# rs-anderson/explicit-alignment-for-vqa-tasks

Measured on AMD Instinct MI355X. Metric: mapper_train_samples_per_sec, higher is better.
Workload: dtype bf16; 1 GPU; cfg2: CLIP ViT-B/32 -> GPT-2-large (774M), MLP mapper, prefix 10, CC-shaped synthetic batches; per-GPU batch 64, S=42; fwd+bwd+AdamW; random-init weights; global_batch=64, seq_len=42, parallelism=dp1

## Files before the change

### explicit-alignment-for-vqa-tasks_amd/_lib.py

```python
from __future__ import annotations

import ctypes as C
import os

_HERE = os.path.dirname(os.path.abspath(__file__))
LIB_PATH = os.path.join(_HERE, "csrc", "libeavqa_hip.so")

F32, BF16 = 0, 1
ACT = {"none": 0, "tanh": 1, "relu": 2, "gelu_new": 3, "quick_gelu": 4}

i32, i64, f32, ptr = C.c_int, C.c_int64, C.c_float, C.c_void_p

SIGNATURES = {
    "eavqa_abi_version": [],
    "eavqa_strerror": [i32],
    "eavqa_check_device": [],
    "eavqa_gemm": [i32, i32, i32, i32, i32, i32, ptr, i64, ptr, i64, ptr, i64, i32, f32, ptr, i32, ptr, ptr, i64, ptr, i64, ptr],
    "eavqa_layernorm_fwd": [i32, i32, i32, i32, ptr, i64, ptr, ptr, f32, ptr, i64, ptr, ptr, ptr],
    "eavqa_layernorm_bwd": [i32, i32, i32, i32, ptr, i64, ptr, i64, ptr, ptr, ptr, ptr, ptr, i64, ptr, ptr, ptr, i64, ptr],
    "eavqa_layernorm_fwd_fp8": [i32, i32, i32, ptr, i64, ptr, ptr, f32, ptr, i64, ptr, ptr, ptr, ptr],
    "eavqa_layernorm_bwd_fp8": [i32, i32, i32, ptr, i64, ptr, i64, ptr, ptr, ptr, ptr, ptr, i64, ptr, i64, ptr, ptr],
    "eavqa_attention_fwd": [i32, i32, i32, i32, i32, i32, ptr, i64, ptr, i64, ptr, i64, ptr, i64, i64, i64, ptr, i64, ptr, i32, f32, ptr, ptr],
    "eavqa_attention_decode": [i32, i32, i32, i32, i32, ptr, i64, ptr, i64, ptr, i64, i64, ptr, ptr, i64, ptr, i64, ptr, i64, f32, ptr],
    "eavqa_attention_decode_splitk": [i32, i32, i32, i32, i32, ptr, i32, ptr, ptr, i64, ptr, i64, i64, ptr, i64, ptr, i64, f32, ptr],
    "eavqa_attention_bwd": [i32, i32, i32, i32, i32, i32, ptr, i64, ptr, i64, ptr, i64, ptr, i64, ptr, i64,
                            ptr, i64, ptr, i64, ptr, i64, ptr, ptr, i32, f32, ptr, ptr, ptr],
    "eavqa_build_prefix_rows": [i32, i32, i32, ptr, ptr, i32, i32, i32, ptr, ptr, ptr, ptr],
    "eavqa_build_fewshot_rows": [i32, i32, i32, i32, i64, ptr, ptr, i32, ptr, ptr, ptr, ptr, ptr],
    "eavqa_build_row_plan": [i32, i32, i32, ptr, ptr, ptr, ptr, ptr, ptr, ptr, ptr, ptr, ptr],
    "eavqa_copy_rows": [i32, i32, i32, i32, ptr, i64, i64, ptr, i64, i64, i64, ptr],
    "eavqa_transpose": [i32, i32, i32, ptr, i64, ptr, i64, ptr],
    "eavqa_select_rows": [i32, ptr, i32, ptr, ptr, ptr, ptr],
    "eavqa_move_rows": [i32, i32, i32, i32, ptr, i64, ptr, ptr, i64, ptr],
    "eavqa_l2_normalize_rows": [i32, i32, ptr, i64, ptr],
    "eavqa_topk_rows": [i32, i32, ptr, i64, i32, ptr, ptr, ptr],
    "eavqa_gemm_splitk_plan": [i32, i32, i32],
    "eavqa_gemm_splitk": [i32, i32, i32, i32, ptr, i64, ptr, i64, ptr, i32, ptr],
    "eavqa_splitk_finish": [i32, i32, i32, ptr, i32, ptr, i32, ptr, i64, i32, i32, ptr, i64, ptr, i64, ptr, i64, ptr],
    "eavqa_layernorm_splitk": [i32, i32, i32, ptr, i64, ptr, i32, ptr, ptr, i64, ptr, ptr, f32, ptr, i64, ptr],
    "eavqa_gemm_fp8_splitk_plan": [i32, i32, i32],
    "eavqa_gemm_fp8_splitk": [i32, i32, i32, ptr, i64, ptr, ptr, i64, f32, ptr, i32, ptr],
    "eavqa_layernorm_splitk_fp8": [i32, i32, ptr, i64, ptr, i32, ptr, ptr, i64, ptr, ptr, f32, ptr, i64, ptr, ptr],
    "eavqa_rmsnorm_splitk": [i32, i32, i32, ptr, i64, ptr, i32, ptr, i64, ptr, f32, ptr, i64, ptr],
    "eavqa_splitk_finish_gated": [i32, i32, i32, ptr, i32, i32, ptr, i64, ptr],
    "eavqa_attention_decode_splitk_rel": [i32, i32, i32, i32, i32, ptr, i32, i32, ptr, i64, ptr, i64, i64, ptr, i64, ptr, i64, f32, ptr, i64, i32, ptr],
    "eavqa_colsum": [i32, i32, i32, ptr, i64, ptr, i32, ptr],
    "eavqa_embed_assemble": [i32, i32, i32, ptr, ptr, ptr, i64, ptr, i64, ptr, i64, ptr, i64, ptr],
    "eavqa_embed_assemble_bwd": [i32, i32, i32, ptr, ptr, i64, ptr, i64, ptr],
    "eavqa_build_labels": [i32, i32, i32, i32, ptr, i64, i64, ptr, ptr],
    "eavqa_ce_fwd": [i32, i32, i32, ptr, i64, ptr, ptr, ptr, ptr, ptr, ptr],
    "eavqa_guard_count": [ptr, i32, ptr, ptr],
    "eavqa_ce_bwd": [i32, i32, i32, i32, ptr, i64, ptr, ptr, ptr, ptr, ptr, i64, ptr],
    "eavqa_greedy_pick": [i32, i32, ptr, i64, i64, i64, ptr, ptr, i64, ptr, ptr, ptr, ptr],
    "eavqa_adamw": [i64, ptr, ptr, ptr, ptr, i32, f32, f32, f32, f32, f32, f32, i32, ptr, ptr],
    "eavqa_patchify": [i32, i32, i32, i32, ptr, ptr, i64, ptr],
    "eavqa_vit_assemble": [i32, i32, i32, i32, ptr, i64, ptr, ptr, ptr, i64, ptr],
    "eavqa_cast_rows": [i32, i32, i64, ptr, i64, ptr, i64, ptr],
    "eavqa_quantize_rows_fp8": [i32, i32, i32, ptr, i64, ptr, i64, ptr, ptr],
    "eavqa_rmsnorm_fwd": [i32, i32, i32, i32, ptr, i64, ptr, f32, ptr, i64, ptr, ptr],
    "eavqa_rmsnorm_bwd": [i32, i32, i32, i32, ptr, i64, ptr, i64, ptr, ptr, ptr, ptr, i64, ptr, i64, ptr],
    "eavqa_gated_act_fwd": [i32, i32, i32, i32, ptr, i64, ptr, i64, ptr],
    "eavqa_gated_act_bwd": [i32, i32, i32, i32, ptr, i64, ptr, i64, ptr, i64, ptr],
    "eavqa_attention_fwd_rel": [i32, i32, i32, i32, i32, i32, ptr, i64, ptr, i64, ptr, i64, ptr, i64, i64, i64, ptr, i64, i32, f32, ptr, i64, i32, ptr, ptr],
    "eavqa_attention_bwd_rel": [i32, i32, i32, i32, i32, i32, ptr, i64, ptr, i64, ptr, i64, ptr, i64, ptr, i64, ptr, i64, ptr, i64, ptr, i64,
                                ptr, i32, f32, ptr, i64, i32, ptr, ptr, ptr],
    "eavqa_gemm_fp8": [i32, i32, i32, ptr, i64, ptr, ptr, i64, f32, ptr, i64, i32, f32, ptr, i32, ptr, ptr, i64, ptr, i64, ptr, i32],
}
class LMLayer(C.Structure):
    _fields_ = [(n, C.c_void_p) for n in ("ln1_g", "ln1_b", "w_qkv", "b_qkv", "w_o", "b_o", "ln2_g", "ln2_b", "w_fc1", "b_fc1",
                                          "w_fc2", "b_fc2", "k_cache", "v_cache")]


class LMLayerScales(C.Structure):
    _fields_ = [(n, C.c_float) for n in ("s_qkv", "s_o", "s_fc1", "s_fc2")]


class T5DecLayer(C.Structure):
    _fields_ = [(n, C.c_void_p) for n in ("ln_sa", "w_qkv", "w_o", "ln_ca", "w_q_ca", "w_o_ca", "ln_ff", "w_i", "w_o_ff", "k_cache", "v_cache",
                                          "cross_kv")]


class DecodeGemm(C.Structure):
    _fields_ = [("M", i32), ("N", i32), ("K", i32), ("A", ptr), ("lda", i64), ("a_kind", i32), ("gamma", ptr), ("beta", ptr), ("eps", f32),
                ("stats_in", ptr), ("n_stats_in", i32), ("stats_in_cols", i32), ("B", ptr), ("ldb", i64), ("gated_rows", i32),
                ("bias", ptr), ("act", i32), ("residual", ptr), ("ld_residual", i64), ("out_f32", i32), ("n_seg", i32),
                ("out", ptr * 3), ("ld_out", i64 * 3), ("stats_out", ptr)]


class GemmLn(C.Structure):
    _fields_ = [("copy_out", ptr), ("ld_copy", i64), ("stats_out", ptr), ("stats_ld", i32), ("ln_stats", ptr), ("ln_parts", i32),
                ("ln_ld", i32), ("ln_cols", i32), ("ln_c", ptr), ("ln_eps", f32), ("mean_out", ptr), ("rstd_out", ptr)]


SIGNATURES["eavqa_gemm_ln"] = SIGNATURES["eavqa_gemm"][:-1] + [C.POINTER(GemmLn), ptr]
SIGNATURES["eavqa_gemm_decode_cols"] = [i32, i32, i32, i32, i32]
SIGNATURES["eavqa_gemm_decode"] = [C.POINTER(DecodeGemm), ptr]
SIGNATURES["eavqa_t5_decoder_step_workspace_bytes"] = [i32, i32, i32, i32, i32, i32]
SIGNATURES["eavqa_t5_decoder_step"] = [i32, i32, C.POINTER(T5DecLayer), ptr, i32, i32, i32, i32, i32, i32, f32, i32, i32, i32, i32, ptr, ptr, ptr, i64,
                                       ptr, i64, i32, ptr, i64, ptr]
SIGNATURES["eavqa_lm_block_workspace_bytes"] = [i32, i32, i32, i32]
SIGNATURES["eavqa_lm_block_fp8_workspace_bytes"] = [i32, i32, i32]
SIGNATURES["eavqa_lm_block_forward_fp8"] = [i32, C.POINTER(LMLayer), C.POINTER(LMLayerScales), i32, i32, i32, i32, f32, i32, i32, i32, i32, ptr, ptr, i64, ptr, i64, ptr]
SIGNATURES["eavqa_lm_block_forward"] = [i32, i32, C.POINTER(LMLayer), i32, i32, i32, i32, f32, i32, i32, i32, i32, ptr, ptr, i64, ptr, i64, ptr]

SIGNATURES["eavqa_gemm_ex"] = SIGNATURES["eavqa_gemm"] + [i32]
SIGNATURES["eavqa_gemm_ln_ex"] = SIGNATURES["eavqa_gemm_ln"] + [i32]
SIGNATURES["eavqa_attention_fwd_ex"] = SIGNATURES["eavqa_attention_fwd"] + [i32]
SIGNATURES["eavqa_attention_bwd_ex"] = SIGNATURES["eavqa_attention_bwd"] + [i32]
SIGNATURES["eavqa_gemm_splitk_ex"] = SIGNATURES["eavqa_gemm_splitk"] + [i32]
SIGNATURES["eavqa_lm_block_forward_ex"] = SIGNATURES["eavqa_lm_block_forward"] + [i32]
SIGNATURES["eavqa_gemm_decode_ex"] = SIGNATURES["eavqa_gemm_decode"] + [i32]
SIGNATURES["eavqa_t5_decoder_step_ex"] = SIGNATURES["eavqa_t5_decoder_step"] + [i32]

_RESTYPES = {"eavqa_strerror": C.c_char_p, "eavqa_lm_block_workspace_bytes": C.c_int64, "eavqa_lm_block_fp8_workspace_bytes": C.c_int64, "eavqa_t5_decoder_step_workspace_bytes": C.c_int64}

_lib = None


class EavqaError(RuntimeError):
    pass


def load() -> C.CDLL:
    global _lib
    if _lib is not None:
        return _lib
    if not os.path.exists(LIB_PATH):
        raise EavqaError(
            f"{LIB_PATH} is missing: the HIP extension is the only compute path. "
            "Build it with `python -m eavqa_amd.build` (needs hipcc, no GPU required to compile)."
        )
    import torch
    lib = C.CDLL(LIB_PATH)
    for name, argtypes in SIGNATURES.items():
        fn = getattr(lib, name)
        fn.argtypes = argtypes
        fn.restype = _RESTYPES.get(name, C.c_int)
    got = lib.eavqa_abi_version()
    if got != 1:
        raise EavqaError(f"libeavqa_hip.so ABI version {got}, host code expects 1")
    _lib = lib
    return lib


def call(name: str, *args) -> None:
    lib = load()
    rc = getattr(lib, name)(*args)
    if rc != 0:
        raise EavqaError(f"{name} failed: {lib.eavqa_strerror(rc).decode()} (code {rc})")
```

### explicit-alignment-for-vqa-tasks_amd/csrc/gemm.hip

```cpp
#include "common.h"

namespace {

struct Knobs {
    int stagger;
    int ablate;
    bool disable_fast;
    int k64_mode;
    int big_mode;
    int deep;
    int shape_mode;
    int group_n;
    bool no_row_split;
    explicit Knobs(int k = 0) : stagger(k & 15), ablate((k >> 4) & 7), disable_fast(((k >> 7) & 1) != 0), k64_mode((k >> 8) & 63),
                                big_mode((k >> 14) & 3), deep((k >> 16) & 3), shape_mode((k >> 18) & 7), group_n((k >> 21) & 15),
                                no_row_split(((k >> 25) & 1) != 0) {}
};

struct GemmParamsBase {
    const void* A; const void* B; void* C;
    const float* bias; const void* aux_in; void* aux_out; const void* residual;
    const float* row_scale;
    int M, N, K;
    int64_t lda, ldb, ldc, ld_aux, ldr;
    int act, out_f32, res_lowp;
    int out_f16;
    int ablate;
    float alpha;
    int tiles_m, tiles_n;
    int group_n;
    int vec_c, vec_aux, vec_res, vec_bias;
};
struct GemmParams : GemmParamsBase {
    void* copy_out = nullptr; int64_t ld_copy = 0; int vec_copy = 0;
    float* stats_out = nullptr; int stats_ld = 0;
    const float* ln_stats = nullptr; int ln_parts = 0, ln_ld = 0;
    const float* ln_c = nullptr; float ln_inv_n = 0.f, ln_eps = 0.f;
    float* mean_out = nullptr; float* rstd_out = nullptr;
};
constexpr int LN_ROWSTAT_BYTES = 2048;
inline int ln_lds(const GemmParams& p) { return p.ln_stats ? LN_ROWSTAT_BYTES : 0; }
__device__ __forceinline__ GemmParams widen(const GemmParams& k) { return k; }
__device__ __forceinline__ GemmParams widen(const GemmParamsBase& k) { GemmParams p; static_cast<GemmParamsBase&>(p) = k; return p; }
template <bool LNX> struct KernArg { using type = GemmParamsBase; };
template <> struct KernArg<true> { using type = GemmParams; };

constexpr int BM = 128, BN = 128;
constexpr int CS_PITCH = 132;
constexpr int CS_BYTES = BM * CS_PITCH * 4;

__device__ __forceinline__ void tile_coords(const GemmParams& p, int& tm, int& tn) {
    const int nwg = p.tiles_m * p.tiles_n;
    const int bid = blockIdx.x;
    const int q = nwg >> 3, r = nwg & 7, xcd = bid & 7;
    const int wgid = (xcd < r ? xcd * (q + 1) : r * (q + 1) + (xcd - r) * q) + (bid >> 3);
    tm = wgid % p.tiles_m;
    tn = wgid / p.tiles_m;
}

__device__ __forceinline__ void ln_rowstat_fill(const GemmParams& p, float2* rowstat, int m0, int n0, int rows, int tid, int nthreads) {
    if (!p.ln_stats) return;
    for (int r = tid; r < rows; r += nthreads) {
        const int m = min(m0 + r, p.M - 1);
        const float2* q = reinterpret_cast<const float2*>(p.ln_stats) + (int64_t)m * p.ln_ld;
        float s = 0.f, ss = 0.f;
        if (((p.ln_ld | p.ln_parts) & 1) == 0 && (reinterpret_cast<uintptr_t>(p.ln_stats) & 15) == 0) {
            const float4* q4 = reinterpret_cast<const float4*>(q);
            const int n4 = p.ln_parts >> 1;
            for (int i = 0; i < n4; i += 4) {
                float4 t[4];
#pragma unroll
                for (int k = 0; k < 4; ++k) t[k] = q4[min(i + k, n4 - 1)];
#pragma unroll
                for (int k = 0; k < 4; ++k) {
                    const float w = (i + k < n4) ? 1.f : 0.f;
                    s += w * (t[k].x + t[k].z);
                    ss += w * (t[k].y + t[k].w);
                }
            }
        } else {
            for (int i = 0; i < p.ln_parts; ++i) { const float2 t = q[i]; s += t.x; ss += t.y; }
        }
        const float mean = s * p.ln_inv_n;
        const float rstd = 1.0f / sqrtf(fmaxf(ss * p.ln_inv_n - mean * mean, 0.f) + p.ln_eps);
        rowstat[r] = make_float2(rstd, -rstd * mean);
        if (n0 == 0 && m0 + r < p.M && p.mean_out) { p.mean_out[m] = mean; p.rstd_out[m] = rstd; }
    }
}

template <int TPR_, int RPP_, int NPASS_, int PITCH_, int ROWS_ = RPP_ * NPASS_, int LN_UNROLL_ = 4> struct EpiGeo {
    static constexpr int TPR = TPR_, RPP = RPP_, NPASS = NPASS_, PITCH = PITCH_, ROWS = ROWS_;
    static constexpr int LN_UNROLL = LN_UNROLL_;
};
using EpiGeo128 = EpiGeo<32, 8, 16, CS_PITCH>;

template <typename T, int ACT, int MODE, bool FULL, bool LNX>
__device__ __forceinline__ void epilogue_quad(const GemmParams& p, int m, int n, float (&v)[4], const float (&bias4)[4], const float2 rs,
                                              const float (&c4)[4]) {
    const T* aux_in = reinterpret_cast<const T*>(p.aux_in);
    T* aux_out = reinterpret_cast<T*>(p.aux_out);
    const bool full = FULL || (n + 3 < p.N);
    const float al = p.row_scale ? p.alpha * p.row_scale[m] : p.alpha;
    if (LNX && p.ln_stats) {
#pragma unroll
        for (int j = 0; j < 4; ++j) v[j] = (al * rs.x) * v[j] + (bias4[j] + rs.y * c4[j]);
    } else {
#pragma unroll
        for (int j = 0; j < 4; ++j) v[j] = al * v[j] + bias4[j];
    }
    if (aux_out) {
        T* q = aux_out + (int64_t)m * p.ld_aux + n;
        if (FULL || (full && p.vec_aux)) elem<T>::st4(q, make_float4(v[0], v[1], v[2], v[3]));
        else
            for (int j = 0; j < 4; ++j)
                if (n + j < p.N) elem<T>::st(q + j, v[j]);
    }
    if (MODE == 2) {
        const T* q = aux_in + (int64_t)m * p.ld_aux + n;
        float u[4] = {0.f, 0.f, 0.f, 0.f};
        if (FULL || (full && p.vec_aux)) { float4 t = elem<T>::ld4(q); u[0] = t.x; u[1] = t.y; u[2] = t.z; u[3] = t.w; }
        else
            for (int j = 0; j < 4; ++j)
                if (n + j < p.N) u[j] = elem<T>::ld(q + j);
#pragma unroll
        for (int j = 0; j < 4; ++j) v[j] *= act_bwd(ACT, u[j]);
    } else if (MODE == 1) {
#pragma unroll
        for (int j = 0; j < 4; ++j) v[j] = act_fwd(ACT, v[j]);
    }
    if (p.residual) {
        if (p.res_lowp == 2) {
            const f16_t* q = reinterpret_cast<const f16_t*>(p.residual) + (int64_t)m * p.ldr + n;
            if (FULL || (full && p.vec_res)) { float4 t = elem<f16_t>::ld4(q); v[0] += t.x; v[1] += t.y; v[2] += t.z; v[3] += t.w; }
            else
                for (int j = 0; j < 4; ++j)
                    if (n + j < p.N) v[j] += elem<f16_t>::ld(q + j);
        } else if (p.res_lowp) {
            const T* q = reinterpret_cast<const T*>(p.residual) + (int64_t)m * p.ldr + n;
            if (FULL || (full && p.vec_res)) { float4 t = elem<T>::ld4(q); v[0] += t.x; v[1] += t.y; v[2] += t.z; v[3] += t.w; }
            else
                for (int j = 0; j < 4; ++j)
                    if (n + j < p.N) v[j] += elem<T>::ld(q + j);
        } else {
            const float* q = reinterpret_cast<const float*>(p.residual) + (int64_t)m * p.ldr + n;
            if (FULL || (full && p.vec_res)) { float4 t = *reinterpret_cast<const float4*>(q); v[0] += t.x; v[1] += t.y; v[2] += t.z; v[3] += t.w; }
            else
                for (int j = 0; j < 4; ++j)
                    if (n + j < p.N) v[j] += q[j];
        }
    }
    if (p.out_f32) {
        float* q = reinterpret_cast<float*>(p.C) + (int64_t)m * p.ldc + n;
        if (FULL || (full && p.vec_c)) *reinterpret_cast<float4*>(q) = make_float4(v[0], v[1], v[2], v[3]);
        else
            for (int j = 0; j < 4; ++j)
                if (n + j < p.N) q[j] = v[j];
    } else if (p.out_f16) {
        f16_t* q = reinterpret_cast<f16_t*>(p.C) + (int64_t)m * p.ldc + n;
        if (FULL || (full && p.vec_c)) elem<f16_t>::st4(q, make_float4(v[0], v[1], v[2], v[3]));
        else
            for (int j = 0; j < 4; ++j)
                if (n + j < p.N) elem<f16_t>::st(q + j, v[j]);
    } else {
        T* q = reinterpret_cast<T*>(p.C) + (int64_t)m * p.ldc + n;
        if (FULL || (full && p.vec_c)) elem<T>::st4(q, make_float4(v[0], v[1], v[2], v[3]));
        else
            for (int j = 0; j < 4; ++j)
                if (n + j < p.N) elem<T>::st(q + j, v[j]);
    }
    if (LNX && p.copy_out) {
        T* q = reinterpret_cast<T*>(p.copy_out) + (int64_t)m * p.ld_copy + n;
        if (full && p.vec_copy) elem<T>::st4(q, make_float4(v[0], v[1], v[2], v[3]));
        else
            for (int j = 0; j < 4; ++j)
                if (n + j < p.N) elem<T>::st(q + j, v[j]);
    }
}

template <bool FULL>
__device__ __forceinline__ void load_bias4(const GemmParams& p, int n, float (&bias4)[4]) {
    bias4[0] = bias4[1] = bias4[2] = bias4[3] = 0.f;
    if (p.bias) {
        if (FULL) { const float4 b = *reinterpret_cast<const float4*>(p.bias + n); bias4[0] = b.x; bias4[1] = b.y; bias4[2] = b.z; bias4[3] = b.w; }
        else {
#pragma unroll
            for (int j = 0; j < 4; ++j)
                if (n + j < p.N) bias4[j] = p.bias[n + j];
        }
    }
}

struct LnArgs { const float2* rowstat; int row_base; };

template <typename T, int ACT, int MODE, bool FULL, typename G, bool LNX>
__device__ __forceinline__ void epilogue_body(const GemmParams& p, float* Cs, int m0, int n0, const LnArgs ln) {
    const int tid = threadIdx.x;
    if (G::ROWS != G::RPP * G::NPASS && tid >= G::TPR * G::RPP) return;
    const int c4 = (tid % G::TPR) * 4;
    const int n = n0 + c4;
    float bias4[4], lc4[4] = {0.f, 0.f, 0.f, 0.f};
    load_bias4<FULL>(p, n, bias4);
    if (LNX && p.ln_stats) {
#pragma unroll
        for (int j = 0; j < 4; ++j)
            if (FULL || n + j < p.N) lc4[j] = p.ln_c[n + j];
    }
    auto one_pass = [&](int pass) {
        const int row = (tid / G::TPR) + pass * G::RPP;
        const int m = m0 + row;
        if (G::ROWS != G::RPP * G::NPASS && row >= G::ROWS) return;
        if (!FULL && (m >= p.M || n >= p.N)) return;
        const float4 a = *reinterpret_cast<const float4*>(&Cs[row * G::PITCH + c4]);
        float v[4] = {a.x, a.y, a.z, a.w};
        const float2 rs = (LNX && p.ln_stats) ? ln.rowstat[ln.row_base + row] : make_float2(1.f, 0.f);
        epilogue_quad<T, ACT, MODE, FULL, LNX>(p, m, n, v, bias4, rs, lc4);
        if (LNX && p.stats_out) {
            if (!FULL) {
#pragma unroll
                for (int j = 0; j < 4; ++j)
                    if (n + j >= p.N) v[j] = 0.f;
            }
            *reinterpret_cast<float4*>(&Cs[row * G::PITCH + c4]) = make_float4(v[0], v[1], v[2], v[3]);
        }
    };
    if constexpr (LNX && G::LN_UNROLL == 1) {
#pragma unroll 1
        for (int pass = 0; pass < G::NPASS; ++pass) one_pass(pass);
    } else {
#pragma unroll 4
        for (int pass = 0; pass < G::NPASS; ++pass) one_pass(pass);
    }
}

template <typename G>
__device__ __forceinline__ void epilogue_row_sums(const GemmParams& p, const float* Cs, int m0, int n0) {
    constexpr int COLS = G::TPR * 4;
    static_assert(COLS >= 64 && COLS % 4 == 0, "a tile covers at least one 64-column slot");
    __syncthreads();
    const int cols = min(COLS, p.N - n0);
    const int slot0 = n0 / 64, slot1 = (n0 + COLS < p.N) ? (n0 + COLS) / 64 : p.stats_ld;
    for (int r = threadIdx.x; r < G::ROWS; r += blockDim.x) {
        const int m = m0 + r;
        if (m >= p.M) continue;
        float s = 0.f, ss = 0.f;
        for (int c = 0; c < cols; c += 4) {
            const float4 t = *reinterpret_cast<const float4*>(&Cs[r * G::PITCH + c]);
            s += (t.x + t.y) + (t.z + t.w);
            ss += (t.x * t.x + t.y * t.y) + (t.z * t.z + t.w * t.w);
        }
        float2* q = reinterpret_cast<float2*>(p.stats_out) + (int64_t)m * p.stats_ld;
        q[slot0] = make_float2(s, ss);
        for (int i = slot0 + 1; i < slot1; ++i) q[i] = make_float2(0.f, 0.f);
    }
}

template <typename T, int ACT, int MODE, typename G, bool LNX>
__device__ __forceinline__ void epilogue_mode(const GemmParams& p, float* Cs, int m0, int n0, const LnArgs ln) {
    constexpr int ROWS = G::ROWS, COLS = G::TPR * 4;
    const bool full_tile = (m0 + ROWS <= p.M) && (n0 + COLS <= p.N) && p.vec_c && (!(p.aux_in || p.aux_out) || p.vec_aux) &&
                           (!p.residual || p.vec_res) && (!p.bias || p.vec_bias);
    if (full_tile) epilogue_body<T, ACT, MODE, true, G, LNX>(p, Cs, m0, n0, ln);
    else epilogue_body<T, ACT, MODE, false, G, LNX>(p, Cs, m0, n0, ln);
    if (LNX && p.stats_out) epilogue_row_sums<G>(p, Cs, m0, n0);
}

template <typename T, typename G = EpiGeo128, bool LNX = true>
__device__ __forceinline__ void epilogue(const GemmParams& p, float* Cs, int m0, int n0, const LnArgs ln = LnArgs{nullptr, 0}) {
    const int mode = p.aux_in ? 2 : (p.act != EAVQA_ACT_NONE ? 1 : 0);
    if (mode == 0) { epilogue_mode<T, EAVQA_ACT_NONE, 0, G, LNX>(p, Cs, m0, n0, ln); return; }
    switch (p.act) {
        case EAVQA_ACT_TANH:
            if (mode == 1) epilogue_mode<T, EAVQA_ACT_TANH, 1, G, LNX>(p, Cs, m0, n0, ln); else epilogue_mode<T, EAVQA_ACT_TANH, 2, G, LNX>(p, Cs, m0, n0, ln);
            break;
        case EAVQA_ACT_RELU:
            if (mode == 1) epilogue_mode<T, EAVQA_ACT_RELU, 1, G, LNX>(p, Cs, m0, n0, ln); else epilogue_mode<T, EAVQA_ACT_RELU, 2, G, LNX>(p, Cs, m0, n0, ln);
            break;
        case EAVQA_ACT_GELU_NEW:
            if (mode == 1) epilogue_mode<T, EAVQA_ACT_GELU_NEW, 1, G, LNX>(p, Cs, m0, n0, ln); else epilogue_mode<T, EAVQA_ACT_GELU_NEW, 2, G, LNX>(p, Cs, m0, n0, ln);
            break;
        case EAVQA_ACT_QUICK_GELU:
            if (mode == 1) epilogue_mode<T, EAVQA_ACT_QUICK_GELU, 1, G, LNX>(p, Cs, m0, n0, ln); else epilogue_mode<T, EAVQA_ACT_QUICK_GELU, 2, G, LNX>(p, Cs, m0, n0, ln);
            break;
        default:
            epilogue_mode<T, EAVQA_ACT_NONE, 0, G, LNX>(p, Cs, m0, n0, ln);
    }
}

template <typename T, typename G = EpiGeo128>
__device__ __forceinline__ void epilogue_any(const GemmParams& p, float* Cs, int m0, int n0, const LnArgs ln = LnArgs{nullptr, 0}) {
    if (p.ln_stats || p.stats_out || p.copy_out) epilogue<T, G, true>(p, Cs, m0, n0, ln);
    else epilogue<T, G, false>(p, Cs, m0, n0, ln);
}


constexpr int BK16 = 64;
constexpr int OPER16_BYTES = 128 * BK16 * 2;

__device__ __forceinline__ int swz16(int row, int kc) { return row * 128 + ((kc ^ (row & 7)) << 4); }

template <bool KC>
__device__ __forceinline__ void g2r_16(uint4 (&r)[4], const bf16_t* X, int64_t ld, int row0, int rows_max,
                                       int k0, int K) {
    const int tid = threadIdx.x;
#pragma unroll
    for (int i = 0; i < 4; ++i) {
        const int c = tid + 256 * i;
        uint4 v = make_uint4(0u, 0u, 0u, 0u);
        if (KC) {
            const int row = c >> 3, kc = c & 7;
            const int gr = row0 + row, gk = k0 + kc * 8;
            if (gr < rows_max && gk < K) v = *reinterpret_cast<const uint4*>(X + (int64_t)gr * ld + gk);
        } else {
            const int k = c >> 4, rc = c & 15;
            const int gk = k0 + k, gr = row0 + rc * 8;
            if (gk < K && gr < rows_max) v = *reinterpret_cast<const uint4*>(X + (int64_t)gk * ld + gr);
        }
        r[i] = v;
    }
}
template <bool KC>
__device__ __forceinline__ void r2s_16(const uint4 (&r)[4], char* S) {
    const int tid = threadIdx.x;
#pragma unroll
    for (int i = 0; i < 4; ++i) {
        const int c = tid + 256 * i;
        if (KC) {
            const int row = c >> 3, kc = c & 7;
            *reinterpret_cast<uint4*>(S + swz16(row, kc)) = r[i];
        } else {
            const int k = c >> 4, rc = c & 15;
            const unsigned w[4] = {r[i].x, r[i].y, r[i].z, r[i].w};
#pragma unroll
            for (int j = 0; j < 8; ++j) {
                const int row = rc * 8 + j;
                const unsigned short e = (unsigned short)((j & 1) ? (w[j >> 1] >> 16) : (w[j >> 1] & 0xffffu));
                *reinterpret_cast<unsigned short*>(S + swz16(row, k >> 3) + (k & 7) * 2) = e;
            }
        }
    }
}

template <bool A_KC, bool B_KC>
__global__ __launch_bounds__(256) void gemm_bf16_kernel(GemmParams p) {
    extern __shared__ __attribute__((aligned(16))) char smem[];
    char* const As0 = smem;
    char* const Bs0 = smem + 2 * OPER16_BYTES;

    int tm, tn;
    tile_coords(p, tm, tn);
    const int m0 = tm * BM, n0 = tn * BN;
    const int tid = threadIdx.x, lane = tid & 63, wave = tid >> 6;
    const int wm = wave >> 1, wn = wave & 1;
    const bf16_t* A = reinterpret_cast<const bf16_t*>(p.A);
    const bf16_t* B = reinterpret_cast<const bf16_t*>(p.B);

    f32x4 acc[4][4];
#pragma unroll
    for (int i = 0; i < 4; ++i)
#pragma unroll
        for (int j = 0; j < 4; ++j) acc[i][j] = (f32x4){0.f, 0.f, 0.f, 0.f};

    const int nk = (p.K + BK16 - 1) / BK16;
    uint4 ra[4], rb[4];
    g2r_16<A_KC>(ra, A, p.lda, m0, p.M, 0, p.K);
    g2r_16<B_KC>(rb, B, p.ldb, n0, p.N, 0, p.K);
    r2s_16<A_KC>(ra, As0);
    r2s_16<B_KC>(rb, Bs0);
    __syncthreads();

    const int frow = lane & 15, fk = lane >> 4;
    for (int kt = 0; kt < nk; ++kt) {
        const int cur = kt & 1;
        if (kt + 1 < nk) {
            g2r_16<A_KC>(ra, A, p.lda, m0, p.M, (kt + 1) * BK16, p.K);
            g2r_16<B_KC>(rb, B, p.ldb, n0, p.N, (kt + 1) * BK16, p.K);
        }
        const char* Ac = As0 + cur * OPER16_BYTES;
        const char* Bc = Bs0 + cur * OPER16_BYTES;
#pragma unroll
        for (int s = 0; s < 2; ++s) {
            bf16x8 af[4], bfr[4];
#pragma unroll
            for (int i = 0; i < 4; ++i) {
                const int row = wm * 64 + i * 16 + frow;
                af[i] = *reinterpret_cast<const bf16x8*>(Ac + swz16(row, s * 4 + fk));
            }
#pragma unroll
            for (int j = 0; j < 4; ++j) {
                const int row = wn * 64 + j * 16 + frow;
                bfr[j] = *reinterpret_cast<const bf16x8*>(Bc + swz16(row, s * 4 + fk));
            }
#pragma unroll
            for (int i = 0; i < 4; ++i)
#pragma unroll
                for (int j = 0; j < 4; ++j)
                    acc[i][j] = __builtin_amdgcn_mfma_f32_16x16x32_bf16(af[i], bfr[j], acc[i][j], 0, 0, 0);
        }
        if (kt + 1 < nk) {
            r2s_16<A_KC>(ra, As0 + (cur ^ 1) * OPER16_BYTES);
            r2s_16<B_KC>(rb, Bs0 + (cur ^ 1) * OPER16_BYTES);
        }
        __syncthreads();
    }

    float* Cs = reinterpret_cast<float*>(smem);
#pragma unroll
    for (int i = 0; i < 4; ++i)
#pragma unroll
        for (int j = 0; j < 4; ++j)
#pragma unroll
            for (int r = 0; r < 4; ++r) {
                const int row = wm * 64 + i * 16 + (lane >> 4) * 4 + r;
                const int col = wn * 64 + j * 16 + (lane & 15);
                Cs[row * CS_PITCH + col] = acc[i][j][r];
            }
    float2* rowstat = reinterpret_cast<float2*>(smem + CS_BYTES);
    ln_rowstat_fill(p, rowstat, m0, n0, BM, tid, 256);
    __syncthreads();
    if constexpr (A_KC && B_KC) epilogue_any<bf16_t>(p, Cs, m0, n0, LnArgs{rowstat, 0});
    else epilogue<bf16_t, EpiGeo128, false>(p, Cs, m0, n0);
}


constexpr int FBK = 32;
constexpr int FOPER = 128 * FBK * 2;
constexpr int FSTAGE = 2 * FOPER;

__device__ __forceinline__ int fswz(int row, int kc) { return row * 64 + ((kc ^ ((-(row >> 2)) & 3)) << 4); }

struct FastMap { int gx, gy; };

__device__ __forceinline__ bool fast_tile(const GemmParams& p, int gx, int gy, int& tm, int& tn) {
    const int bid = blockIdx.x, xcd = bid & 7, local = bid >> 3;
    const int xi = xcd % gx, yi = xcd / gx;
    const int qm = p.tiles_m / gx, rm = p.tiles_m % gx, qn = p.tiles_n / gy, rn = p.tiles_n % gy;
    const int m_begin = xi * qm + min(xi, rm), m_cnt = qm + (xi < rm ? 1 : 0);
    const int n_begin = yi * qn + min(yi, rn), n_cnt = qn + (yi < rn ? 1 : 0);
    if (m_cnt == 0 || local >= m_cnt * n_cnt) return false;
    tm = m_begin + local % m_cnt;
    tn = n_begin + local / m_cnt;
    return true;
}

#define EAVQA_FAST_STEP(P, t)                                                                         \
    {                                                                                                 \
        const int rem = nk - 2 - (t);                                      \
         \
         \
         \
         \
        __builtin_amdgcn_sched_barrier(0);                                                            \
        __builtin_amdgcn_s_waitcnt(0xC07F);                                            \
        if ((t) + 1 < nk) {                                                                           \
             \
             \
             \
            if (ABL < 3) {                                                                            \
            if (rem >= NST - 2) __builtin_amdgcn_s_waitcnt(vm_only(4 * (NST - 2)));                   \
            else if (rem >= 6) __builtin_amdgcn_s_waitcnt(vm_only(24));                               \
            else if (rem == 5) __builtin_amdgcn_s_waitcnt(vm_only(20));                               \
            else if (rem == 4) __builtin_amdgcn_s_waitcnt(vm_only(16));                               \
            else if (rem == 3) __builtin_amdgcn_s_waitcnt(vm_only(12));                               \
            else if (rem == 2) __builtin_amdgcn_s_waitcnt(vm_only(8));                                \
            else if (rem == 1) __builtin_amdgcn_s_waitcnt(vm_only(4));                                \
            else __builtin_amdgcn_s_waitcnt(vm_only(0));                                              \
            __builtin_amdgcn_s_barrier();                                                             \
            }                                                                                         \
            if ((ABL < 1 || ABL >= 4) && (t) + NST < nk) issue((t) + NST);                            \
            if (ABL < 2) {                                                                            \
            const char* st = smem + (((t) + 1) & (NST - 1)) * FSTAGE;                                 \
            _Pragma("unroll") for (int i = 0; i < 4; ++i)                                             \
                fa[(P) ^ 1][i] = *reinterpret_cast<const bf16x8*>(st + a_off + i * 1024);             \
            _Pragma("unroll") for (int j = 0; j < 4; ++j)                                             \
                fb[(P) ^ 1][j] = *reinterpret_cast<const bf16x8*>(st + b_off + j * 1024);             \
            } else {                                                                                  \
            _Pragma("unroll") for (int i = 0; i < 4; ++i) { fa[(P) ^ 1][i] = fa[P][i]; fb[(P) ^ 1][i] = fb[P][i]; } \
            }                                                                                         \
        }                                                                                             \
        if (ABL != 4) {                                                                               \
        _Pragma("unroll") for (int i = 0; i < 4; ++i)                                                 \
            _Pragma("unroll") for (int j = 0; j < 4; ++j)                                             \
                acc[i][j] = __builtin_amdgcn_mfma_f32_16x16x32_bf16(fa[P][i], fb[P][j], acc[i][j], 0, 0, 0); \
        }                                                                                             \
    }

__device__ __host__ constexpr int vm_only(int n) { return (n & 15) | ((n >> 4) << 14) | 0x0F70; }

template <int ABL, int NST>
__global__ __launch_bounds__(256, 2) void gemm_bf16_fast_kernel(GemmParams p, int gx, int gy, int stagger) {
    extern __shared__ __attribute__((aligned(16))) char smem[];
    int tm, tn;
    if (!fast_tile(p, gx, gy, tm, tn)) return;
    if (stagger > 0 && ((blockIdx.x >> 3) & 1))
        for (int i = 0; i < stagger; ++i) __builtin_amdgcn_s_sleep(8);
    const int m0 = tm * BM, n0 = tn * BN;
    const int tid = threadIdx.x, lane = tid & 63;
    const int wave = __builtin_amdgcn_readfirstlane(tid >> 6);
    const int wm = wave >> 1, wn = wave & 1;
    const bf16_t* A = reinterpret_cast<const bf16_t*>(p.A);
    const bf16_t* B = reinterpret_cast<const bf16_t*>(p.B);

    const bf16_t* asrc[2];
    const bf16_t* bsrc[2];
#pragma unroll
    for (int i = 0; i < 2; ++i) {
        const int c = tid + 256 * i;
        const int row = c >> 2, pc = c & 3;
        const int kc = pc ^ ((-(row >> 2)) & 3);
        asrc[i] = A + (int64_t)min(m0 + row, p.M - 1) * p.lda + kc * 8;
        bsrc[i] = B + (int64_t)min(n0 + row, p.N - 1) * p.ldb + kc * 8;
    }
    const int dma_off = wave * 1024;

    auto issue = [&](int kt) {
        char* st = smem + (kt & (NST - 1)) * FSTAGE;
#pragma unroll
        for (int i = 0; i < 2; ++i) {
            __builtin_amdgcn_global_load_lds((const __attribute__((address_space(1))) void*)(asrc[i] + kt * FBK),
                                             (__attribute__((address_space(3))) void*)(st + dma_off + i * 4096), 16, 0, 0);
            if (ABL != 5 || i == 0 || lane < 16)
            __builtin_amdgcn_global_load_lds((const __attribute__((address_space(1))) void*)(bsrc[i] + kt * FBK),
                                             (__attribute__((address_space(3))) void*)(st + FOPER + dma_off + i * 4096), 16, 0, 0);
        }
    };

    f32x4 acc[4][4];
#pragma unroll
    for (int i = 0; i < 4; ++i)
#pragma unroll
        for (int j = 0; j < 4; ++j) acc[i][j] = (f32x4){0.f, 0.f, 0.f, 0.f};

    const int nk = p.K / FBK;
    const int frow = lane & 15, fk = lane >> 4;
    const int a_off = fswz(wm * 64 + frow, fk);
    const int b_off = FOPER + fswz(wn * 64 + frow, fk);
    bf16x8 fa[2][4], fb[2][4];

#pragma unroll
    for (int i = 0; i < NST; ++i)
        if (i < nk) issue(i);
    {
        const int later = min(nk, NST) - 1;
        if (later >= 7) __builtin_amdgcn_s_waitcnt(vm_only(28));
        else if (later == 6) __builtin_amdgcn_s_waitcnt(vm_only(24));
        else if (later == 5) __builtin_amdgcn_s_waitcnt(vm_only(20));
        else if (later == 4) __builtin_amdgcn_s_waitcnt(vm_only(16));
        else if (later == 3) __builtin_amdgcn_s_waitcnt(vm_only(12));
        else if (later == 2) __builtin_amdgcn_s_waitcnt(vm_only(8));
        else if (later == 1) __builtin_amdgcn_s_waitcnt(vm_only(4));
        else __builtin_amdgcn_s_waitcnt(vm_only(0));
    }
    __builtin_amdgcn_s_barrier();
#pragma unroll
    for (int i = 0; i < 4; ++i) fa[0][i] = *reinterpret_cast<const bf16x8*>(smem + a_off + i * 1024);
#pragma unroll
    for (int j = 0; j < 4; ++j) fb[0][j] = *reinterpret_cast<const bf16x8*>(smem + b_off + j * 1024);

    int t = 0;
    for (; t + 1 < nk; t += 2) {
        EAVQA_FAST_STEP(0, t)
        EAVQA_FAST_STEP(1, t + 1)
    }
    if (t < nk) EAVQA_FAST_STEP(0, t)
    __syncthreads();

    float* Cs = reinterpret_cast<float*>(smem);
#pragma unroll
    for (int i = 0; i < 4; ++i)
#pragma unroll
        for (int j = 0; j < 4; ++j)
#pragma unroll
            for (int r = 0; r < 4; ++r) {
                const int row = wm * 64 + i * 16 + (lane >> 4) * 4 + r;
                const int col = wn * 64 + j * 16 + (lane & 15);
                Cs[row * CS_PITCH + col] = acc[i][j][r];
            }
    __syncthreads();
    epilogue<bf16_t, EpiGeo128, false>(p, Cs, m0, n0);
}
#undef EAVQA_FAST_STEP


typedef void (*fast_kernel_t)(GemmParams, int, int, int);

int launch_fast(const GemmParams& p, hipStream_t stream, const Knobs& kn) {
    static const fast_kernel_t kernels[2] = {gemm_bf16_fast_kernel<0, 4>, gemm_bf16_fast_kernel<0, 8>};
    static std::atomic<bool> configured{false};
    if (!configured.load(std::memory_order_acquire)) {
        for (int i = 0; i < 2; ++i)
            if (hipFuncSetAttribute(reinterpret_cast<const void*>(kernels[i]), hipFuncAttributeMaxDynamicSharedMemorySize,
                                    8 * FSTAGE) != hipSuccess)
                return EAVQA_E_LAUNCH;
        configured.store(true, std::memory_order_release);
    }
    const bool deep = kn.deep == 2;
    const fast_kernel_t kernel = deep ? kernels[1] : kernels[0];
    const int lds_bytes = deep ? 8 * FSTAGE : CS_BYTES;
    int best_gx = 8, best_cost = 1 << 30;
    const int cand[4] = {8, 4, 2, 1};
    for (int c = 0; c < 4; ++c) {
        const int gx = cand[c], gy = 8 / gx;
        const int cost = (p.tiles_m + gx - 1) / gx + (p.tiles_n + gy - 1) / gy;
        if (cost < best_cost) { best_cost = cost; best_gx = gx; }
    }
    const int gx = best_gx, gy = 8 / gx;
    const int per_xcd = ((p.tiles_m + gx - 1) / gx) * ((p.tiles_n + gy - 1) / gy);
    hipLaunchKernelGGL(kernel, dim3(per_xcd * 8), dim3(256), lds_bytes, stream, p, gx, gy, kn.stagger);
    EAVQA_LAUNCH_CHECK();
    return EAVQA_OK;
}


__device__ __forceinline__ bool shaped_tile(int gx, int gy, int tiles_m, int tiles_n, int& tm, int& tn) {
    const int bid = blockIdx.x, xcd = bid & 7, local = bid >> 3;
    if (gx == 0) {
        const int nwg = tiles_m * tiles_n, q = nwg >> 3, r = nwg & 7;
        if (local >= q + (xcd < r ? 1 : 0)) return false;
        const int wgid = (xcd < r ? xcd * (q + 1) : r * (q + 1) + (xcd - r) * q) + local;
        tm = wgid % tiles_m;
        tn = wgid / tiles_m;
        return true;
    }
    const int xi = xcd % gx, yi = xcd / gx;
    const int qm = tiles_m / gx, rm = tiles_m % gx, qn = tiles_n / gy, rn = tiles_n % gy;
    const int m_begin = xi * qm + min(xi, rm), m_cnt = qm + (xi < rm ? 1 : 0);
    const int n_begin = yi * qn + min(yi, rn), n_cnt = qn + (yi < rn ? 1 : 0);
    if (m_cnt == 0 || local >= m_cnt * n_cnt) return false;
    tm = m_begin + local % m_cnt;
    tn = n_begin + local / m_cnt;
    return true;
}

struct GridPlan { int gx, gy, per_xcd; };
inline GridPlan plan_grid(int tiles_m, int tiles_n, int bm, int bn) {
    GridPlan g{8, 1, 0};
    int best_cost = 1 << 30;
    const int cand[4] = {8, 4, 2, 1};
    for (int c = 0; c < 4; ++c) {
        const int gx = cand[c], gy = 8 / gx;
        const int cost = ((tiles_m + gx - 1) / gx) * bm + ((tiles_n + gy - 1) / gy) * bn;
        if (cost < best_cost) { best_cost = cost; g.gx = gx; g.gy = gy; }
    }
    g.per_xcd = ((tiles_m + g.gx - 1) / g.gx) * ((tiles_n + g.gy - 1) / g.gy);
    const int even = (tiles_m * tiles_n + 7) / 8;
    if ((g.per_xcd + 31) / 32 > (even + 31) / 32) { g.gx = 0; g.gy = 0; g.per_xcd = even; }
    return g;
}

template <int WM, int WN, int MF, int NF> struct TileGeo {
    static constexpr int NT = 64 * WM * WN, NW = WM * WN;
    static constexpr int TBM = 16 * MF * WM, TBN = 16 * NF * WN;
    static constexpr int AFULL = 4 * TBM / NT, BFULL = 4 * TBN / NT;
    static constexpr int BREM = (4 * TBN - BFULL * NT) / NW;
    static constexpr int NDMA = AFULL + BFULL + (BREM > 0 ? 1 : 0);
    static constexpr int AOPER = TBM * 64, STAGE = (TBM + TBN) * 64, RING = 4 * STAGE;
    static constexpr int PITCH = TBN + 4;
    static constexpr int SP = (16 * MF * WM * PITCH * 4 <= RING) ? WM : ((16 * MF * (WM / 2) * PITCH * 4 <= RING) ? WM / 2 : 1);
    static constexpr int PROWS = 16 * MF * SP;
    static constexpr int TPR = TBN / 4, RPP = NT / TPR, NPASS = (PROWS + RPP - 1) / RPP;
    static_assert(4 * TBM == AFULL * NT, "A stage must split evenly");
    static_assert(BFULL * NT + BREM * NW == 4 * TBN && BREM < 64, "B stage: full pieces + one partial piece per wave");
    static_assert(16 * MF * PITCH * 4 <= RING, "one wave row of C must fit the ring");
    static_assert(WM % SP == 0, "passes cover whole wave rows");
};

#define EAVQA_SHAPED_STEP(P, t)                                                                       \
    {                                                                                                 \
        const int rem = nk - 2 - (t);                                                                 \
        __builtin_amdgcn_sched_barrier(0);                                                            \
        __builtin_amdgcn_s_waitcnt(0xC07F);                \
        if ((t) + 1 < nk) {                                                                           \
            if (rem >= 2) __builtin_amdgcn_s_waitcnt(vm_only(2 * G::NDMA));                           \
            else if (rem == 1) __builtin_amdgcn_s_waitcnt(vm_only(G::NDMA));                          \
            else __builtin_amdgcn_s_waitcnt(vm_only(0));                                              \
            __builtin_amdgcn_s_barrier();                                                             \
            if ((t) + 4 < nk) issue((t) + 4);                                                         \
            const char* st = smem + (((t) + 1) & 3) * G::STAGE;                                       \
            _Pragma("unroll") for (int i = 0; i < MF; ++i)                                            \
                fa[(P) ^ 1][i] = *reinterpret_cast<const bf16x8*>(st + a_off + i * 1024);             \
            _Pragma("unroll") for (int j = 0; j < NF; ++j)                                            \
                fb[(P) ^ 1][j] = *reinterpret_cast<const bf16x8*>(st + b_off + j * 1024);             \
        }                                                                                             \
        _Pragma("unroll") for (int i = 0; i < MF; ++i)                                                \
            _Pragma("unroll") for (int j = 0; j < NF; ++j)                                            \
                acc[i][j] = __builtin_amdgcn_mfma_f32_16x16x32_bf16(fa[P][i], fb[P][j], acc[i][j], 0, 0, 0); \
    }

template <int WM, int WN, int MF, int NF>
__global__ __launch_bounds__(64 * WM * WN, (WM * WN <= 4) ? 2 : 1) void gemm_bf16_shaped_kernel(GemmParams p, int gx, int gy, int tiles_m, int tiles_n) {
    using G = TileGeo<WM, WN, MF, NF>;
    extern __shared__ __attribute__((aligned(16))) char smem[];
    int tm, tn;
    if (!shaped_tile(gx, gy, tiles_m, tiles_n, tm, tn)) return;
    const int m0 = tm * G::TBM, n0 = tn * G::TBN;
    const int tid = threadIdx.x, lane = tid & 63;
    const int wave = __builtin_amdgcn_readfirstlane(tid >> 6);
    const int wm = wave / WN, wn = wave % WN;
    const bf16_t* A = reinterpret_cast<const bf16_t*>(p.A);
    const bf16_t* B = reinterpret_cast<const bf16_t*>(p.B);

    auto src_of = [&](const bf16_t* X, int64_t ld, int row0, int rows_max, int c) {
        const int row = c >> 2, pc = c & 3;
        return X + (int64_t)min(row0 + row, rows_max - 1) * ld + (pc ^ ((-(row >> 2)) & 3)) * 8;
    };
    const bf16_t* asrc[G::AFULL];
    const bf16_t* bsrc[G::BFULL + 1];
#pragma unroll
    for (int i = 0; i < G::AFULL; ++i) asrc[i] = src_of(A, p.lda, m0, p.M, tid + G::NT * i);
#pragma unroll
    for (int i = 0; i < G::BFULL; ++i) bsrc[i] = src_of(B, p.ldb, n0, p.N, tid + G::NT * i);
    bsrc[G::BFULL] = src_of(B, p.ldb, n0, p.N, G::BFULL * G::NT + wave * G::BREM + min(lane, max(G::BREM, 1) - 1));
    const int dma_off = wave * 1024;
    const int dma_off_x = G::AOPER + G::BFULL * G::NT * 16 + wave * G::BREM * 16;

    auto issue = [&](int kt) {
        char* st = smem + (kt & 3) * G::STAGE;
#pragma unroll
        for (int i = 0; i < G::AFULL; ++i)
            __builtin_amdgcn_global_load_lds((const __attribute__((address_space(1))) void*)(asrc[i] + kt * FBK),
                                             (__attribute__((address_space(3))) void*)(st + dma_off + i * G::NT * 16), 16, 0, 0);
#pragma unroll
        for (int i = 0; i < G::BFULL; ++i)
            __builtin_amdgcn_global_load_lds((const __attribute__((address_space(1))) void*)(bsrc[i] + kt * FBK),
                                             (__attribute__((address_space(3))) void*)(st + G::AOPER + dma_off + i * G::NT * 16), 16, 0, 0);
        if (G::BREM > 0 && lane < G::BREM)
            __builtin_amdgcn_global_load_lds((const __attribute__((address_space(1))) void*)(bsrc[G::BFULL] + kt * FBK),
                                             (__attribute__((address_space(3))) void*)(st + dma_off_x), 16, 0, 0);
    };

    f32x4 acc[MF][NF];
#pragma unroll
    for (int i = 0; i < MF; ++i)
#pragma unroll
        for (int j = 0; j < NF; ++j) acc[i][j] = (f32x4){0.f, 0.f, 0.f, 0.f};

    const int nk = p.K / FBK;
    const int frow = lane & 15, fk = lane >> 4;
    const int a_off = fswz(wm * 16 * MF + frow, fk);
    const int b_off = G::AOPER + fswz(wn * 16 * NF + frow, fk);
    bf16x8 fa[2][MF], fb[2][NF];

#pragma unroll
    for (int i = 0; i < 4; ++i)
        if (i < nk) issue(i);
    {
        const int later = min(nk, 4) - 1;
        if (later == 3) __builtin_amdgcn_s_waitcnt(vm_only(3 * G::NDMA));
        else if (later == 2) __builtin_amdgcn_s_waitcnt(vm_only(2 * G::NDMA));
        else if (later == 1) __builtin_amdgcn_s_waitcnt(vm_only(G::NDMA));
        else __builtin_amdgcn_s_waitcnt(vm_only(0));
    }
    __builtin_amdgcn_s_barrier();
#pragma unroll
    for (int i = 0; i < MF; ++i) fa[0][i] = *reinterpret_cast<const bf16x8*>(smem + a_off + i * 1024);
#pragma unroll
    for (int j = 0; j < NF; ++j) fb[0][j] = *reinterpret_cast<const bf16x8*>(smem + b_off + j * 1024);

    int t = 0;
    for (; t + 1 < nk; t += 2) {
        EAVQA_SHAPED_STEP(0, t)
        EAVQA_SHAPED_STEP(1, t + 1)
    }
    if (t < nk) EAVQA_SHAPED_STEP(0, t)
    __syncthreads();

    float* Cs = reinterpret_cast<float*>(smem);
    for (int pass = 0; pass < WM / G::SP; ++pass) {
        if (wm / G::SP == pass) {
            const int r0 = (wm % G::SP) * 16 * MF;
#pragma unroll
            for (int i = 0; i < MF; ++i)
#pragma unroll
                for (int j = 0; j < NF; ++j)
#pragma unroll
                    for (int r = 0; r < 4; ++r) {
                        const int row = r0 + i * 16 + (lane >> 4) * 4 + r;
                        const int col = wn * 16 * NF + j * 16 + (lane & 15);
                        Cs[row * G::PITCH + col] = acc[i][j][r];
                    }
        }
        __syncthreads();
        epilogue<bf16_t, EpiGeo<G::TPR, G::RPP, G::NPASS, G::PITCH, G::PROWS>, false>(p, Cs, m0 + pass * G::PROWS, n0);
        if (pass + 1 < WM / G::SP) __syncthreads();
    }
}
#undef EAVQA_SHAPED_STEP

template <int WM, int WN, int MF, int NF>
int launch_shaped(const GemmParams& p, hipStream_t stream) {
    using G = TileGeo<WM, WN, MF, NF>;
    static std::atomic<bool> configured{false};
    if (!configured.load(std::memory_order_acquire)) {
        if (hipFuncSetAttribute(reinterpret_cast<const void*>(gemm_bf16_shaped_kernel<WM, WN, MF, NF>),
                                hipFuncAttributeMaxDynamicSharedMemorySize, G::RING) != hipSuccess)
            return EAVQA_E_LAUNCH;
        configured.store(true, std::memory_order_release);
    }
    const int tiles_m = (p.M + G::TBM - 1) / G::TBM, tiles_n = (p.N + G::TBN - 1) / G::TBN;
    const GridPlan g = plan_grid(tiles_m, tiles_n, G::TBM, G::TBN);
    hipLaunchKernelGGL((gemm_bf16_shaped_kernel<WM, WN, MF, NF>), dim3(g.per_xcd * 8), dim3(G::NT), G::RING, stream, p, g.gx, g.gy,
                       tiles_m, tiles_n);
    EAVQA_LAUNCH_CHECK();
    return EAVQA_OK;
}


struct ShapeChoice { int bm, bn; float rate; int (*launch)(const GemmParams&, hipStream_t); };
const ShapeChoice SHAPES[5] = {
    {128, 80, 1.17f, launch_shaped<4, 1, 2, 5>}, {128, 96, 1.20f, launch_shaped<4, 1, 2, 6>},
    {256, 128, 1.15f, launch_shaped<4, 2, 4, 4>}, {256, 160, 1.23f, launch_shaped<4, 2, 4, 5>}, {256, 192, 1.39f, launch_shaped<4, 2, 4, 6>},
};
constexpr float RATE_FAST = 1.245f, RATE_BIG = 1.27f;

inline float tile_cost(const GemmParams& p, int bm, int bn, float rate) {
    const int tiles_m = (p.M + bm - 1) / bm, tiles_n = (p.N + bn - 1) / bn;
    const GridPlan g = plan_grid(tiles_m, tiles_n, bm, bn);
    const float rounds = float((g.per_xcd + 31) / 32);
    return rounds * (rate * (bm + bn) * (p.K / 32) + 0.25f * bm * bn);
}

constexpr int GBM = 256, GBN = 256, GBK = 64;
constexpr int BIG_GROUP_N = 8;
constexpr int GOPER = GBM * GBK * 2;
constexpr int GSTAGE = 2 * GOPER;
constexpr int GCS_PITCH = GBN + 4;
constexpr int GLDS_BYTES = 2 * GSTAGE;
using EpiGeo256 = EpiGeo<64, 16, 4, GCS_PITCH, 64, 1>;

__device__ __forceinline__ bool big_tile(const GemmParams& p, int gx, int gy, int tiles_m, int tiles_n, int& tm, int& tn) {
    const int bid = blockIdx.x, xcd = bid & 7, local = bid >> 3;
    const int xi = xcd % gx, yi = xcd / gx;
    const int qm = tiles_m / gx, rm = tiles_m % gx, qn = tiles_n / gy, rn = tiles_n % gy;
    const int m_begin = xi * qm + min(xi, rm), m_cnt = qm + (xi < rm ? 1 : 0);
    const int n_begin = yi * qn + min(yi, rn), n_cnt = qn + (yi < rn ? 1 : 0);
    if (m_cnt == 0 || local >= m_cnt * n_cnt) return false;
    const int GN = p.group_n;
    if (GN <= 0) {
        tm = m_begin + local % m_cnt;
        tn = n_begin + local / m_cnt;
        return true;
    }
    const int per_group = m_cnt * GN;
    const int g = local / per_group, r = local - g * per_group;
    const int gn = min(GN, n_cnt - g * GN);
    tm = m_begin + r / gn;
    tn = n_begin + g * GN + r % gn;
    return true;
}

template <bool LNX>
__global__ __launch_bounds__(1024) void gemm_bf16_big_kernel(typename KernArg<LNX>::type pk, int gx, int gy, int tiles_m, int tiles_n) {
    const GemmParams p = widen(pk);
    extern __shared__ __attribute__((aligned(16))) char smem[];
    int tm, tn;
    if (!big_tile(p, gx, gy, tiles_m, tiles_n, tm, tn)) return;
    const int m0 = tm * GBM, n0 = tn * GBN;
    const int tid = threadIdx.x, lane = tid & 63;
    const int wave = __builtin_amdgcn_readfirstlane(tid >> 6);
    const int wm = wave >> 2, wn = wave & 3;
    const bf16_t* A = reinterpret_cast<const bf16_t*>(p.A);
    const bf16_t* B = reinterpret_cast<const bf16_t*>(p.B);

    const bf16_t* asrc[2];
    const bf16_t* bsrc[2];
#pragma unroll
    for (int i = 0; i < 2; ++i) {
        const int c = tid + 1024 * i;
        const int row = c >> 3, pc = c & 7;
        asrc[i] = A + (int64_t)min(m0 + row, p.M - 1) * p.lda + (pc ^ (row & 7)) * 8;
        bsrc[i] = B + (int64_t)min(n0 + row, p.N - 1) * p.ldb + (pc ^ (row & 7)) * 8;
    }
    const int dma_off = wave * 1024;
    auto issue = [&](int kt) {
        char* st = smem + (kt & 1) * GSTAGE;
#pragma unroll
        for (int i = 0; i < 2; ++i) {
            __builtin_amdgcn_global_load_lds((const __attribute__((address_space(1))) void*)(asrc[i] + kt * GBK),
                                             (__attribute__((address_space(3))) void*)(st + dma_off + i * 16384), 16, 0, 0);
            __builtin_amdgcn_global_load_lds((const __attribute__((address_space(1))) void*)(bsrc[i] + kt * GBK),
                                             (__attribute__((address_space(3))) void*)(st + GOPER + dma_off + i * 16384), 16, 0, 0);
        }
    };

    f32x4 acc[4][4];
#pragma unroll
    for (int i = 0; i < 4; ++i)
#pragma unroll
        for (int j = 0; j < 4; ++j) acc[i][j] = (f32x4){0.f, 0.f, 0.f, 0.f};

    const int nk = p.K / GBK;
    const int frow = lane & 15, fk = lane >> 4;
    const int arow = wm * 64 + frow, brow = wn * 64 + frow;
    issue(0);
    float2* rowstat = reinterpret_cast<float2*>(smem + GLDS_BYTES);
    if (LNX) ln_rowstat_fill(p, rowstat, m0, n0, GBM, tid, 1024);
    for (int kt = 0; kt < nk; ++kt) {
        __builtin_amdgcn_sched_barrier(0);
        __builtin_amdgcn_s_waitcnt(0x0070);
        __builtin_amdgcn_s_barrier();
        if (kt + 1 < nk) issue(kt + 1);
        const char* st = smem + (kt & 1) * GSTAGE;
#pragma unroll
        for (int s = 0; s < 2; ++s) {
            bf16x8 af[4], bfr[4];
            const int sw = ((s * 4 + fk) ^ (frow & 7)) << 4;
#pragma unroll
            for (int i = 0; i < 4; ++i) af[i] = *reinterpret_cast<const bf16x8*>(st + (arow + 16 * i) * 128 + sw);
#pragma unroll
            for (int j = 0; j < 4; ++j) bfr[j] = *reinterpret_cast<const bf16x8*>(st + GOPER + (brow + 16 * j) * 128 + sw);
#pragma unroll
            for (int i = 0; i < 4; ++i)
#pragma unroll
                for (int j = 0; j < 4; ++j)
                    acc[i][j] = __builtin_amdgcn_mfma_f32_16x16x32_bf16(af[i], bfr[j], acc[i][j], 0, 0, 0);
        }
    }
    __syncthreads();

    float* Cs = reinterpret_cast<float*>(smem);
    for (int slab = 0; slab < 4; ++slab) {
        if (wm == slab) {
#pragma unroll
            for (int i = 0; i < 4; ++i)
#pragma unroll
                for (int j = 0; j < 4; ++j)
#pragma unroll
                    for (int r = 0; r < 4; ++r) {
                        const int row = i * 16 + (lane >> 4) * 4 + r;
                        const int col = wn * 64 + j * 16 + (lane & 15);
                        Cs[row * GCS_PITCH + col] = acc[i][j][r];
                    }
        }
        __syncthreads();
        epilogue<bf16_t, EpiGeo256, LNX>(p, Cs, m0 + slab * 64, n0, LnArgs{rowstat, slab * 64});
        __syncthreads();
    }
}

inline int big_grid(int tiles_m, int tiles_n, int& gx, int& gy) {
    int best_gx = 8, best_cost = 1 << 30, best_rounds = 1 << 30;
    const int cand[4] = {8, 4, 2, 1};
    for (int c = 0; c < 4; ++c) {
        const int x = cand[c], y = 8 / x;
        const int pm = (tiles_m + x - 1) / x, pn = (tiles_n + y - 1) / y;
        const int rounds = (pm * pn + 31) / 32, cost = pm + pn;
        if (rounds < best_rounds || (rounds == best_rounds && cost < best_cost)) { best_rounds = rounds; best_cost = cost; best_gx = x; }
    }
    gx = best_gx; gy = 8 / gx;
    return ((tiles_m + gx - 1) / gx) * ((tiles_n + gy - 1) / gy);
}

int launch_big(const GemmParams& p, hipStream_t stream) {
    static std::atomic<bool> configured{false};
    if (!configured.load(std::memory_order_acquire)) {
        if (hipFuncSetAttribute(reinterpret_cast<const void*>(gemm_bf16_big_kernel<false>), hipFuncAttributeMaxDynamicSharedMemorySize,
                                GLDS_BYTES) != hipSuccess ||
            hipFuncSetAttribute(reinterpret_cast<const void*>(gemm_bf16_big_kernel<true>), hipFuncAttributeMaxDynamicSharedMemorySize,
                                GLDS_BYTES + LN_ROWSTAT_BYTES) != hipSuccess)
            return EAVQA_E_LAUNCH;
        configured.store(true, std::memory_order_release);
    }
    const int tiles_m = (p.M + GBM - 1) / GBM, tiles_n = (p.N + GBN - 1) / GBN;
    int gx, gy;
    const int per_xcd = big_grid(tiles_m, tiles_n, gx, gy);
    if (p.ln_stats || p.stats_out || p.copy_out)
        hipLaunchKernelGGL(gemm_bf16_big_kernel<true>, dim3(per_xcd * 8), dim3(1024), GLDS_BYTES + ln_lds(p), stream, p, gx, gy, tiles_m, tiles_n);
    else
        hipLaunchKernelGGL(gemm_bf16_big_kernel<false>, dim3(per_xcd * 8), dim3(1024), GLDS_BYTES, stream, p, gx, gy, tiles_m, tiles_n);
    EAVQA_LAUNCH_CHECK();
    return EAVQA_OK;
}

inline int big_split_rows(int M, int N) {
    const int rem = M % GBM;
    if (rem == 0 || rem > 192 || M <= GBM) return 0;
    int gx, gy;
    const int tiles_n = (N + GBN - 1) / GBN;
    const int with = (big_grid((M + GBM - 1) / GBM, tiles_n, gx, gy) + 31) / 32, without = (big_grid(M / GBM, tiles_n, gx, gy) + 31) / 32;
    return without < with ? rem : 0;
}

bool use_big(const GemmParams& p, const Knobs& kn) {
    if (p.K % GBK) return false;
    if (kn.big_mode == 1) return false;
    if (kn.big_mode == 2) return true;
    const int tiles = ((p.M + GBM - 1) / GBM) * ((p.N + GBN - 1) / GBN);
    return tiles >= 144;
}


#include "gemm_k64.hip"

inline float k64_cost(const GemmParams& p, const K64Choice& c, float* multi_round_loop = nullptr) {
    const int tiles_m = (p.M + c.bm - 1) / c.bm, tiles_n = (p.N + c.bn - 1) / c.bn;
    const GridPlan g = plan_grid(tiles_m, tiles_n, c.bm, c.bn);
    const float rounds = float((g.per_xcd + 31) / 32);
    const float loop = rounds * c.rate * (c.bm + c.bn) * (p.K / 64);
    if (multi_round_loop) *multi_round_loop = rounds > 1.f ? loop : 0.f;
    return loop + rounds * 0.1f * c.bm * c.bn + 4500.f;
}

#include "gemm_fp8.hip"

template <int MF>
__global__ __launch_bounds__(512) void gemm_bf16_skinny_kernel(GemmParams p) {
    __shared__ float red[8][64][17];
    const int tid = threadIdx.x, lane = tid & 63, wave = tid >> 6;
    const int x = lane & 15, g = lane >> 4;
    const int n0 = blockIdx.x * 16;
    const bf16_t* A = reinterpret_cast<const bf16_t*>(p.A);
    const bf16_t* B = reinterpret_cast<const bf16_t*>(p.B);
    const int nsteps = p.K >> 5;
    const int per_wave = (nsteps + 7) >> 3;
    const int s_begin = wave * per_wave, s_end = min(nsteps, s_begin + per_wave);
    const bf16_t* bp = B + (int64_t)min(n0 + x, p.N - 1) * p.ldb + 8 * g;
    const bf16_t* ap[MF];
#pragma unroll
    for (int f = 0; f < MF; ++f) ap[f] = A + (int64_t)min(16 * f + x, p.M - 1) * p.lda + 8 * g;
    f32x4 acc[MF];
#pragma unroll
    for (int f = 0; f < MF; ++f) acc[f] = (f32x4){0.f, 0.f, 0.f, 0.f};

    int s = s_begin;
    for (; s + 8 <= s_end; s += 8) {
        bf16x8 b[8], a[8][MF];
#pragma unroll
        for (int u = 0; u < 8; ++u) {
            b[u] = *reinterpret_cast<const bf16x8*>(bp + (s + u) * 32);
#pragma unroll
            for (int f = 0; f < MF; ++f) a[u][f] = *reinterpret_cast<const bf16x8*>(ap[f] + (s + u) * 32);
        }
#pragma unroll
        for (int u = 0; u < 8; ++u)
#pragma unroll
            for (int f = 0; f < MF; ++f) acc[f] = __builtin_amdgcn_mfma_f32_16x16x32_bf16(a[u][f], b[u], acc[f], 0, 0, 0);
    }
    for (; s < s_end; ++s) {
        const bf16x8 b = *reinterpret_cast<const bf16x8*>(bp + s * 32);
#pragma unroll
        for (int f = 0; f < MF; ++f) {
            const bf16x8 a = *reinterpret_cast<const bf16x8*>(ap[f] + s * 32);
            acc[f] = __builtin_amdgcn_mfma_f32_16x16x32_bf16(a, b, acc[f], 0, 0, 0);
        }
    }
#pragma unroll
    for (int f = 0; f < MF; ++f)
#pragma unroll
        for (int r = 0; r < 4; ++r) red[wave][16 * f + 4 * g + r][x] = acc[f][r];
    __syncthreads();
    for (int e = tid; e < MF * 16 * 16; e += 512) {
        const int m = e >> 4, c = e & 15, n = n0 + c;
        if (m >= p.M || n >= p.N) continue;
        float v = 0.f;
#pragma unroll
        for (int w = 0; w < 8; ++w) v += red[w][m][c];
        v = p.alpha * v + (p.bias ? p.bias[n] : 0.f);
        const int64_t ia = (int64_t)m * p.ld_aux + n;
        if (p.aux_out) elem<bf16_t>::st(reinterpret_cast<bf16_t*>(p.aux_out) + ia, v);
        if (p.aux_in) v *= act_bwd(p.act, elem<bf16_t>::ld(reinterpret_cast<const bf16_t*>(p.aux_in) + ia));
        else v = act_fwd(p.act, v);
        if (p.residual) v += p.res_lowp == 2 ? elem<f16_t>::ld(reinterpret_cast<const f16_t*>(p.residual) + (int64_t)m * p.ldr + n)
                             : p.res_lowp ? elem<bf16_t>::ld(reinterpret_cast<const bf16_t*>(p.residual) + (int64_t)m * p.ldr + n)
                                          : reinterpret_cast<const float*>(p.residual)[(int64_t)m * p.ldr + n];
        if (p.out_f32) reinterpret_cast<float*>(p.C)[(int64_t)m * p.ldc + n] = v;
        else if (p.out_f16) elem<f16_t>::st(reinterpret_cast<f16_t*>(p.C) + (int64_t)m * p.ldc + n, v);
        else elem<bf16_t>::st(reinterpret_cast<bf16_t*>(p.C) + (int64_t)m * p.ldc + n, v);
    }
}

int launch_skinny(const GemmParams& p, hipStream_t stream) {
    const int blocks = (p.N + 15) / 16;
    const int mf = (p.M + 15) / 16;
    if (mf == 1) hipLaunchKernelGGL(gemm_bf16_skinny_kernel<1>, dim3(blocks), dim3(512), 0, stream, p);
    else if (mf == 2) hipLaunchKernelGGL(gemm_bf16_skinny_kernel<2>, dim3(blocks), dim3(512), 0, stream, p);
    else if (mf == 3) hipLaunchKernelGGL(gemm_bf16_skinny_kernel<3>, dim3(blocks), dim3(512), 0, stream, p);
    else hipLaunchKernelGGL(gemm_bf16_skinny_kernel<4>, dim3(blocks), dim3(512), 0, stream, p);
    EAVQA_LAUNCH_CHECK();
    return EAVQA_OK;
}

constexpr int BK32 = 16;
constexpr int PITCH32 = 17;
constexpr int OPER32_FLOATS = 128 * PITCH32;

template <bool KC>
__device__ __forceinline__ void g2r_32(float4 (&r)[2], const float* X, int64_t ld, int row0, int rows_max,
                                       int k0, int K) {
    const int tid = threadIdx.x;
#pragma unroll
    for (int i = 0; i < 2; ++i) {
        const int c = tid + 256 * i;
        float4 v = make_float4(0.f, 0.f, 0.f, 0.f);
        if (KC) {
            const int row = c >> 2, kc = c & 3;
            const int gr = row0 + row, gk = k0 + kc * 4;
            if (gr < rows_max && gk < K) v = *reinterpret_cast<const float4*>(X + (int64_t)gr * ld + gk);
        } else {
            const int k = c >> 5, rc = c & 31;
            const int gk = k0 + k, gr = row0 + rc * 4;
            if (gk < K && gr < rows_max) v = *reinterpret_cast<const float4*>(X + (int64_t)gk * ld + gr);
        }
        r[i] = v;
    }
}
template <bool KC>
__device__ __forceinline__ void r2s_32(const float4 (&r)[2], float* S) {
    const int tid = threadIdx.x;
#pragma unroll
    for (int i = 0; i < 2; ++i) {
        const int c = tid + 256 * i;
        const float w[4] = {r[i].x, r[i].y, r[i].z, r[i].w};
        if (KC) {
            const int row = c >> 2, kc = c & 3;
#pragma unroll
            for (int j = 0; j < 4; ++j) S[row * PITCH32 + kc * 4 + j] = w[j];
        } else {
            const int k = c >> 5, rc = c & 31;
#pragma unroll
            for (int j = 0; j < 4; ++j) S[(rc * 4 + j) * PITCH32 + k] = w[j];
        }
    }
}

template <bool A_KC, bool B_KC>
__global__ __launch_bounds__(256) void gemm_f32_kernel(GemmParams p) {
    extern __shared__ __attribute__((aligned(16))) char smem[];
    float* sm = reinterpret_cast<float*>(smem);
    float* const As0 = sm;
    float* const Bs0 = sm + 2 * OPER32_FLOATS;

    int tm, tn;
    tile_coords(p, tm, tn);
    const int m0 = tm * BM, n0 = tn * BN;
    const int tid = threadIdx.x, lane = tid & 63, wave = tid >> 6;
    const int wm = wave >> 1, wn = wave & 1;
    const float* A = reinterpret_cast<const float*>(p.A);
    const float* B = reinterpret_cast<const float*>(p.B);

    f32x16 acc[2][2];
#pragma unroll
    for (int i = 0; i < 2; ++i)
#pragma unroll
        for (int j = 0; j < 2; ++j)
#pragma unroll
            for (int r = 0; r < 16; ++r) acc[i][j][r] = 0.f;

    const int nk = (p.K + BK32 - 1) / BK32;
    float4 ra[2], rb[2];
    g2r_32<A_KC>(ra, A, p.lda, m0, p.M, 0, p.K);
    g2r_32<B_KC>(rb, B, p.ldb, n0, p.N, 0, p.K);
    r2s_32<A_KC>(ra, As0);
    r2s_32<B_KC>(rb, Bs0);
    __syncthreads();

    const int frow = lane & 31, fk = lane >> 5;
    for (int kt = 0; kt < nk; ++kt) {
        const int cur = kt & 1;
        if (kt + 1 < nk) {
            g2r_32<A_KC>(ra, A, p.lda, m0, p.M, (kt + 1) * BK32, p.K);
            g2r_32<B_KC>(rb, B, p.ldb, n0, p.N, (kt + 1) * BK32, p.K);
        }
        const float* Ac = As0 + cur * OPER32_FLOATS;
        const float* Bc = Bs0 + cur * OPER32_FLOATS;
#pragma unroll
        for (int s = 0; s < BK32 / 2; ++s) {
            float af[2], bfr[2];
#pragma unroll
            for (int i = 0; i < 2; ++i) af[i] = Ac[(wm * 64 + i * 32 + frow) * PITCH32 + s * 2 + fk];
#pragma unroll
            for (int j = 0; j < 2; ++j) bfr[j] = Bc[(wn * 64 + j * 32 + frow) * PITCH32 + s * 2 + fk];
#pragma unroll
            for (int i = 0; i < 2; ++i)
#pragma unroll
                for (int j = 0; j < 2; ++j)
                    acc[i][j] = __builtin_amdgcn_mfma_f32_32x32x2f32(af[i], bfr[j], acc[i][j], 0, 0, 0);
        }
        if (kt + 1 < nk) {
            r2s_32<A_KC>(ra, As0 + (cur ^ 1) * OPER32_FLOATS);
            r2s_32<B_KC>(rb, Bs0 + (cur ^ 1) * OPER32_FLOATS);
        }
        __syncthreads();
    }

    float* Cs = reinterpret_cast<float*>(smem);
#pragma unroll
    for (int i = 0; i < 2; ++i)
#pragma unroll
        for (int j = 0; j < 2; ++j)
#pragma unroll
            for (int r = 0; r < 16; ++r) {
                const int row = wm * 64 + i * 32 + (r & 3) + 8 * (r >> 2) + 4 * (lane >> 5);
                const int col = wn * 64 + j * 32 + (lane & 31);
                Cs[row * CS_PITCH + col] = acc[i][j][r];
            }
    float2* rowstat = reinterpret_cast<float2*>(smem + CS_BYTES);
    ln_rowstat_fill(p, rowstat, m0, n0, BM, tid, 256);
    __syncthreads();
    if constexpr (A_KC && B_KC) epilogue_any<float>(p, Cs, m0, n0, LnArgs{rowstat, 0});
    else epilogue<float, EpiGeo128, false>(p, Cs, m0, n0);
}

typedef void (*gemm_kernel_t)(GemmParams);

int launch(gemm_kernel_t kernel, const GemmParams& p, hipStream_t stream) {
    static std::atomic<gemm_kernel_t> configured[8];
    bool done = false;
    for (int i = 0; i < 8; ++i) done |= (configured[i].load(std::memory_order_acquire) == kernel);
    if (!done) {
        if (hipFuncSetAttribute(reinterpret_cast<const void*>(kernel), hipFuncAttributeMaxDynamicSharedMemorySize,
                                CS_BYTES + LN_ROWSTAT_BYTES) != hipSuccess)
            return EAVQA_E_LAUNCH;
        for (int i = 0; i < 8; ++i) {
            gemm_kernel_t expected = nullptr;
            if (configured[i].compare_exchange_strong(expected, kernel, std::memory_order_acq_rel) || expected == kernel) break;
        }
    }
    const int nwg = p.tiles_m * p.tiles_n;
    hipLaunchKernelGGL(kernel, dim3(nwg), dim3(256), CS_BYTES + ln_lds(p), stream, p);
    EAVQA_LAUNCH_CHECK();
    return EAVQA_OK;
}


}

namespace {
eavqa_gemm_ln_t ln_rows_from(const eavqa_gemm_ln_t& x, int64_t r0, size_t esz) {
    eavqa_gemm_ln_t y = x;
    if (x.copy_out) y.copy_out = static_cast<char*>(x.copy_out) + (size_t)r0 * (size_t)x.ld_copy * esz;
    if (x.stats_out) y.stats_out = x.stats_out + (size_t)r0 * (size_t)x.stats_ld * 2;
    if (x.ln_stats) y.ln_stats = x.ln_stats + (size_t)r0 * (size_t)x.ln_ld * 2;
    if (x.mean_out) y.mean_out = x.mean_out + r0;
    if (x.rstd_out) y.rstd_out = x.rstd_out + r0;
    return y;
}

int gemm_impl(int dtype, int a_kc, int b_kc, int M, int N, int K,
              const void* A, int64_t lda, const void* B, int64_t ldb,
              void* C, int64_t ldc, int out_flags, float alpha,
              const float* bias, int act,
              const void* aux_in, void* aux_out, int64_t ld_aux,
              const void* residual, int64_t ldr, const eavqa_gemm_ln_t* ln, void* stream, int knobs) {
    const Knobs kn(knobs);
    const bool ln_consumer = ln && ln->ln_stats;
    if (ln) {
        if (ln->copy_out && ln->ld_copy < N) return EAVQA_E_ARG;
        if (ln->stats_out && ln->stats_ld < (N + 63) / 64) return EAVQA_E_ARG;
        if (ln_consumer && (!ln->ln_c || ln->ln_parts <= 0 || ln->ln_ld < ln->ln_parts || ln->ln_cols <= 0 || !(ln->ln_eps >= 0.f))) return EAVQA_E_ARG;
        if ((ln->mean_out != nullptr) != (ln->rstd_out != nullptr) || (ln->mean_out && !ln_consumer)) return EAVQA_E_ARG;
        if (!(a_kc && b_kc)) return EAVQA_E_SHAPE;
    }
    if (out_flags & ~(EAVQA_GEMM_OUT_F32 | EAVQA_GEMM_RESIDUAL_LOWP | EAVQA_GEMM_STREAM_F16)) return EAVQA_E_ARG;
    if ((out_flags & (EAVQA_GEMM_RESIDUAL_LOWP | EAVQA_GEMM_STREAM_F16)) && dtype != EAVQA_BF16) return EAVQA_E_DTYPE;
    const int out_f32 = out_flags & EAVQA_GEMM_OUT_F32;
    const int stream_f16 = (out_flags & EAVQA_GEMM_STREAM_F16) != 0;
    const int res_lowp = (out_flags & EAVQA_GEMM_RESIDUAL_LOWP) ? (stream_f16 ? 2 : 1) : 0;
    if (!A || !B || !C) return EAVQA_E_ARG;
    if (M <= 0 || N <= 0 || K <= 0) return EAVQA_E_ARG;
    if (dtype != EAVQA_F32 && dtype != EAVQA_BF16) return EAVQA_E_DTYPE;
    if (act < EAVQA_ACT_NONE || act > EAVQA_ACT_QUICK_GELU) return EAVQA_E_DTYPE;
    const int vec = dtype == EAVQA_BF16 ? 8 : 4;
    const int a_contig = a_kc ? K : M, b_contig = b_kc ? K : N;
    if (a_contig % vec || b_contig % vec) return EAVQA_E_SHAPE;
    if (lda % vec || ldb % vec) return EAVQA_E_ALIGN;
    if (!eavqa_aligned16(A) || !eavqa_aligned16(B)) return EAVQA_E_ALIGN;
    if (lda < a_contig || ldb < b_contig || ldc < N) return EAVQA_E_ARG;
    if ((aux_in || aux_out) && ld_aux < N) return EAVQA_E_ARG;
    if (residual && ldr < N) return EAVQA_E_ARG;

    GemmParams p;
    p.A = A; p.B = B; p.C = C; p.bias = bias; p.aux_in = aux_in; p.aux_out = aux_out; p.residual = residual; p.row_scale = nullptr; p.ablate = kn.ablate;
    p.M = M; p.N = N; p.K = K; p.lda = lda; p.ldb = ldb; p.ldc = ldc; p.ld_aux = ld_aux; p.ldr = ldr;
    p.act = act; p.out_f32 = out_f32; p.res_lowp = res_lowp; p.out_f16 = stream_f16 && !out_f32; p.alpha = alpha;
    p.group_n = kn.group_n == 0 ? BIG_GROUP_N : kn.group_n - 1;
    p.tiles_m = (M + BM - 1) / BM;
    p.tiles_n = (N + BN - 1) / BN;
    const int esz = dtype == EAVQA_BF16 ? 2 : 4;
    auto vec_ok = [](const void* ptr, int64_t ld, int bytes_per_elem) {
        return ((reinterpret_cast<uintptr_t>(ptr) % (4 * bytes_per_elem)) == 0) && (ld % 4 == 0);
    };
    p.vec_c = vec_ok(C, ldc, out_f32 ? 4 : esz);
    p.vec_aux = vec_ok(aux_in ? aux_in : aux_out, ld_aux, esz);
    p.vec_res = vec_ok(residual, ldr, res_lowp ? esz : 4);
    p.vec_bias = (reinterpret_cast<uintptr_t>(bias) % 16) == 0;
    if (ln) {
        p.copy_out = ln->copy_out; p.ld_copy = ln->ld_copy; p.vec_copy = ln->copy_out ? vec_ok(ln->copy_out, ln->ld_copy, esz) : 0;
        p.stats_out = ln->stats_out; p.stats_ld = ln->stats_ld;
        if (ln_consumer) {
            p.ln_stats = ln->ln_stats; p.ln_parts = ln->ln_parts; p.ln_ld = ln->ln_ld; p.ln_c = ln->ln_c;
            p.ln_inv_n = 1.0f / float(ln->ln_cols); p.ln_eps = ln->ln_eps; p.mean_out = ln->mean_out; p.rstd_out = ln->rstd_out;
        }
    }
    hipStream_t s = reinterpret_cast<hipStream_t>(stream);
    if (dtype == EAVQA_BF16) {
        if (a_kc && b_kc && (K % 64) == 0 && kn.k64_mode >= 2 && kn.k64_mode < 2 + N_K64) return K64_SHAPES[kn.k64_mode - 2].launch(p, s);
        const bool few_columns = kn.k64_mode == 0 && kn.shape_mode == 0 && kn.big_mode == 0 && N <= 4096;
        if (!ln && a_kc && b_kc && !kn.disable_fast && M <= 64 && (K % 32) == 0 && N >= 64 && (kn.k64_mode == 1 || (K % 64) != 0 || few_columns)) return launch_skinny(p, s);
        const int big_rem = (a_kc && b_kc && kn.big_mode != 1 && !kn.no_row_split) ? big_split_rows(M, N) : 0;
        const float big_split_ns = big_rem ? 12000.f : 0.f;
        auto run_big = [&](const GemmParams& pp) -> int {
            if (!big_rem) return launch_big(pp, s);
            GemmParams p1 = pp;
            p1.M = M - big_rem;
            p1.tiles_m = (p1.M + BM - 1) / BM;
            const int rc1 = launch_big(p1, s);
            if (rc1) return rc1;
            const int64_t r0 = M - big_rem;
            const size_t ces = out_f32 ? 4 : 2, res_es = res_lowp ? 2 : 4;
            auto off = [](const void* base, int64_t rows, int64_t ld, size_t es) -> const void* {
                return base ? static_cast<const char*>(base) + (size_t)rows * (size_t)ld * es : nullptr;
            };
            eavqa_gemm_ln_t ln2;
            if (ln) ln2 = ln_rows_from(*ln, r0, 2);
            return gemm_impl(dtype, a_kc, b_kc, big_rem, N, K, off(A, r0, lda, 2), lda, B, ldb, const_cast<void*>(off(C, r0, ldc, ces)), ldc, out_flags,
                             alpha, bias, act, off(aux_in, r0, ld_aux, 2), const_cast<void*>(off(aux_out, r0, ld_aux, 2)), ld_aux,
                             off(residual, r0, ldr, res_es), ldr, ln ? &ln2 : nullptr, stream, 0);
        };
        int bgx, bgy;
        const int big_rounds = (big_grid((M - big_rem + GBM - 1) / GBM, (N + GBN - 1) / GBN, bgx, bgy) + 31) / 32;
        const bool many_big_tiles = big_rounds >= 4 || (big_rounds >= 2 && (M + GBM - 1) / GBM > 96);
        if (a_kc && b_kc && !kn.disable_fast && (K % 64) == 0 && kn.k64_mode != 1 && kn.shape_mode == 0 && kn.big_mode == 0 && !many_big_tiles) {
            int pick = K64_AUTO[0];
            float best_loop = 0.f;
            float best = k64_cost(p, K64_SHAPES[pick], &best_loop);
            for (int i = 1; i < N_K64_AUTO; ++i) {
                float loop;
                const float c = k64_cost(p, K64_SHAPES[K64_AUTO[i]], &loop);
                if (c < best) { best = c; pick = K64_AUTO[i]; best_loop = loop; }
            }
            best += 0.35f * best_loop;
            const float big_cost = float(big_rounds) * (float(K / 64) * (big_rounds == 1 ? 1380.f : 1530.f) + 9000.f) + 3000.f + big_split_ns;
            if (M > 64 && big_cost < best) return run_big(p);
            return K64_SHAPES[pick].launch(p, s);
        }
        if (a_kc && b_kc && !kn.disable_fast && (K % FBK) == 0 && !ln) {
            if (kn.shape_mode >= 2 && kn.shape_mode < 7) return SHAPES[kn.shape_mode - 2].launch(p, s);
            const bool big_ok = (K % GBK) == 0 && kn.big_mode != 1;
            if (big_ok && kn.big_mode == 2) return run_big(p);
            float best = tile_cost(p, 128, 128, RATE_FAST);
            int pick = -1;
            if (big_ok && use_big(p, kn)) {
                GemmParams pf = p;
                pf.M = M - big_rem;
                best = fminf(best, tile_cost(pf, 256, 256, RATE_BIG) + big_split_ns);
                pick = -2;
            }
            if (kn.shape_mode != 1)
                for (int i = 0; i < 5; ++i) {
                    const float c = tile_cost(p, SHAPES[i].bm, SHAPES[i].bn, SHAPES[i].rate);
                    if (c < best * 0.95f) { best = c; pick = i; }
                }
            if (pick >= 0) return SHAPES[pick].launch(p, s);
            if (pick == -2) return run_big(p);
            return launch_fast(p, s, kn);
        }
        if (a_kc && b_kc) return launch(gemm_bf16_kernel<true, true>, p, s);
        if (a_kc && !b_kc) return launch(gemm_bf16_kernel<true, false>, p, s);
        if (!a_kc && b_kc) return launch(gemm_bf16_kernel<false, true>, p, s);
        return launch(gemm_bf16_kernel<false, false>, p, s);
    }
    if (a_kc && b_kc) return launch(gemm_f32_kernel<true, true>, p, s);
    if (a_kc && !b_kc) return launch(gemm_f32_kernel<true, false>, p, s);
    if (!a_kc && b_kc) return launch(gemm_f32_kernel<false, true>, p, s);
    return launch(gemm_f32_kernel<false, false>, p, s);
}
}

extern "C" int eavqa_gemm_ex(int dtype, int a_kc, int b_kc, int M, int N, int K,
                             const void* A, int64_t lda, const void* B, int64_t ldb,
                             void* C, int64_t ldc, int out_flags, float alpha,
                             const float* bias, int act,
                             const void* aux_in, void* aux_out, int64_t ld_aux,
                             const void* residual, int64_t ldr, void* stream, int knobs) {
    return gemm_impl(dtype, a_kc, b_kc, M, N, K, A, lda, B, ldb, C, ldc, out_flags, alpha, bias, act, aux_in, aux_out, ld_aux, residual, ldr,
                     nullptr, stream, knobs);
}

extern "C" int eavqa_gemm_ln_ex(int dtype, int a_kc, int b_kc, int M, int N, int K,
                                const void* A, int64_t lda, const void* B, int64_t ldb,
                                void* C, int64_t ldc, int out_flags, float alpha,
                                const float* bias, int act,
                                const void* aux_in, void* aux_out, int64_t ld_aux,
                                const void* residual, int64_t ldr, const eavqa_gemm_ln_t* ln, void* stream, int knobs) {
    if (!ln) return EAVQA_E_ARG;
    return gemm_impl(dtype, a_kc, b_kc, M, N, K, A, lda, B, ldb, C, ldc, out_flags, alpha, bias, act, aux_in, aux_out, ld_aux, residual, ldr,
                     ln, stream, knobs);
}

extern "C" int eavqa_gemm_ln(int dtype, int a_kc, int b_kc, int M, int N, int K,
                             const void* A, int64_t lda, const void* B, int64_t ldb,
                             void* C, int64_t ldc, int out_flags, float alpha,
                             const float* bias, int act,
                             const void* aux_in, void* aux_out, int64_t ld_aux,
                             const void* residual, int64_t ldr, const eavqa_gemm_ln_t* ln, void* stream) {
    return eavqa_gemm_ln_ex(dtype, a_kc, b_kc, M, N, K, A, lda, B, ldb, C, ldc, out_flags, alpha, bias, act, aux_in, aux_out, ld_aux, residual,
                            ldr, ln, stream, 0);
}

extern "C" int eavqa_gemm(int dtype, int a_kc, int b_kc, int M, int N, int K,
                          const void* A, int64_t lda, const void* B, int64_t ldb,
                          void* C, int64_t ldc, int out_flags, float alpha,
                          const float* bias, int act,
                          const void* aux_in, void* aux_out, int64_t ld_aux,
                          const void* residual, int64_t ldr, void* stream) {
    return eavqa_gemm_ex(dtype, a_kc, b_kc, M, N, K, A, lda, B, ldb, C, ldc, out_flags, alpha, bias, act, aux_in, aux_out, ld_aux,
                         residual, ldr, stream, 0);
}

extern "C" int eavqa_quantize_rows_fp8(int dtype, int rows, int cols, const void* x, int64_t ldx, void* out, int64_t ld_out,
                                       float* row_scale, void* stream) {
    if (!x || !out || !row_scale || rows <= 0 || cols <= 0) return EAVQA_E_ARG;
    if (cols % 4) return EAVQA_E_SHAPE;
    if (ldx % 4 || ld_out % 4 || ldx < cols || ld_out < cols) return EAVQA_E_ALIGN;
    if ((reinterpret_cast<uintptr_t>(x) & 7u) || (reinterpret_cast<uintptr_t>(out) & 3u)) return EAVQA_E_ALIGN;
    hipStream_t s = reinterpret_cast<hipStream_t>(stream);
    const bool reg_ok = dtype == EAVQA_BF16 && cols % 8 == 0 && cols <= 16384 && ldx % 8 == 0 && ld_out % 8 == 0 &&
                        !(reinterpret_cast<uintptr_t>(x) & 15u) && !(reinterpret_cast<uintptr_t>(out) & 7u);
    if (reg_ok) {
        const int nv = (cols / 8 + 255) / 256;
#define EAVQA_QR(NV) hipLaunchKernelGGL(quantize_rows_fp8_reg_kernel<NV>, dim3(rows), dim3(256), 0, s, cols, reinterpret_cast<const bf16_t*>(x), \
                                        ldx, reinterpret_cast<unsigned char*>(out), ld_out, row_scale)
        if (nv <= 1) EAVQA_QR(1); else if (nv <= 2) EAVQA_QR(2); else if (nv <= 4) EAVQA_QR(4); else EAVQA_QR(8);
#undef EAVQA_QR
    } else if (dtype == EAVQA_BF16)
        hipLaunchKernelGGL(quantize_rows_fp8_kernel<bf16_t>, dim3(rows), dim3(256), 0, s, cols, reinterpret_cast<const bf16_t*>(x), ldx,
                           reinterpret_cast<unsigned char*>(out), ld_out, row_scale);
    else if (dtype == EAVQA_F32)
        hipLaunchKernelGGL(quantize_rows_fp8_kernel<float>, dim3(rows), dim3(256), 0, s, cols, reinterpret_cast<const float*>(x), ldx,
                           reinterpret_cast<unsigned char*>(out), ld_out, row_scale);
    else return EAVQA_E_DTYPE;
    EAVQA_LAUNCH_CHECK();
    return EAVQA_OK;
}

extern "C" int eavqa_gemm_fp8(int M, int N, int K, const void* A, int64_t lda, const float* a_row_scale, const void* B, int64_t ldb,
                              float b_scale, void* C, int64_t ldc, int out_f32, float alpha, const float* bias, int act,
                              const void* aux_in, void* aux_out, int64_t ld_aux, const float* residual, int64_t ldr, void* stream, int tile) {
    if (!A || !B || !C || !a_row_scale) return EAVQA_E_ARG;
    if (M <= 0 || N <= 0 || K <= 0) return EAVQA_E_ARG;
    if (act < EAVQA_ACT_NONE || act > EAVQA_ACT_QUICK_GELU) return EAVQA_E_DTYPE;
    if (K % 128) return EAVQA_E_SHAPE;
    if (lda % 16 || ldb % 16 || !eavqa_aligned16(A) || !eavqa_aligned16(B)) return EAVQA_E_ALIGN;
    if (lda < K || ldb < K || ldc < N) return EAVQA_E_ARG;
    if ((aux_in || aux_out) && ld_aux < N) return EAVQA_E_ARG;
    if (residual && ldr < N) return EAVQA_E_ARG;
    GemmParams p;
    p.A = A; p.B = B; p.C = C; p.bias = bias; p.aux_in = aux_in; p.aux_out = aux_out; p.residual = residual; p.row_scale = a_row_scale; p.ablate = 0;
    p.M = M; p.N = N; p.K = K; p.lda = lda; p.ldb = ldb; p.ldc = ldc; p.ld_aux = ld_aux; p.ldr = ldr;
    p.act = act; p.out_f32 = out_f32; p.res_lowp = 0; p.out_f16 = 0; p.alpha = alpha * b_scale;
    p.group_n = 0;
    p.tiles_m = (M + BM - 1) / BM;
    p.tiles_n = (N + BN - 1) / BN;
    auto vec_ok = [](const void* ptr, int64_t ld, int bytes_per_elem) {
        return ((reinterpret_cast<uintptr_t>(ptr) % (4 * bytes_per_elem)) == 0) && (ld % 4 == 0);
    };
    p.vec_c = vec_ok(C, ldc, out_f32 ? 4 : 2);
    p.vec_aux = vec_ok(aux_in ? aux_in : aux_out, ld_aux, 2);
    p.vec_res = vec_ok(residual, ldr, 4);
    p.vec_bias = (reinterpret_cast<uintptr_t>(bias) % 16) == 0;
    hipStream_t s = reinterpret_cast<hipStream_t>(stream);
    if (tile > 0 && tile <= N_FP8) return FP8_SHAPES[tile - 1].launch(p, s);
    GemmParams q = p;
    q.K = K / 2;
    int pick = 0;
    float best = k64_cost(q, FP8_SHAPES[0]);
    for (int i = 1; i < N_FP8; ++i) {
        const float c = k64_cost(q, FP8_SHAPES[i]);
        if (c < best) { best = c; pick = i; }
    }
    return FP8_SHAPES[pick].launch(p, s);
}
```

### explicit-alignment-for-vqa-tasks_amd/csrc/gemm_k64.hip

```cpp
template <int N> __device__ __forceinline__ void wait_vm() { __builtin_amdgcn_s_waitcnt(vm_only(N)); }


template <int WM, int WN, int MF, int NF, int NST_, int LW_> struct K64SGeo {
    static constexpr int NST = NST_, LW = LW_;
    static constexpr int NC = WM * WN;
    static constexpr int NT = 64 * (NC + LW);
    static constexpr int TBM = 16 * MF * WM, TBN = 16 * NF * WN;
    static constexpr int PT = (TBM + TBN) / 8;
    static constexpr int P_LO = PT / LW, P_HI = (PT + LW - 1) / LW, N_HI = PT % LW;
    static constexpr int AOPER = TBM * 128, STAGE = (TBM + TBN) * 128, RING = NST * STAGE;
    static constexpr int PITCH = TBN + 4;
    static constexpr int SP = (16 * MF * WM * PITCH * 4 <= RING) ? WM : ((16 * MF * (WM / 2) * PITCH * 4 <= RING && WM >= 2) ? WM / 2 : 1);
    static constexpr int MFC = (16 * MF * PITCH * 4 <= RING) ? MF : MF / 2;
    static constexpr int PROWS = 16 * MFC * SP;
    static constexpr int TPR = TBN / 4;
    static constexpr int RPP = NT / TPR, NPASS = (PROWS + RPP - 1) / RPP;
    static_assert((TBM + TBN) % 8 == 0 && P_LO >= 1, "stage must cut into whole pieces, at least one per loader");
    static_assert(16 * MFC * PITCH * 4 <= RING && MF % MFC == 0 && (MFC == MF || SP == 1), "C staging pass must fit the ring");
    static_assert(WM % SP == 0 && RING <= 160 * 1024 && NT <= 1024, "geometry");
    static_assert(P_HI * (NST - 1) <= 63 && NST >= 2 && NST <= 6, "vmcnt field");
};

template <class G>
__device__ __forceinline__ void k64s_loader_role(const char* A, const char* B, int64_t lda_bytes, int64_t ldb_bytes, int M, int N, int m0,
                                                 int n0, int nk, char* smem, int lw, int lane) {
    constexpr int NST = G::NST;
    const bool hi = lw < G::N_HI;
    const char* src[G::P_HI];
    int dst[G::P_HI];
#pragma unroll
    for (int i = 0; i < G::P_HI; ++i) {
        const int piece = min(lw + G::LW * i, G::PT - 1);
        const int row = piece * 8 + (lane >> 3), slot = lane & 7;
        const int kc = (slot ^ (lane >> 3)) * 16;
        src[i] = row < G::TBM ? A + (int64_t)min(m0 + row, M - 1) * lda_bytes + kc
                              : B + (int64_t)min(n0 + row - G::TBM, N - 1) * ldb_bytes + kc;
        dst[i] = piece * 1024;
    }
    auto issue = [&](int kt, int stage) {
        char* st = smem + stage * G::STAGE;
#pragma unroll
        for (int i = 0; i < G::P_HI; ++i)
            if (i < G::P_LO || hi)
                __builtin_amdgcn_global_load_lds((const __attribute__((address_space(1))) void*)(src[i] + (int64_t)kt * 128),
                                                 (__attribute__((address_space(3))) void*)(st + dst[i]), 16, 0, 0);
    };
    auto wait_tiles = [&](int tiles) {
        if (hi) {
            if (NST >= 6 && tiles >= 5) wait_vm<(NST >= 6 ? 5 : 0) * G::P_HI>();
            else if (NST >= 5 && tiles >= 4) wait_vm<(NST >= 5 ? 4 : 0) * G::P_HI>();
            else if (NST >= 4 && tiles >= 3) wait_vm<(NST >= 4 ? 3 : 0) * G::P_HI>();
            else if (NST >= 3 && tiles >= 2) wait_vm<(NST >= 3 ? 2 : 0) * G::P_HI>();
            else if (tiles >= 1) wait_vm<G::P_HI>();
            else wait_vm<0>();
        } else {
            if (NST >= 6 && tiles >= 5) wait_vm<(NST >= 6 ? 5 : 0) * G::P_LO>();
            else if (NST >= 5 && tiles >= 4) wait_vm<(NST >= 5 ? 4 : 0) * G::P_LO>();
            else if (NST >= 4 && tiles >= 3) wait_vm<(NST >= 4 ? 3 : 0) * G::P_LO>();
            else if (NST >= 3 && tiles >= 2) wait_vm<(NST >= 3 ? 2 : 0) * G::P_LO>();
            else if (tiles >= 1) wait_vm<G::P_LO>();
            else wait_vm<0>();
        }
    };
#pragma unroll
    for (int i = 0; i < NST; ++i)
        if (i < nk) issue(i, i);
    wait_tiles(min(nk, NST) - 1);
    __builtin_amdgcn_s_barrier();
    int stage = 0;
    for (int t = 0; t + 1 < nk; ++t) {
        wait_tiles(min(nk - 1, t + NST - 1) - (t + 1));
        __builtin_amdgcn_s_barrier();
        if (t + NST < nk) issue(t + NST, stage);
        stage = (stage + 1 == NST) ? 0 : stage + 1;
    }
}

template <class G, int WM, int WN, int MF, int NF, bool LNX = false>
__device__ __forceinline__ void k64s_store_tile(const GemmParams& p, const f32x4 (&acc)[MF][NF], char* smem, int wave, int lane, int m0, int n0,
                                                const float2* rowstat = nullptr) {
    const int wm = wave / WN, wn = wave % WN;
    float* Cs = reinterpret_cast<float*>(smem);
    constexpr int CH = MF / G::MFC;
    constexpr int NPASSES = (WM / G::SP) * CH;
    for (int pass = 0; pass < NPASSES; ++pass) {
        const int wgrp = pass / CH, chunk = pass % CH;
        if (wave < G::NC && wm / G::SP == wgrp) {
            const int r0 = (wm % G::SP) * 16 * G::MFC;
#pragma unroll
            for (int i = 0; i < MF; ++i) {
                if (i / G::MFC != chunk) continue;
#pragma unroll
                for (int j = 0; j < NF; ++j)
#pragma unroll
                    for (int r = 0; r < 4; ++r) {
                        const int row = r0 + (i % G::MFC) * 16 + (lane >> 4) * 4 + r;
                        const int col = wn * 16 * NF + j * 16 + (lane & 15);
                        Cs[row * G::PITCH + col] = acc[i][j][r];
                    }
            }
        }
        __syncthreads();
        const int row_base = wgrp * G::SP * 16 * MF + chunk * 16 * G::MFC;
        epilogue<bf16_t, EpiGeo<G::TPR, G::RPP, G::NPASS, G::PITCH, G::PROWS>, LNX>(p, Cs, m0 + row_base, n0, LnArgs{rowstat, row_base});
        if (pass + 1 < NPASSES) __syncthreads();
    }
}

template <int WM, int WN, int MF, int NF, int NST, int LW, bool LNX>
__global__ __launch_bounds__(64 * (WM * WN + LW)) void gemm_bf16_k64s_kernel(typename KernArg<LNX>::type pk, int gx, int gy, int tiles_m, int tiles_n) {
    const GemmParams p = widen(pk);
    using G = K64SGeo<WM, WN, MF, NF, NST, LW>;
    extern __shared__ __attribute__((aligned(16))) char smem[];
    int tm, tn;
    if (!shaped_tile(gx, gy, tiles_m, tiles_n, tm, tn)) return;
    const int m0 = tm * G::TBM, n0 = tn * G::TBN;
    const int tid = threadIdx.x, lane = tid & 63;
    const int wave = __builtin_amdgcn_readfirstlane(tid >> 6);
    if (p.ablate & 4) return;
    const int nk = (p.ablate & 2) ? 1 : (p.K >> 6);
    f32x4 acc[MF][NF];
#pragma unroll
    for (int i = 0; i < MF; ++i)
#pragma unroll
        for (int j = 0; j < NF; ++j) acc[i][j] = (f32x4){0.f, 0.f, 0.f, 0.f};
    const int wm = wave / WN, wn = wave % WN;
    float2* rowstat = reinterpret_cast<float2*>(smem + G::RING);

    if (wave >= G::NC) {
        k64s_loader_role<G>(reinterpret_cast<const char*>(p.A), reinterpret_cast<const char*>(p.B), p.lda * 2, p.ldb * 2, p.M, p.N, m0, n0, nk,
                            smem, wave - G::NC, lane);
    } else {
        const int frow = lane & 15, fk = lane >> 4;
        const int sw0 = ((fk ^ (frow & 7)) << 4);
        const int a_off = (wm * 16 * MF + frow) * 128;
        const int b_off = G::AOPER + (wn * 16 * NF + frow) * 128;
        bf16x8 fa[2][MF], fb[2][NF];
        auto read_frags = [&](int set, const char* st, int sw) {
#pragma unroll
            for (int i = 0; i < MF; ++i) fa[set][i] = *reinterpret_cast<const bf16x8*>(st + a_off + i * 2048 + sw);
#pragma unroll
            for (int j = 0; j < NF; ++j) fb[set][j] = *reinterpret_cast<const bf16x8*>(st + b_off + j * 2048 + sw);
        };
        auto mfma_all = [&](int set) {
#pragma unroll
            for (int i = 0; i < MF; ++i)
#pragma unroll
                for (int j = 0; j < NF; ++j)
                    acc[i][j] = __builtin_amdgcn_mfma_f32_16x16x32_bf16(fa[set][i], fb[set][j], acc[i][j], 0, 0, 0);
        };
        if (LNX) ln_rowstat_fill(p, rowstat, m0, n0, G::TBM, tid, 64 * G::NC);
        __builtin_amdgcn_s_barrier();
        read_frags(0, smem, sw0);
        int stage = 0;
        for (int t = 0; t < nk; ++t) {
            const char* st = smem + stage * G::STAGE;
            const int nstage = (stage + 1 == NST) ? 0 : stage + 1;
            __builtin_amdgcn_sched_barrier(0);
            __builtin_amdgcn_s_waitcnt(0xC07F);
            read_frags(1, st, sw0 ^ 64);
            mfma_all(0);
            __builtin_amdgcn_sched_barrier(0);
            __builtin_amdgcn_s_waitcnt(0xC07F);
            if (t + 1 < nk) {
                __builtin_amdgcn_s_barrier();
                read_frags(0, smem + nstage * G::STAGE, sw0);
            }
            mfma_all(1);
            stage = nstage;
        }
    }
    __syncthreads();
    if (p.ablate & 1) {
        if (acc[0][0][0] == 12345.678f) reinterpret_cast<float*>(p.C)[0] = acc[0][0][0];
        return;
    }
    k64s_store_tile<G, WM, WN, MF, NF, LNX>(p, acc, smem, wave, lane, m0, n0, rowstat);
}

template <int WM, int WN, int MF, int NF, int NST, int LW, bool WITH_LN = false>
int launch_k64s(const GemmParams& p, hipStream_t stream) {
    using G = K64SGeo<WM, WN, MF, NF, NST, LW>;
    const bool ln = p.ln_stats || p.stats_out || p.copy_out;
    if (ln && !WITH_LN) return EAVQA_E_SHAPE;
    static std::atomic<bool> configured{false};
    if (!configured.load(std::memory_order_acquire)) {
        if (hipFuncSetAttribute(reinterpret_cast<const void*>(gemm_bf16_k64s_kernel<WM, WN, MF, NF, NST, LW, false>),
                                hipFuncAttributeMaxDynamicSharedMemorySize, G::RING) != hipSuccess)
            return EAVQA_E_LAUNCH;
        if constexpr (WITH_LN) {
            if (hipFuncSetAttribute(reinterpret_cast<const void*>(gemm_bf16_k64s_kernel<WM, WN, MF, NF, NST, LW, true>),
                                    hipFuncAttributeMaxDynamicSharedMemorySize, G::RING + LN_ROWSTAT_BYTES) != hipSuccess)
                return EAVQA_E_LAUNCH;
        }
        configured.store(true, std::memory_order_release);
    }
    static_assert(!WITH_LN || G::RING + LN_ROWSTAT_BYTES <= 160 * 1024, "ring + row statistics of eavqa_gemm_ln");
    const int tiles_m = (p.M + G::TBM - 1) / G::TBM, tiles_n = (p.N + G::TBN - 1) / G::TBN;
    const GridPlan g = plan_grid(tiles_m, tiles_n, G::TBM, G::TBN);
    if constexpr (WITH_LN) {
        if (ln) {
            hipLaunchKernelGGL((gemm_bf16_k64s_kernel<WM, WN, MF, NF, NST, LW, true>), dim3(g.per_xcd * 8), dim3(G::NT), G::RING + ln_lds(p), stream, p,
                               g.gx, g.gy, tiles_m, tiles_n);
            EAVQA_LAUNCH_CHECK();
            return EAVQA_OK;
        }
    }
    hipLaunchKernelGGL((gemm_bf16_k64s_kernel<WM, WN, MF, NF, NST, LW, false>), dim3(g.per_xcd * 8), dim3(G::NT), G::RING, stream, p, g.gx, g.gy,
                       tiles_m, tiles_n);
    EAVQA_LAUNCH_CHECK();
    return EAVQA_OK;
}

struct K64Choice { int bm, bn, wg_per_cu; float rate; int (*launch)(const GemmParams&, hipStream_t); };
const K64Choice K64_SHAPES[] = {
    {128, 80, 2, 1.1f, launch_k64s<4, 1, 2, 5, 3, 2>},
    {128, 80, 2, 1.1f, launch_k64s<4, 1, 2, 5, 3, 4>},
    {128, 128, 2, 1.1f, launch_k64s<2, 2, 4, 4, 2, 4>},
    {256, 128, 1, 1.97f, launch_k64s<4, 2, 4, 4, 3, 4, true>},
    {256, 160, 1, 1.93f, launch_k64s<4, 2, 4, 5, 3, 4, true>},
    {128, 80, 1, 1.56f, launch_k64s<4, 1, 2, 5, 4, 2, true>},
    {128, 96, 1, 1.1f, launch_k64s<4, 1, 2, 6, 3, 2>},
    {256, 192, 1, 1.1f, launch_k64s<4, 2, 4, 6, 2, 4>},
    {256, 256, 1, 1.1f, launch_k64s<2, 4, 8, 4, 2, 4>},
    {128, 128, 1, 1.73f, launch_k64s<2, 2, 4, 4, 3, 2, true>},
    {128, 256, 1, 1.97f, launch_k64s<2, 4, 4, 4, 3, 4, true>},
};
constexpr int N_K64 = sizeof(K64_SHAPES) / sizeof(K64_SHAPES[0]);
constexpr int K64_AUTO[] = {5, 3, 4, 9, 10};
constexpr int N_K64_AUTO = sizeof(K64_AUTO) / sizeof(K64_AUTO[0]);
```

### explicit-alignment-for-vqa-tasks_amd/models/lm.py

```python
from __future__ import annotations

import json
import math
import os
from dataclasses import dataclass
from typing import Dict, Optional

import torch

from .. import ops

Tensor = torch.Tensor


@dataclass
class LMConfig:
    arch: str
    n_layer: int
    n_head: int
    n_embd: int
    ffn: int
    vocab: int
    n_pos: int
    eps: float = 1e-5
    act: str = "gelu_new"
    eos_token_id: Optional[int] = None
    pad_token_id: Optional[int] = None

    @property
    def head_dim(self) -> int:
        return self.n_embd // self.n_head

    @property
    def pos_mode(self) -> int:
        return 0 if self.arch == "gpt2" else 1

    @staticmethod
    def from_hf_dict(d: dict) -> "LMConfig":
        mt = d.get("model_type", "gpt2")
        if mt == "gpt2":
            E = d.get("n_embd", 768)
            return LMConfig("gpt2", d.get("n_layer", 12), d.get("n_head", 12), E, d.get("n_inner") or 4 * E,
                            d.get("vocab_size", 50257), d.get("n_positions", 1024), d.get("layer_norm_epsilon", 1e-5),
                            d.get("activation_function", "gelu_new"), d.get("eos_token_id", 50256), d.get("pad_token_id"))
        if mt == "opt":
            E = d.get("hidden_size", 768)
            if d.get("word_embed_proj_dim", E) != E or not d.get("do_layer_norm_before", True):
                raise NotImplementedError("OPT-350m style project_in/out / post-LN is not on the hot path")
            return LMConfig("opt", d.get("num_hidden_layers", 12), d.get("num_attention_heads", 12), E, d.get("ffn_dim", 3072),
                            d.get("vocab_size", 50272), d.get("max_position_embeddings", 2048), 1e-5,
                            d.get("activation_function", "relu"), d.get("eos_token_id", 2), d.get("pad_token_id", 1))
        raise NotImplementedError(f"model_type {mt!r} is not a causal LM on the hot path")


KNOWN_CONFIGS = {
    "gpt2": dict(model_type="gpt2", n_embd=768, n_layer=12, n_head=12, vocab_size=50257, n_positions=1024),
    "gpt2-medium": dict(model_type="gpt2", n_embd=1024, n_layer=24, n_head=16, vocab_size=50257, n_positions=1024),
    "gpt2-large": dict(model_type="gpt2", n_embd=1280, n_layer=36, n_head=20, vocab_size=50257, n_positions=1024),
    "gpt2-xl": dict(model_type="gpt2", n_embd=1600, n_layer=48, n_head=25, vocab_size=50257, n_positions=1024),
    "facebook/opt-125m": dict(model_type="opt", hidden_size=768, num_hidden_layers=12, num_attention_heads=12, ffn_dim=3072),
    "facebook/opt-1.3b": dict(model_type="opt", hidden_size=2048, num_hidden_layers=24, num_attention_heads=32, ffn_dim=8192),
    "facebook/opt-2.7b": dict(model_type="opt", hidden_size=2560, num_hidden_layers=32, num_attention_heads=32, ffn_dim=10240),
    "facebook/opt-6.7b": dict(model_type="opt", hidden_size=4096, num_hidden_layers=32, num_attention_heads=32, ffn_dim=16384),
}


def random_init_state_dict(cfg: LMConfig, seed: int = 2021, device="cpu") -> Dict[str, Tensor]:
    g = torch.Generator(device=device).manual_seed(seed)
    E, F, V = cfg.n_embd, cfg.ffn, cfg.vocab

    def n(*shape, std=0.02):
        return torch.randn(*shape, generator=g, device=device) * std

    sd: Dict[str, Tensor] = {}
    ones, zeros = (lambda k: torch.ones(k, device=device)), (lambda k: torch.zeros(k, device=device))
    if cfg.arch == "gpt2":
        sd["transformer.wte.weight"] = n(V, E)
        sd["transformer.wpe.weight"] = n(cfg.n_pos, E)
        ps = 0.02 / math.sqrt(2 * cfg.n_layer)
        for i in range(cfg.n_layer):
            p = f"transformer.h.{i}."
            sd[p + "ln_1.weight"], sd[p + "ln_1.bias"] = ones(E), zeros(E)
            sd[p + "attn.c_attn.weight"], sd[p + "attn.c_attn.bias"] = n(E, 3 * E), zeros(3 * E)
            sd[p + "attn.c_proj.weight"], sd[p + "attn.c_proj.bias"] = n(E, E, std=ps), zeros(E)
            sd[p + "ln_2.weight"], sd[p + "ln_2.bias"] = ones(E), zeros(E)
            sd[p + "mlp.c_fc.weight"], sd[p + "mlp.c_fc.bias"] = n(E, F), zeros(F)
            sd[p + "mlp.c_proj.weight"], sd[p + "mlp.c_proj.bias"] = n(F, E, std=ps), zeros(E)
        sd["transformer.ln_f.weight"], sd["transformer.ln_f.bias"] = ones(E), zeros(E)
    else:
        pre = "model.decoder."
        sd[pre + "embed_tokens.weight"] = n(V, E)
        sd[pre + "embed_positions.weight"] = n(cfg.n_pos + 2, E)
        for i in range(cfg.n_layer):
            p = f"{pre}layers.{i}."
            for nm in ("q_proj", "k_proj", "v_proj", "out_proj"):
                sd[p + f"self_attn.{nm}.weight"], sd[p + f"self_attn.{nm}.bias"] = n(E, E), zeros(E)
            sd[p + "self_attn_layer_norm.weight"], sd[p + "self_attn_layer_norm.bias"] = ones(E), zeros(E)
            sd[p + "fc1.weight"], sd[p + "fc1.bias"] = n(F, E), zeros(F)
            sd[p + "fc2.weight"], sd[p + "fc2.bias"] = n(E, F), zeros(E)
            sd[p + "final_layer_norm.weight"], sd[p + "final_layer_norm.bias"] = ones(E), zeros(E)
        sd[pre + "final_layer_norm.weight"], sd[pre + "final_layer_norm.bias"] = ones(E), zeros(E)
    return sd


def synthetic_weights_notice(model_version: str) -> None:
    if os.environ.get("EAVQA_REQUIRE_PRETRAINED", "0") == "1":
        raise FileNotFoundError(f"{model_version!r}: no local HF directory (EAVQA_MODEL_DIR) and EAVQA_REQUIRE_PRETRAINED=1 forbids "
                                "the seeded random-init stand-in")
    import warnings
    warnings.warn(f"{model_version!r} is not a local HF directory: using SEEDED RANDOM-INIT weights of that architecture (synthetic runs "
                  "only; set EAVQA_MODEL_DIR to a directory of HF checkpoints, or EAVQA_REQUIRE_PRETRAINED=1 to make this an error)",
                  RuntimeWarning, stacklevel=3)


def load_local_hf(path: str):
    with open(os.path.join(path, "config.json")) as f:
        cfg = json.load(f)
    st = os.path.join(path, "model.safetensors")
    if os.path.exists(st):
        from safetensors.torch import load_file
        return cfg, load_file(st)
    pt = os.path.join(path, "pytorch_model.bin")
    if os.path.exists(pt):
        return cfg, torch.load(pt, map_location="cpu", weights_only=True)
    raise FileNotFoundError(f"no model.safetensors / pytorch_model.bin under {path}")


class Fp8Weight:

    __slots__ = ("q", "scale", "shape")

    def __init__(self, q: Tensor, scale: float):
        self.q, self.scale, self.shape = q, float(scale), tuple(q.shape)

    @staticmethod
    def quantize(w: Tensor, device) -> "Fp8Weight":
        w = w.to(device=device, dtype=torch.float32)
        amax = float(w.abs().max().item())
        scale = amax / 448.0 if amax > 0 else 1.0
        q = (w / scale).to(torch.float8_e4m3fn).view(torch.uint8).contiguous()
        return Fp8Weight(q, scale)

    def t(self) -> "Fp8Weight":
        return Fp8Weight(self.q.T.contiguous(), self.scale)

    def dequantize(self) -> Tensor:
        return self.q.view(torch.float8_e4m3fn).float() * self.scale


def linear(a: Tensor, w, **kw) -> Tensor:
    if isinstance(w, Fp8Weight):
        aq, a_scale = a if isinstance(a, tuple) else ops.quantize_rows_fp8(a)
        return ops.gemm_fp8(aq, a_scale, w.q, w.scale, **kw)
    return ops.gemm(a, w, **kw)


class _Layer:
    __slots__ = ("ln1_g", "ln1_b", "w_qkv", "b_qkv", "w_o", "b_o", "ln2_g", "ln2_b", "w_fc1", "b_fc1", "w_fc2", "b_fc2",
                 "w_qkv_t", "w_o_t", "w_fc1_t", "w_fc2_t",
                 "w_qkv_f", "c_qkv", "d_qkv", "w_fc1_f", "c_fc1", "d_fc1")


class FrozenCausalLM:

    def __init__(self, cfg: LMConfig, state_dict: Dict[str, Tensor], dtype: torch.dtype = torch.bfloat16, device="cuda",
                 weight_format: str = "native"):
        self.cfg = cfg
        self.dtype = dtype
        self.device = torch.device(device)
        if weight_format not in ("native", "fp8"):
            raise ValueError("weight_format must be 'native' or 'fp8'")
        if weight_format == "fp8" and (dtype != torch.bfloat16 or cfg.n_embd % 128 or cfg.ffn % 128):
            raise ValueError("fp8 weights need bfloat16 activations and n_embd / ffn multiples of 128")
        self.weight_format = weight_format
        self._pack(state_dict)
        self._bwd_ready = False
        self.fold_layernorm = (dtype == torch.bfloat16 and weight_format == "native" and os.environ.get("EAVQA_LN_FOLD", "0") == "1")
        self._fold_ready = False
        self.fuse_quantizer = os.environ.get("EAVQA_FUSE_QUANT", "1") != "0"

    def _T(self, t: Tensor) -> Tensor:
        return t.to(device=self.device, dtype=self.dtype).contiguous()

    def _F(self, t: Tensor) -> Tensor:
        return t.to(device=self.device, dtype=torch.float32).contiguous()

    def _pack(self, sd: Dict[str, Tensor]) -> None:
        c = self.cfg
        self.layers = []
        if c.arch == "gpt2":
            self.wte = self._T(sd["transformer.wte.weight"])
            self.wpe = self._T(sd["transformer.wpe.weight"])
            for i in range(c.n_layer):
                p = f"transformer.h.{i}."
                L = _Layer()
                L.ln1_g, L.ln1_b = self._F(sd[p + "ln_1.weight"]), self._F(sd[p + "ln_1.bias"])
                L.w_qkv, L.b_qkv = self._T(sd[p + "attn.c_attn.weight"].T), self._F(sd[p + "attn.c_attn.bias"])
                L.w_o, L.b_o = self._T(sd[p + "attn.c_proj.weight"].T), self._F(sd[p + "attn.c_proj.bias"])
                L.ln2_g, L.ln2_b = self._F(sd[p + "ln_2.weight"]), self._F(sd[p + "ln_2.bias"])
                L.w_fc1, L.b_fc1 = self._T(sd[p + "mlp.c_fc.weight"].T), self._F(sd[p + "mlp.c_fc.bias"])
                L.w_fc2, L.b_fc2 = self._T(sd[p + "mlp.c_proj.weight"].T), self._F(sd[p + "mlp.c_proj.bias"])
                L.w_qkv_t = L.w_o_t = L.w_fc1_t = L.w_fc2_t = None
                self.layers.append(L)
            self.lnf_g, self.lnf_b = self._F(sd["transformer.ln_f.weight"]), self._F(sd["transformer.ln_f.bias"])
            head = sd.get("lm_head.weight")
        else:
            pre = "model.decoder."
            self.wte = self._T(sd[pre + "embed_tokens.weight"])
            self.wpe = self._T(sd[pre + "embed_positions.weight"])
            for i in range(c.n_layer):
                p = f"{pre}layers.{i}."
                L = _Layer()
                L.ln1_g, L.ln1_b = self._F(sd[p + "self_attn_layer_norm.weight"]), self._F(sd[p + "self_attn_layer_norm.bias"])
                L.w_qkv = self._T(torch.cat([sd[p + f"self_attn.{n}_proj.weight"] for n in "qkv"], dim=0))
                L.b_qkv = self._F(torch.cat([sd[p + f"self_attn.{n}_proj.bias"] for n in "qkv"], dim=0))
                L.w_o, L.b_o = self._T(sd[p + "self_attn.out_proj.weight"]), self._F(sd[p + "self_attn.out_proj.bias"])
                L.ln2_g, L.ln2_b = self._F(sd[p + "final_layer_norm.weight"]), self._F(sd[p + "final_layer_norm.bias"])
                L.w_fc1, L.b_fc1 = self._T(sd[p + "fc1.weight"]), self._F(sd[p + "fc1.bias"])
                L.w_fc2, L.b_fc2 = self._T(sd[p + "fc2.weight"]), self._F(sd[p + "fc2.bias"])
                L.w_qkv_t = L.w_o_t = L.w_fc1_t = L.w_fc2_t = None
                self.layers.append(L)
            self.lnf_g, self.lnf_b = self._F(sd[pre + "final_layer_norm.weight"]), self._F(sd[pre + "final_layer_norm.bias"])
            head = sd.get("lm_head.weight")
        self.head = self.wte if head is None or head.shape == self.wte.shape and _same(head, self.wte) else self._T(head)
        self.head_t = None
        self.head_q = None
        if self.weight_format == "fp8":
            for L in self.layers:
                for name in ("w_qkv", "w_o", "w_fc1", "w_fc2"):
                    setattr(L, name, Fp8Weight.quantize(getattr(L, name), self.device))
            self.head_q = Fp8Weight.quantize(self.head, self.device)

    @property
    def vocab(self) -> int:
        return self.wte.shape[0]

    @property
    def vpad(self) -> int:
        q = 128 if self.weight_format == "fp8" else 64
        return (self.vocab + q - 1) // q * q

    def _prepare_backward(self) -> None:
        if self._bwd_ready:
            return
        tr = (lambda w: w.t()) if self.weight_format == "fp8" else (lambda w: w.T.contiguous())
        for L in self.layers:
            L.w_qkv_t = tr(L.w_qkv)
            L.w_o_t = tr(L.w_o)
            L.w_fc1_t = tr(L.w_fc1)
            L.w_fc2_t = tr(L.w_fc2)
        V, E = self.head.shape
        if self.weight_format == "fp8":
            qt = torch.zeros((E, self.vpad), device=self.device, dtype=torch.uint8)
            qt[:, :V] = self.head_q.q.T
            self.head_t = Fp8Weight(qt, self.head_q.scale)
        else:
            self.head_t = torch.zeros((E, self.vpad), device=self.device, dtype=self.dtype)
            self.head_t[:, :V] = self.head.T
        self._bwd_ready = True

    def _prepare_fold(self) -> None:
        if self._fold_ready:
            return
        for L in self.layers:
            for w, b, g, be, nm in ((L.w_qkv, L.b_qkv, L.ln1_g, L.ln1_b, "qkv"), (L.w_fc1, L.b_fc1, L.ln2_g, L.ln2_b, "fc1")):
                w32 = w.float()
                wf = (w32 * g[None, :]).to(self.dtype).contiguous()
                setattr(L, f"w_{nm}_f", wf)
                setattr(L, f"c_{nm}", wf.float().sum(1).contiguous())
                setattr(L, f"d_{nm}", (w32 @ be + b).contiguous())
                del w32
        self._fold_ready = True

    def resize_token_embeddings(self, n: int) -> None:
        V, E = self.wte.shape
        if n == V:
            return
        tied = self.head is self.wte
        new = torch.empty((n, E), device=self.device, dtype=self.dtype)
        keep = min(n, V)
        new[:keep] = self.wte[:keep]
        if n > V:
            new[V:] = self.wte.float().mean(0).to(self.dtype)
        self.wte = new
        if tied:
            self.head = new
        else:
            h = torch.empty((n, E), device=self.device, dtype=self.dtype)
            h[:keep] = self.head[:keep]
            if n > V:
                h[V:] = self.head.float().mean(0).to(self.dtype)
            self.head = h
        self.cfg.vocab = n
        self._bwd_ready = False
        if self.weight_format == "fp8":
            self.head_q = Fp8Weight.quantize(self.head, self.device)

    def load_token_embeddings(self, weight: Tensor) -> None:
        if tuple(weight.shape) != tuple(self.wte.shape):
            raise ValueError(f"token embedding shape {tuple(weight.shape)} does not match {tuple(self.wte.shape)}")
        tied = self.head is self.wte
        self.wte = self._T(weight)
        if tied:
            self.head = self.wte
        self._bwd_ready = False
        if self.weight_format == "fp8":
            self.head_q = Fp8Weight.quantize(self.head, self.device)

    def forward(self, prefix_rows: Optional[Tensor], src: Tensor, pos: Tensor, mask: Tensor, B: int, S: int, *,
                labels: Optional[Tensor] = None, save: bool = False, logits: str = "none", pack: bool = False,
                lengths=None, n_scored: Optional[int] = None):
        c, T = self.cfg, self.dtype
        E, H, hd = c.n_embd, c.n_head, c.head_dim
        scale = hd ** -0.5
        cu = flat = row_labels = None
        M = B * S
        if pack:
            cu, src_r, pos_r, row_labels, flat = ops.build_row_plan(mask, labels, src, pos, True)
            M = int(sum(lengths)) if lengths is not None else int(cu[-1].item())
            src, pos, flat = src_r[:M], pos_r[:M], flat[:M]
            row_labels = row_labels[:M] if labels is not None else None
            attn_mask = None
        else:
            attn_mask = mask
        x = ops.embed_assemble(src, pos, self.wte, prefix_rows, self.wpe)
        tape = [] if save else None
        fold = self.fold_layernorm and M > 64
        if fold:
            self._prepare_fold()
        n_slots = (E + 63) // 64
        f32 = dict(device=self.device, dtype=torch.float32)
        fuse_q = self.weight_format == "fp8" and self.fuse_quantizer

        def ln(xx, g, b, stats):
            if fuse_q:
                r = ops.layernorm_fwd_fp8(xx, g, b, c.eps, save_stats=stats)
                return ((r[0], r[1]), r[2], r[3]) if stats else r
            return ops.layernorm_fwd(xx, g, b, c.eps, T, save_stats=stats)

        xT = st = None
        for li, L in enumerate(self.layers):
            if st is not None:
                mean1, rstd1 = (torch.empty(M, **f32), torch.empty(M, **f32)) if save else (None, None)
                qkv = ops.gemm(xT, L.w_qkv_f, bias=L.d_qkv, ln_stats=st, ln_c=L.c_qkv, ln_eps=c.eps, ln_save=(mean1, rstd1) if save else None)
            else:
                if save:
                    a, mean1, rstd1 = ln(x, L.ln1_g, L.ln1_b, True)
                else:
                    a = ln(x, L.ln1_g, L.ln1_b, False)
                qkv = linear(a, L.w_qkv, bias=L.b_qkv)
            q, k, v = qkv[:, :E], qkv[:, E:2 * E], qkv[:, 2 * E:]
            if save:
                ctx, lse = ops.attention_fwd(q, k, v, B, H, S, S, hd, key_mask=attn_mask, causal=True, scale=scale,
                                             save_lse=True, cu_seqlens=cu)
            else:
                ctx = ops.attention_fwd(q, k, v, B, H, S, S, hd, key_mask=attn_mask, causal=True, scale=scale, cu_seqlens=cu)
            if fold:
                x1T = torch.empty((M, E), device=self.device, dtype=T)
                st1 = torch.empty((M, n_slots, 2), **f32)
                x1 = ops.gemm(ctx, L.w_o, bias=L.b_o, residual=x, out_f32=True, copy_out=x1T, stats_out=st1)
                mean2, rstd2 = (torch.empty(M, **f32), torch.empty(M, **f32)) if save else (None, None)
                u = torch.empty((M, c.ffn), device=self.device, dtype=T) if save else None
                f = ops.gemm(x1T, L.w_fc1_f, bias=L.d_fc1, act=c.act, aux_out=u, ln_stats=st1, ln_c=L.c_fc1, ln_eps=c.eps,
                             ln_save=(mean2, rstd2) if save else None)
                if li + 1 < len(self.layers):
                    xT = torch.empty((M, E), device=self.device, dtype=T)
                    st = torch.empty((M, n_slots, 2), **f32)
                    x2 = ops.gemm(f, L.w_fc2, bias=L.b_fc2, residual=x1, out_f32=True, copy_out=xT, stats_out=st)
                else:
                    x2 = ops.gemm(f, L.w_fc2, bias=L.b_fc2, residual=x1, out_f32=True)
            else:
                x1 = linear(ctx, L.w_o, bias=L.b_o, residual=x, out_f32=True)
                if save:
                    a2, mean2, rstd2 = ln(x1, L.ln2_g, L.ln2_b, True)
                    u = torch.empty((M, c.ffn), device=self.device, dtype=T)
                    f = linear(a2, L.w_fc1, bias=L.b_fc1, act=c.act, aux_out=u)
                else:
                    a2 = ln(x1, L.ln2_g, L.ln2_b, False)
                    f = linear(a2, L.w_fc1, bias=L.b_fc1, act=c.act)
                x2 = linear(f, L.w_fc2, bias=L.b_fc2, residual=x1, out_f32=True)
            if save:
                tape.append((x, mean1, rstd1, qkv, ctx, lse, x1, mean2, rstd2, u))
            x = x2
        out = {"rows": M, "flat_index": flat}
        if logits == "last" and labels is None and not pack:
            xl = x.view(B, S, E)[:, -1]
            hf = ops.layernorm_fwd(xl, self.lnf_g, self.lnf_b, c.eps, T)
            out["logits"] = self._head(hf)
            return out
        if save:
            hf, meanf, rstdf = ops.layernorm_fwd(x, self.lnf_g, self.lnf_b, c.eps, T, save_stats=True)
        else:
            hf = ops.layernorm_fwd(x, self.lnf_g, self.lnf_b, c.eps, T)
        out["hidden"] = hf
        if labels is not None or logits == "all":
            sel = sel_count = None
            if pack and labels is not None and n_scored is not None and logits != "all" and 0 < n_scored < M:
                sel, ce_labels, sel_count = ops.select_rows(row_labels, int(n_scored))
                lg = self._head(ops.gather_rows(hf, sel))
            else:
                lg = self._head(hf)
                ce_labels = row_labels if pack else labels
            out["logits"], out["sel"] = lg, sel
            if labels is not None:
                loss, count, row_lse = ops.ce_fwd(lg, ce_labels, self.vocab)
                if sel_count is not None:
                    ops.guard_count(sel_count, int(n_scored), loss)
                out["loss"], out["count"] = loss, count
                if save:
                    out["tape"] = dict(layers=tape, x_last=x, meanf=meanf, rstdf=rstdf, logits=lg, labels=ce_labels, sel=sel,
                                       row_lse=row_lse, count=count, src=src, mask=attn_mask, cu=cu, B=B, S=S, M=M)
        return out

    def _head(self, hf: Tensor) -> Tensor:
        lg = torch.empty((hf.shape[0], self.vpad), device=self.device, dtype=torch.float32)
        if self.head_q is not None:
            linear(hf, self.head_q, out=lg[:, :self.vocab])
            return lg
        if hf.shape[0] <= 64 and hf.dtype == torch.bfloat16 and self.vocab % 4 == 0 and self.cfg.n_embd % 32 == 0:
            ops.splitk_finish(ops.gemm_splitk(hf, self.head[:self.vocab]), [lg[:, :self.vocab]])
        else:
            ops.gemm(hf, self.head, out=lg[:, :self.vocab])
        return lg

    def backward(self, tape: dict, gloss: Tensor, n_prefix_rows: int) -> Tensor:
        self._prepare_backward()
        c, T = self.cfg, self.dtype
        E, H, hd = c.n_embd, c.n_head, c.head_dim
        B, S, M = tape["B"], tape["S"], tape["M"]
        scale = hd ** -0.5
        mask, cu = tape["mask"], tape["cu"]
        lowp = T != torch.float32

        dlog = ops.ce_bwd(tape["logits"], tape["labels"], self.vocab, tape["row_lse"], tape["count"], gloss, T, self.vpad)
        dhf = linear(dlog, self.head_t)
        if tape.get("sel") is not None:
            dhf = ops.scatter_rows(dhf, tape["sel"], M)
        fuse_q = self.weight_format == "fp8" and self.fuse_quantizer
        if fuse_q:
            dxq = (torch.empty((M, E), device=self.device, dtype=torch.uint8), torch.empty(M, device=self.device, dtype=torch.float32))
            dxT = dxq

            def ln_bwd(xx, dy, g, mean, rstd, **kw):
                return ops.layernorm_bwd_fp8(xx, dy, g, mean, rstd, dxq[0], dxq[1], **kw)
        else:
            dxT = torch.empty((M, E), device=self.device, dtype=T) if lowp else None

            def ln_bwd(xx, dy, g, mean, rstd, **kw):
                return ops.layernorm_bwd(xx, dy, g, mean, rstd, lowp_out=dxT, **kw)
        dx = ln_bwd(tape["x_last"], dhf, self.lnf_g, tape["meanf"], tape["rstdf"])
        for L, (x, mean1, rstd1, qkv, ctx, lse, x1, mean2, rstd2, u) in zip(reversed(self.layers), reversed(tape["layers"])):
            du = linear(dxT if lowp else dx, L.w_fc2_t, act=c.act, aux_in=u)
            da2 = linear(du, L.w_fc1_t)
            dx1 = ln_bwd(x1, da2, L.ln2_g, mean2, rstd2, dres=dx, out=dx)
            dctx = linear(dxT if lowp else dx1, L.w_o_t)
            dqkv = torch.empty_like(qkv)
            q, k, v = qkv[:, :E], qkv[:, E:2 * E], qkv[:, 2 * E:]
            ops.attention_bwd(q, k, v, ctx, dctx, lse, B, H, S, S, hd, key_mask=mask, causal=True, scale=scale,
                              dq=dqkv[:, :E], dk=dqkv[:, E:2 * E], dv=dqkv[:, 2 * E:], cu_seqlens=cu)
            da = linear(dqkv, L.w_qkv_t)
            dx = ln_bwd(x, da, L.ln1_g, mean1, rstd1, dres=dx1, out=dx1)
        return ops.embed_assemble_bwd(tape["src"], dx, n_prefix_rows, T)


def _same(a: Tensor, b: Tensor) -> bool:
    try:
        return a.data_ptr() == b.data_ptr() or bool(torch.equal(a.to(b.device, b.dtype), b))
    except Exception:
        return False
```

### explicit-alignment-for-vqa-tasks_amd/ops.py

```python
from __future__ import annotations

import ctypes as C
from typing import Optional, Tuple

import torch

from . import _lib
from ._lib import ACT, BF16, F32, call

Tensor = torch.Tensor


F16 = 2


def dtype_id(dt: torch.dtype, stream: bool = False) -> int:
    if dt == torch.float32:
        return F32
    if dt == torch.bfloat16:
        return BF16
    if stream and dt == torch.float16:
        return F16
    raise _lib.EavqaError(f"unsupported storage dtype {dt}")


def _stream() -> int:
    return torch._C._cuda_getCurrentRawStream(torch._C._cuda_getDevice())


class KernelSelect:
    gemm = 0
    attention = 0
    decode_route = 0


def _p(t: Optional[Tensor]) -> Optional[int]:
    return None if t is None else t.data_ptr()


def _dev(t: Tensor) -> None:
    if not t.is_cuda:
        raise _lib.EavqaError("eavqa ops run on the GPU only (no CPU fallback): got a CPU tensor")


def _ld(t: Tensor) -> int:
    if t.stride(-1) != 1 and t.shape[-1] != 1:
        raise _lib.EavqaError("last dimension must be contiguous")
    return t.stride(-2) if t.dim() >= 2 else t.shape[-1]


def gemm(a: Tensor, b: Tensor, *, a_kc: bool = True, b_kc: bool = True, bias: Optional[Tensor] = None,
         act: str = "none", aux_in: Optional[Tensor] = None, aux_out: Optional[Tensor] = None,
         residual: Optional[Tensor] = None, out: Optional[Tensor] = None, out_f32: bool = False,
         alpha: float = 1.0, copy_out: Optional[Tensor] = None, stats_out: Optional[Tensor] = None, ln_stats: Optional[Tensor] = None,
         ln_c: Optional[Tensor] = None, ln_eps: float = 1e-5, ln_save: Optional[Tuple[Tensor, Tensor]] = None) -> Tensor:
    _dev(a)
    M, K = (a.shape if a_kc else (a.shape[1], a.shape[0]))
    N, Kb = (b.shape if b_kc else (b.shape[1], b.shape[0]))
    if K != Kb:
        raise _lib.EavqaError(f"gemm inner dims differ: {K} vs {Kb}")
    if a.dtype != b.dtype:
        raise _lib.EavqaError("gemm operands must share a dtype")
    dt = dtype_id(a.dtype)
    half = torch.float16
    if out is None:
        out = torch.empty((M, N), device=a.device, dtype=torch.float32 if out_f32 else a.dtype)
    elif out.dtype != torch.float32 and out.dtype != a.dtype and not (out.dtype == half and a.dtype == torch.bfloat16):
        raise _lib.EavqaError("gemm out dtype must be float32, the operand dtype or (bf16 operands) float16")
    out_f32 = out.dtype == torch.float32
    aux = aux_in if aux_in is not None else aux_out
    flags = int(out_f32)
    if residual is not None and residual.dtype != torch.float32:
        if residual.dtype != a.dtype and not (residual.dtype == half and a.dtype == torch.bfloat16):
            raise _lib.EavqaError("gemm residual must be float32, the operand dtype or (bf16 operands) float16")
        flags |= 2
    stream_half = (out.dtype == half) or (residual is not None and residual.dtype == half)
    if stream_half:
        if (out.dtype not in (half, torch.float32)) or (residual is not None and residual.dtype not in (half, torch.float32)):
            raise _lib.EavqaError("gemm: a float16 stream needs float16 (or float32) for both the residual and the output")
        flags |= 4
    args = (dt, int(a_kc), int(b_kc), M, N, K, _p(a), _ld(a), _p(b), _ld(b), _p(out), _ld(out),
            flags, float(alpha), _p(bias), ACT[act], _p(aux_in), _p(aux_out), _ld(aux) if aux is not None else 0,
            _p(residual), _ld(residual) if residual is not None else 0, _stream())
    if copy_out is not None or stats_out is not None or ln_stats is not None:
        g = _lib.GemmLn()
        if copy_out is not None:
            if copy_out.dtype != a.dtype or tuple(copy_out.shape) != (M, N):
                raise _lib.EavqaError("gemm copy_out must be [M, N] in the operand dtype")
            g.copy_out, g.ld_copy = _p(copy_out), _ld(copy_out)
        if stats_out is not None:
            if stats_out.dtype != torch.float32 or stats_out.dim() != 3 or stats_out.shape[0] != M or stats_out.shape[2] != 2 or not stats_out.is_contiguous():
                raise _lib.EavqaError("gemm stats_out must be a contiguous float32 [M, slots, 2]")
            g.stats_out, g.stats_ld = _p(stats_out), stats_out.shape[1]
        if ln_stats is not None:
            if ln_stats.dtype != torch.float32 or ln_stats.dim() != 3 or ln_stats.shape[0] != M or ln_stats.shape[2] != 2 or not ln_stats.is_contiguous():
                raise _lib.EavqaError("gemm ln_stats must be a contiguous float32 [M, slots, 2]")
            if ln_c is None or ln_c.dtype != torch.float32 or ln_c.numel() != N:
                raise _lib.EavqaError("gemm ln_c must be float32 [N]")
            g.ln_stats, g.ln_parts, g.ln_ld, g.ln_cols = _p(ln_stats), ln_stats.shape[1], ln_stats.shape[1], K
            g.ln_c, g.ln_eps = _p(ln_c), float(ln_eps)
            if ln_save is not None:
                g.mean_out, g.rstd_out = _p(ln_save[0]), _p(ln_save[1])
        if KernelSelect.gemm:
            call("eavqa_gemm_ln_ex", *args[:-1], C.byref(g), args[-1], KernelSelect.gemm)
        else:
            call("eavqa_gemm_ln", *args[:-1], C.byref(g), args[-1])
    elif KernelSelect.gemm:
        call("eavqa_gemm_ex", *args, KernelSelect.gemm)
    else:
        call("eavqa_gemm", *args)
    return out


def quantize_rows_fp8(x: Tensor):
    _dev(x)
    rows, cols = x.shape
    q = torch.empty((rows, cols), device=x.device, dtype=torch.uint8)
    sc = torch.empty(rows, device=x.device, dtype=torch.float32)
    call("eavqa_quantize_rows_fp8", dtype_id(x.dtype), rows, cols, _p(x), _ld(x), _p(q), _ld(q), _p(sc), _stream())
    return q, sc


def gemm_fp8(a_q: Tensor, a_scale: Tensor, b_q: Tensor, b_scale: float, *, bias: Optional[Tensor] = None, act: str = "none",
             aux_in: Optional[Tensor] = None, aux_out: Optional[Tensor] = None, residual: Optional[Tensor] = None,
             out: Optional[Tensor] = None, out_f32: bool = False, alpha: float = 1.0, tile: int = 0) -> Tensor:
    _dev(a_q)
    M, K = a_q.shape
    N = b_q.shape[0]
    if b_q.shape[1] != K:
        raise _lib.EavqaError(f"gemm_fp8 inner dims differ: {K} vs {b_q.shape[1]}")
    if out is None:
        out = torch.empty((M, N), device=a_q.device, dtype=torch.float32 if out_f32 else torch.bfloat16)
    aux = aux_in if aux_in is not None else aux_out
    call("eavqa_gemm_fp8", M, N, K, _p(a_q), _ld(a_q), _p(a_scale), _p(b_q), _ld(b_q), float(b_scale), _p(out), _ld(out),
         int(out.dtype == torch.float32), float(alpha), _p(bias), ACT[act], _p(aux_in), _p(aux_out), _ld(aux) if aux is not None else 0,
         _p(residual), _ld(residual) if residual is not None else 0, _stream(), int(tile))
    return out


def layernorm_fwd(x: Tensor, gamma: Optional[Tensor], beta: Optional[Tensor], eps: float, out_dtype: torch.dtype,
                  save_stats: bool = False, out: Optional[Tensor] = None):
    _dev(x)
    rows, cols = x.shape
    y = out if out is not None else torch.empty((rows, cols), device=x.device, dtype=out_dtype)
    mean = rstd = None
    if save_stats:
        mean = torch.empty(rows, device=x.device, dtype=torch.float32)
        rstd = torch.empty(rows, device=x.device, dtype=torch.float32)
    x_kind = {torch.float32: 1, torch.bfloat16: 2, torch.float16: 3}.get(x.dtype)
    if x_kind is None:
        raise _lib.EavqaError(f"unsupported layernorm input dtype {x.dtype}")
    call("eavqa_layernorm_fwd", dtype_id(out_dtype, stream=True), x_kind, rows, cols, _p(x), _ld(x),
         _p(gamma), _p(beta), float(eps), _p(y), _ld(y), _p(mean), _p(rstd), _stream())
    return (y, mean, rstd) if save_stats else y


def layernorm_fwd_fp8(x: Tensor, gamma: Optional[Tensor], beta: Optional[Tensor], eps: float, save_stats: bool = False):
    _dev(x)
    rows, cols = x.shape
    q = torch.empty((rows, cols), device=x.device, dtype=torch.uint8)
    sc = torch.empty(rows, device=x.device, dtype=torch.float32)
    mean = rstd = None
    if save_stats:
        mean = torch.empty(rows, device=x.device, dtype=torch.float32)
        rstd = torch.empty(rows, device=x.device, dtype=torch.float32)
    x_kind = {torch.float32: 1, torch.bfloat16: 2, torch.float16: 3}.get(x.dtype)
    if x_kind is None:
        raise _lib.EavqaError(f"unsupported layernorm input dtype {x.dtype}")
    call("eavqa_layernorm_fwd_fp8", x_kind, rows, cols, _p(x), _ld(x), _p(gamma), _p(beta), float(eps), _p(q), _ld(q), _p(sc), _p(mean), _p(rstd),
         _stream())
    return (q, sc, mean, rstd) if save_stats else (q, sc)


def layernorm_bwd_fp8(x: Tensor, dy: Tensor, gamma: Optional[Tensor], mean: Tensor, rstd: Tensor, q_out: Tensor, scale_out: Tensor,
                      dres: Optional[Tensor] = None, out: Optional[Tensor] = None) -> Tensor:
    _dev(x)
    rows, cols = x.shape
    if dy.dtype != torch.bfloat16:
        raise _lib.EavqaError("layernorm_bwd_fp8: dy must be bfloat16")
    dx = out if out is not None else torch.empty((rows, cols), device=x.device, dtype=torch.float32)
    if dres is not None and _ld(dres) != _ld(dx):
        raise _lib.EavqaError("dres must share dx's leading dimension")
    call("eavqa_layernorm_bwd_fp8", int(x.dtype == torch.float32), rows, cols, _p(x), _ld(x), _p(dy), _ld(dy), _p(gamma), _p(mean), _p(rstd),
         _p(dres), _p(dx), _ld(dx), _p(q_out), _ld(q_out), _p(scale_out), _stream())
    return dx


def layernorm_bwd(x: Tensor, dy: Tensor, gamma: Optional[Tensor], mean: Tensor, rstd: Tensor,
                  dres: Optional[Tensor] = None, dgamma: Optional[Tensor] = None, dbeta: Optional[Tensor] = None,
                  out: Optional[Tensor] = None, lowp_out: Optional[Tensor] = None) -> Tensor:
    _dev(x)
    rows, cols = x.shape
    dx = out if out is not None else torch.empty((rows, cols), device=x.device, dtype=torch.float32)
    if dres is not None and _ld(dres) != _ld(dx):
        raise _lib.EavqaError("dres must share dx's leading dimension")
    call("eavqa_layernorm_bwd", dtype_id(dy.dtype), int(x.dtype == torch.float32), rows, cols, _p(x), _ld(x), _p(dy), _ld(dy),
         _p(gamma), _p(mean), _p(rstd), _p(dres), _p(dx), _ld(dx), _p(dgamma), _p(dbeta), _p(lowp_out),
         _ld(lowp_out) if lowp_out is not None else 0, _stream())
    return dx


def attention_fwd(q: Tensor, k: Tensor, v: Tensor, B: int, H: int, Sq: int, Sk: int, hd: int, *,
                  key_mask: Optional[Tensor] = None, causal: bool = False, scale: float = 1.0, save_lse: bool = False,
                  q_batch_rows: int = 0, kv_batch_rows: int = 0, ld_mask: int = 0, out: Optional[Tensor] = None,
                  cu_seqlens: Optional[Tensor] = None):
    _dev(q)
    o = out if out is not None else torch.empty((q.shape[0] if cu_seqlens is not None else B * Sq, H * hd), device=q.device, dtype=q.dtype)
    lse = torch.empty((B, H, Sq), device=q.device, dtype=torch.float32) if save_lse else None
    args = (dtype_id(q.dtype), B, H, Sq, Sk, hd, _p(q), _ld(q), _p(k), _ld(k), _p(v), _ld(v), _p(o), _ld(o),
            q_batch_rows, kv_batch_rows, _p(key_mask), ld_mask, _p(cu_seqlens), int(causal), float(scale), _p(lse), _stream())
    if KernelSelect.attention:
        call("eavqa_attention_fwd_ex", *args, KernelSelect.attention)
    else:
        call("eavqa_attention_fwd", *args)
    return (o, lse) if save_lse else o


def attention_decode(q: Tensor, k_cache: Tensor, v_cache: Tensor, k_new: Tensor, v_new: Tensor, B: int, H: int, Sk: int, hd: int, *,
                     kv_batch_rows: int, key_mask: Optional[Tensor] = None, ld_mask: int = 0, scale: float = 1.0,
                     out: Optional[Tensor] = None) -> Tensor:
    _dev(q)
    o = out if out is not None else torch.empty((B, H * hd), device=q.device, dtype=q.dtype)
    call("eavqa_attention_decode", dtype_id(q.dtype), B, H, Sk, hd, _p(q), _ld(q), _p(k_cache), _ld(k_cache), _p(v_cache), _ld(v_cache),
         kv_batch_rows, _p(k_new), _p(v_new), _ld(k_new), _p(o), _ld(o), _p(key_mask), ld_mask, float(scale), _stream())
    return o


def attention_decode_splitk(part: Tensor, bias: Optional[Tensor], k_cache: Tensor, v_cache: Tensor, B: int, H: int, Sk: int, hd: int, *,
                            kv_batch_rows: int, key_mask: Optional[Tensor] = None, ld_mask: int = 0, scale: float = 1.0,
                            out: Optional[Tensor] = None) -> Tensor:
    _dev(part)
    o = out if out is not None else torch.empty((B, H * hd), device=part.device, dtype=k_cache.dtype)
    call("eavqa_attention_decode_splitk", dtype_id(k_cache.dtype), B, H, Sk, hd, _p(part), part.shape[0], _p(bias), _p(k_cache), _ld(k_cache),
         _p(v_cache), _ld(v_cache), kv_batch_rows, _p(o), _ld(o), _p(key_mask), ld_mask, float(scale), _stream())
    return o


def attention_bwd(q, k, v, o, d_o, lse, B, H, Sq, Sk, hd, *, key_mask=None, causal=False, scale=1.0,
                  dq=None, dk=None, dv=None, cu_seqlens=None):
    _dev(q)
    nq = q.shape[0] if cu_seqlens is not None else B * Sq
    nk = k.shape[0] if cu_seqlens is not None else B * Sk
    dq = dq if dq is not None else torch.empty((nq, H * hd), device=q.device, dtype=q.dtype)
    dk = dk if dk is not None else torch.empty((nk, H * hd), device=q.device, dtype=q.dtype)
    dv = dv if dv is not None else torch.empty((nk, H * hd), device=q.device, dtype=q.dtype)
    delta = torch.empty((B, H, Sq), device=q.device, dtype=torch.float32)
    args = (dtype_id(q.dtype), B, H, Sq, Sk, hd, _p(q), _ld(q), _p(k), _ld(k), _p(v), _ld(v), _p(o), _ld(o),
            _p(d_o), _ld(d_o), _p(dq), _ld(dq), _p(dk), _ld(dk), _p(dv), _ld(dv), _p(key_mask), _p(cu_seqlens), int(causal),
            float(scale), _p(lse), _p(delta), _stream())
    if KernelSelect.attention:
        call("eavqa_attention_bwd_ex", *args, KernelSelect.attention)
    else:
        call("eavqa_attention_bwd", *args)
    return dq, dk, dv


def build_prefix_rows(tokens: Tensor, question_mask: Tensor, L: int, pos_mode: int, prefix_row_stride: Optional[int] = None,
                      prefix_row_offset: int = 0):
    _dev(tokens)
    B, T = tokens.shape
    tokens = tokens.contiguous()
    qm = question_mask.to(torch.int64).contiguous()
    S = L + T
    src = torch.empty((B, S), device=tokens.device, dtype=torch.int32)
    msk = torch.empty_like(src)
    pos = torch.empty_like(src)
    call("eavqa_build_prefix_rows", B, L, T, _p(tokens), _p(qm), pos_mode, L if prefix_row_stride is None else prefix_row_stride,
         prefix_row_offset, _p(src), _p(msk), _p(pos), _stream())
    return src, msk, pos


def build_fewshot_rows(tokens: Tensor, question_mask: Tensor, L: int, n_img: int, special_token_id: int, pos_mode: int):
    _dev(tokens)
    B, T = tokens.shape
    tokens = tokens.contiguous()
    qm = question_mask.to(torch.int64).contiguous()
    T_out = T + (L - 1) * n_img
    src = torch.empty((B, T_out), device=tokens.device, dtype=torch.int32)
    msk = torch.empty_like(src)
    pos = torch.empty_like(src)
    status = torch.empty(B, device=tokens.device, dtype=torch.int32)
    call("eavqa_build_fewshot_rows", B, T, L, n_img, int(special_token_id), _p(tokens), _p(qm), pos_mode, _p(src), _p(msk),
         _p(pos), _p(status), _stream())
    return src, msk, pos, status


def embed_assemble(src: Tensor, pos: Optional[Tensor], wte: Tensor, prefix_rows: Optional[Tensor], wpe: Optional[Tensor],
                   out: Optional[Tensor] = None) -> Tensor:
    _dev(src)
    rows = src.numel()
    E = wte.shape[1]
    x = out if out is not None else torch.empty((rows, E), device=src.device, dtype=torch.float32)
    call("eavqa_embed_assemble", dtype_id(wte.dtype), rows, E, _p(src), _p(pos), _p(wte), _ld(wte), _p(prefix_rows),
         _ld(prefix_rows) if prefix_rows is not None else 0, _p(wpe), _ld(wpe) if wpe is not None else 0, _p(x), _ld(x), _stream())
    return x


def embed_assemble_bwd(src: Tensor, dx: Tensor, n_prefix_rows: int, dtype: torch.dtype) -> Tensor:
    rows, E = dx.shape
    d = torch.zeros((n_prefix_rows, E), device=dx.device, dtype=dtype)
    call("eavqa_embed_assemble_bwd", dtype_id(dtype), rows, E, _p(src), _p(dx), _ld(dx), _p(d), _ld(d), _stream())
    return d


def build_labels(input_ids: Tensor, L: int, pad_token_id: int, bos_token_id: int = -1, mode: int = 0) -> Tensor:
    _dev(input_ids)
    B, T = input_ids.shape
    ids = input_ids.contiguous()
    out = torch.empty((B, L + T), device=ids.device, dtype=torch.int64)
    call("eavqa_build_labels", mode, B, T, L, _p(ids), int(pad_token_id), int(bos_token_id), _p(out), _stream())
    return out


def build_row_plan(mask: Tensor, labels: Optional[Tensor], src: Tensor, pos: Tensor, pack: bool):
    _dev(mask)
    B, S = mask.shape
    dev = mask.device
    cu = torch.empty(B + 1, device=dev, dtype=torch.int32)
    src_r = torch.empty(B * S, device=dev, dtype=torch.int32)
    pos_r = torch.empty(B * S, device=dev, dtype=torch.int32)
    flat = torch.empty(B * S, device=dev, dtype=torch.int32)
    lab = torch.empty(B * S, device=dev, dtype=torch.int64)
    call("eavqa_build_row_plan", B, S, int(pack), _p(mask), _p(labels), _p(src), _p(pos), _p(cu), _p(src_r), _p(pos_r), _p(lab),
         _p(flat), _stream())
    return cu, src_r, pos_r, lab, flat


def _ce_dims(labels: Tensor):
    if labels.dim() == 2:
        return labels.shape[0], labels.shape[1], labels.shape[0] * labels.shape[1]
    return labels.shape[0], 0, labels.shape[0]


def ce_fwd(logits: Tensor, labels: Tensor, V: int):
    _dev(logits)
    B, S, rows = _ce_dims(labels)
    row_loss = torch.empty(rows, device=logits.device, dtype=torch.float32)
    row_lse = torch.empty(rows, device=logits.device, dtype=torch.float32)
    loss = torch.empty(1, device=logits.device, dtype=torch.float32)
    count = torch.empty(1, device=logits.device, dtype=torch.float32)
    call("eavqa_ce_fwd", B, S, V, _p(logits), _ld(logits), _p(labels), _p(row_loss), _p(row_lse), _p(loss), _p(count), _stream())
    return loss, count, row_lse


def guard_count(count: Tensor, capacity: int, loss: Tensor) -> None:
    call("eavqa_guard_count", _p(count), int(capacity), _p(loss), _stream())


def ce_bwd(logits: Tensor, labels: Tensor, V: int, row_lse: Tensor, count: Tensor, gscale: Tensor, dtype: torch.dtype,
           ldd: int) -> Tensor:
    B, S, rows = _ce_dims(labels)
    d = torch.empty((rows, ldd), device=logits.device, dtype=dtype)
    call("eavqa_ce_bwd", dtype_id(dtype), B, S, V, _p(logits), _ld(logits), _p(labels), _p(row_lse), _p(count), _p(gscale),
         _p(d), ldd, _stream())
    return d


def greedy_pick(logits: Tensor, V: int, pad_token_id: int, eos_token_id: Optional[int], raw: Tensor, emitted_col: Tensor,
                unfinished: Tensor, logprob: Optional[Tensor] = None, any_unfinished: Optional[Tensor] = None) -> None:
    B = logits.shape[0]
    call("eavqa_greedy_pick", B, V, _p(logits), _ld(logits), int(pad_token_id if pad_token_id is not None else 0),
         int(eos_token_id) if eos_token_id is not None else -1, _p(raw), _p(emitted_col), emitted_col.stride(0),
         _p(unfinished), _p(logprob), _p(any_unfinished), _stream())


def adamw(param: Tensor, grad: Tensor, m: Tensor, v: Tensor, step: int, lr: float, beta1: float = 0.9, beta2: float = 0.999,
          eps: float = 1e-8, weight_decay: float = 0.01, grad_scale: float = 1.0, shadow: Optional[Tensor] = None) -> None:
    _dev(param)
    call("eavqa_adamw", param.numel(), _p(param), _p(grad), _p(m), _p(v), int(step), float(lr), float(beta1), float(beta2),
         float(eps), float(weight_decay), float(grad_scale), dtype_id(shadow.dtype) if shadow is not None else 0, _p(shadow), _stream())


def patchify(pixels: Tensor, ps: int, dtype: torch.dtype, ldp: int) -> Tensor:
    _dev(pixels)
    B, C3, img, _ = pixels.shape
    g = img // ps
    pixels = pixels.contiguous().float()
    out = torch.empty((B * g * g, ldp), device=pixels.device, dtype=dtype)
    call("eavqa_patchify", dtype_id(dtype), B, img, ps, _p(pixels), _p(out), ldp, _stream())
    return out


def vit_assemble(patch_embed: Tensor, cls: Tensor, pos: Tensor, B: int, n_patch: int) -> Tensor:
    W = patch_embed.shape[1]
    x = torch.empty((B * (n_patch + 1), W), device=patch_embed.device, dtype=torch.float32)
    call("eavqa_vit_assemble", dtype_id(patch_embed.dtype), B, n_patch, W, _p(patch_embed), _ld(patch_embed), _p(cls), _p(pos),
         _p(x), _ld(x), _stream())
    return x


def cast_rows(x: Tensor, dtype: torch.dtype, out: Optional[Tensor] = None) -> Tensor:
    rows, cols = x.shape
    y = out if out is not None else torch.empty((rows, cols), device=x.device, dtype=dtype)
    call("eavqa_cast_rows", dtype_id(dtype), rows, cols, _p(x), _ld(x), _p(y), _ld(y), _stream())
    return y


def copy_rows(src: Tensor, dst: Tensor, B: int, S: int, cols: int, src_batch_rows: int, dst_batch_rows: int, dst_row0: int) -> None:
    call("eavqa_copy_rows", dtype_id(src.dtype), B, S, cols, _p(src), _ld(src), src_batch_rows, _p(dst), _ld(dst),
         dst_batch_rows, dst_row0, _stream())


def colsum(x: Tensor, out: Tensor, accumulate: bool) -> None:
    rows, cols = x.shape
    call("eavqa_colsum", dtype_id(x.dtype), rows, cols, _p(x), _ld(x), _p(out), int(accumulate), _stream())


def transpose(x: Tensor, out: Optional[Tensor] = None) -> Tensor:
    rows, cols = x.shape
    y = out if out is not None else torch.empty((cols, rows), device=x.device, dtype=x.dtype)
    call("eavqa_transpose", dtype_id(x.dtype), rows, cols, _p(x), _ld(x), _p(y), _ld(y), _stream())
    return y


def gemm_splitk(a: Tensor, b: Tensor, ks: Optional[int] = None, unroll: int = 0, out: Optional[Tensor] = None) -> Tensor:
    M, K = a.shape
    N = b.shape[0]
    if ks is None:
        ks = int(_lib.load().eavqa_gemm_splitk_plan(M, N, K))
        if ks <= 0:
            raise _lib.EavqaError(f"eavqa_gemm_splitk: unsupported shape M={M} N={N} K={K}")
    part = out if out is not None else torch.empty((ks, M, N), device=a.device, dtype=torch.float32)
    if unroll:
        call("eavqa_gemm_splitk_ex", dtype_id(a.dtype), M, N, K, _p(a), _ld(a), _p(b), _ld(b), _p(part), ks, _stream(), unroll)
    else:
        call("eavqa_gemm_splitk", dtype_id(a.dtype), M, N, K, _p(a), _ld(a), _p(b), _ld(b), _p(part), ks, _stream())
    return part


def splitk_finish(part: Tensor, outs, bias: Optional[Tensor] = None, act: str = "none", residual: Optional[Tensor] = None) -> None:
    ks, M, N = part.shape
    o = list(outs) + [None] * (3 - len(outs))
    call("eavqa_splitk_finish", dtype_id(outs[0].dtype), M, N, _p(part), ks, _p(bias),
         _lib.ACT[act], _p(residual), residual.stride(0) if residual is not None else 0, int(outs[0].dtype == torch.float32), len(outs),
         _p(o[0]), o[0].stride(0), _p(o[1]), o[1].stride(0) if o[1] is not None else 0, _p(o[2]), o[2].stride(0) if o[2] is not None else 0,
         _stream())


def layernorm_splitk(x_in: Tensor, gamma: Tensor, beta: Tensor, eps: float, out_dtype, part: Optional[Tensor] = None,
                     bias: Optional[Tensor] = None, x_out: Optional[Tensor] = None) -> Tensor:
    rows, cols = x_in.shape
    y = torch.empty((rows, cols), device=x_in.device, dtype=out_dtype)
    call("eavqa_layernorm_splitk", dtype_id(out_dtype), rows, cols, _p(x_in), _ld(x_in), _p(part), 0 if part is None else part.shape[0],
         _p(bias), _p(x_out), _ld(x_out) if x_out is not None else 0, _p(gamma), _p(beta), float(eps), _p(y), _ld(y), _stream())
    return y


def gemm_fp8_splitk(a_q: Tensor, a_scale: Tensor, b_q: Tensor, b_scale: float, ks: Optional[int] = None, out: Optional[Tensor] = None) -> Tensor:
    M, K = a_q.shape
    N = b_q.shape[0]
    if ks is None:
        ks = int(_lib.load().eavqa_gemm_fp8_splitk_plan(M, N, K))
        if ks <= 0:
            raise _lib.EavqaError(f"eavqa_gemm_fp8_splitk: unsupported shape M={M} N={N} K={K}")
    part = out if out is not None else torch.empty((ks, M, N), device=a_q.device, dtype=torch.float32)
    call("eavqa_gemm_fp8_splitk", M, N, K, _p(a_q), _ld(a_q), _p(a_scale), _p(b_q), _ld(b_q), float(b_scale), _p(part), ks, _stream())
    return part


def layernorm_splitk_fp8(x_in: Tensor, gamma: Tensor, beta: Tensor, eps: float, part: Optional[Tensor] = None, bias: Optional[Tensor] = None,
                         x_out: Optional[Tensor] = None):
    rows, cols = x_in.shape
    yq = torch.empty((rows, cols), device=x_in.device, dtype=torch.uint8)
    sc = torch.empty(rows, device=x_in.device, dtype=torch.float32)
    call("eavqa_layernorm_splitk_fp8", rows, cols, _p(x_in), _ld(x_in), _p(part), 0 if part is None else part.shape[0], _p(bias), _p(x_out),
         _ld(x_out) if x_out is not None else 0, _p(gamma), _p(beta), float(eps), _p(yq), _ld(yq), _p(sc), _stream())
    return yq, sc


def rmsnorm_splitk(x_in: Tensor, gamma: Tensor, eps: float, out_dtype, part: Optional[Tensor] = None, x_out: Optional[Tensor] = None,
                   out: Optional[Tensor] = None) -> Tensor:
    rows, cols = x_in.shape
    y = out if out is not None else torch.empty((rows, cols), device=x_in.device, dtype=out_dtype)
    call("eavqa_rmsnorm_splitk", dtype_id(out_dtype), rows, cols, _p(x_in), _ld(x_in), _p(part), 0 if part is None else part.shape[0],
         _p(x_out), _ld(x_out) if x_out is not None else 0, _p(gamma), float(eps), _p(y), _ld(y), _stream())
    return y


def splitk_finish_gated(part: Tensor, act: str, out_dtype) -> Tensor:
    ks, M, N2 = part.shape
    h = torch.empty((M, N2 // 2), device=part.device, dtype=out_dtype)
    call("eavqa_splitk_finish_gated", dtype_id(out_dtype), M, N2 // 2, _p(part), ks, _lib.ACT[act], _p(h), _ld(h), _stream())
    return h


def attention_decode_splitk_rel(part: Tensor, k: Tensor, v: Tensor, B: int, H: int, Sk: int, hd: int, *, kv_batch_rows: int,
                                key_mask: Optional[Tensor] = None, scale: float = 1.0, rel_bias: Optional[Tensor] = None, rel_zero: int = 0) -> Tensor:
    ks, _, cols = part.shape
    o = torch.empty((B, H * hd), device=part.device, dtype=k.dtype)
    call("eavqa_attention_decode_splitk_rel", dtype_id(k.dtype), B, H, Sk, hd, _p(part), ks, cols, _p(k), k.stride(0), _p(v), v.stride(0),
         kv_batch_rows, _p(o), _ld(o), _p(key_mask), key_mask.stride(0) if key_mask is not None else 0, float(scale),
         _p(rel_bias), rel_bias.stride(0) if rel_bias is not None else 0, int(rel_zero), _stream())
    return o


def gemm_decode_cols(M: int, N: int, K: int, a_kind: int = 0, gated: bool = False) -> int:
    return int(_lib.load().eavqa_gemm_decode_cols(M, N, K, a_kind, int(gated)))


def gemm_decode(a: Tensor, b: Tensor, outs, *, norm: Optional[str] = None, gamma: Optional[Tensor] = None, beta: Optional[Tensor] = None,
                eps: float = 1e-5, stats_in: Optional[Tensor] = None, stats_in_cols: int = 0, gated: bool = False,
                bias: Optional[Tensor] = None, act: str = "none", residual: Optional[Tensor] = None, want_stats: bool = False, sel: int = 0):
    M, K = a.shape
    N = b.shape[0] // 2 if gated else b.shape[0]
    a_kind = {None: 0, "layer": 1, "rms": 2}[norm]
    g = _lib.DecodeGemm()
    g.M, g.N, g.K = M, N, K
    g.A, g.lda, g.a_kind = _p(a), _ld(a), a_kind
    g.gamma, g.beta, g.eps = _p(gamma), _p(beta), float(eps)
    if a_kind:
        g.stats_in, g.n_stats_in, g.stats_in_cols = _p(stats_in), stats_in.shape[1], int(stats_in_cols)
    g.B, g.ldb, g.gated_rows = _p(b), _ld(b), N if gated else 0
    g.bias, g.act = _p(bias), _lib.ACT[act]
    g.residual, g.ld_residual = _p(residual), residual.stride(0) if residual is not None else 0
    g.out_f32, g.n_seg = int(outs[0].dtype == torch.float32), len(outs)
    for i, o in enumerate(outs):
        g.out[i], g.ld_out[i] = _p(o), o.stride(0)
    stats = None
    if want_stats:
        nf = (sel & 0xF) * (8 if gated else 16) if (sel & 0xF) else gemm_decode_cols(M, N, K, a_kind, gated)
        if nf <= 0:
            raise _lib.EavqaError(f"eavqa_gemm_decode: unsupported shape M={M} N={N} K={K}")
        stats = torch.empty((M, (N + nf - 1) // nf, 2), device=a.device, dtype=torch.float32)
        g.stats_out = _p(stats)
    import ctypes
    if sel:
        call("eavqa_gemm_decode_ex", ctypes.byref(g), _stream(), sel)
    else:
        call("eavqa_gemm_decode", ctypes.byref(g), _stream())
    return stats


def l2_normalize_rows_(x: Tensor) -> Tensor:
    if x.dtype != torch.float32:
        raise _lib.EavqaError("l2_normalize_rows_: float32 only")
    call("eavqa_l2_normalize_rows", x.shape[0], x.shape[1], _p(x), _ld(x), _stream())
    return x


def topk_rows(scores: Tensor, k: int):
    if scores.dtype != torch.float32:
        raise _lib.EavqaError("topk_rows: float32 scores only")
    rows, cols = scores.shape
    val = torch.empty((rows, k), device=scores.device, dtype=torch.float32)
    idx = torch.empty((rows, k), device=scores.device, dtype=torch.int64)
    call("eavqa_topk_rows", rows, cols, _p(scores), _ld(scores), int(k), _p(val), _p(idx), _stream())
    return val, idx


def select_rows(row_labels: Tensor, capacity: int):
    M = row_labels.shape[0]
    idx = torch.zeros(capacity, device=row_labels.device, dtype=torch.int32)
    lab = torch.full((capacity,), -100, device=row_labels.device, dtype=torch.int64)
    cnt = torch.zeros(1, device=row_labels.device, dtype=torch.int32)
    call("eavqa_select_rows", M, _p(row_labels), int(capacity), _p(idx), _p(lab), _p(cnt), _stream())
    return idx, lab, cnt


def gather_rows(src: Tensor, idx: Tensor) -> Tensor:
    out = torch.empty((idx.shape[0], src.shape[1]), device=src.device, dtype=src.dtype)
    call("eavqa_move_rows", dtype_id(src.dtype), 0, idx.shape[0], src.shape[1], _p(src), _ld(src), _p(idx), _p(out), _ld(out), _stream())
    return out


def scatter_rows(src: Tensor, idx: Tensor, rows: int) -> Tensor:
    out = torch.zeros((rows, src.shape[1]), device=src.device, dtype=src.dtype)
    call("eavqa_move_rows", dtype_id(src.dtype), 1, idx.shape[0], src.shape[1], _p(src), _ld(src), _p(idx), _p(out), _ld(out), _stream())
    return out


_X_KIND = {torch.float32: 1, torch.bfloat16: 2, torch.float16: 3}


def rmsnorm_fwd(x: Tensor, gamma: Optional[Tensor], eps: float, out_dtype: torch.dtype, save_stats: bool = False):
    _dev(x)
    rows, cols = x.shape
    y = torch.empty((rows, cols), device=x.device, dtype=out_dtype)
    rstd = torch.empty(rows, device=x.device, dtype=torch.float32) if save_stats else None
    call("eavqa_rmsnorm_fwd", dtype_id(out_dtype), _X_KIND[x.dtype], rows, cols, _p(x), _ld(x), _p(gamma), float(eps), _p(y), _ld(y), _p(rstd), _stream())
    return (y, rstd) if save_stats else y


def rmsnorm_bwd(x: Tensor, dy: Tensor, gamma: Optional[Tensor], rstd: Tensor, dres: Optional[Tensor] = None, out: Optional[Tensor] = None,
                lowp_out: Optional[Tensor] = None) -> Tensor:
    _dev(x)
    rows, cols = x.shape
    dx = out if out is not None else torch.empty((rows, cols), device=x.device, dtype=torch.float32)
    if dres is not None and _ld(dres) != _ld(dx):
        raise _lib.EavqaError("dres must share dx's leading dimension")
    call("eavqa_rmsnorm_bwd", dtype_id(dy.dtype), _X_KIND[x.dtype], rows, cols, _p(x), _ld(x), _p(dy), _ld(dy), _p(gamma), _p(rstd), _p(dres),
         _p(dx), _ld(dx), _p(lowp_out), _ld(lowp_out) if lowp_out is not None else 0, _stream())
    return dx


def gated_act_fwd(u: Tensor, act: str) -> Tensor:
    _dev(u)
    rows, F2 = u.shape
    h = torch.empty((rows, F2 // 2), device=u.device, dtype=u.dtype)
    call("eavqa_gated_act_fwd", dtype_id(u.dtype), rows, F2 // 2, ACT[act], _p(u), _ld(u), _p(h), _ld(h), _stream())
    return h


def gated_act_bwd(u: Tensor, dh: Tensor, act: str) -> Tensor:
    rows, F2 = u.shape
    du = torch.empty_like(u)
    call("eavqa_gated_act_bwd", dtype_id(u.dtype), rows, F2 // 2, ACT[act], _p(u), _ld(u), _p(dh), _ld(dh), _p(du), _ld(du), _stream())
    return du


def attention_fwd_rel(q: Tensor, k: Tensor, v: Tensor, B: int, H: int, Sq: int, Sk: int, hd: int, *, rel_bias: Optional[Tensor], rel_zero: int = 0,
                      key_mask: Optional[Tensor] = None, causal: bool = False, scale: float = 1.0, save_lse: bool = False,
                      q_batch_rows: int = 0, kv_batch_rows: int = 0, ld_mask: int = 0):
    _dev(q)
    o = torch.empty((B * Sq, H * hd), device=q.device, dtype=q.dtype)
    lse = torch.empty((B, H, Sq), device=q.device, dtype=torch.float32) if save_lse else None
    call("eavqa_attention_fwd_rel", dtype_id(q.dtype), B, H, Sq, Sk, hd, _p(q), _ld(q), _p(k), _ld(k), _p(v), _ld(v), _p(o), _ld(o), q_batch_rows,
         kv_batch_rows, _p(key_mask), ld_mask, int(causal), float(scale), _p(rel_bias), rel_bias.stride(0) if rel_bias is not None else 0,
         int(rel_zero), _p(lse), _stream())
    return (o, lse) if save_lse else o


def attention_bwd_rel(q, k, v, o, d_o, lse, B, H, Sq, Sk, hd, *, rel_bias=None, rel_zero=0, key_mask=None, causal=False, scale=1.0,
                      dq=None, dk=None, dv=None):
    _dev(q)
    dq = dq if dq is not None else torch.empty((B * Sq, H * hd), device=q.device, dtype=q.dtype)
    dk = dk if dk is not None else torch.empty((B * Sk, H * hd), device=q.device, dtype=q.dtype)
    dv = dv if dv is not None else torch.empty((B * Sk, H * hd), device=q.device, dtype=q.dtype)
    delta = torch.empty((B, H, Sq), device=q.device, dtype=torch.float32)
    call("eavqa_attention_bwd_rel", dtype_id(q.dtype), B, H, Sq, Sk, hd, _p(q), _ld(q), _p(k), _ld(k), _p(v), _ld(v), _p(o), _ld(o), _p(d_o), _ld(d_o),
         _p(dq), _ld(dq), _p(dk), _ld(dk), _p(dv), _ld(dv), _p(key_mask), int(causal), float(scale), _p(rel_bias),
         rel_bias.stride(0) if rel_bias is not None else 0, int(rel_zero), _p(lse), _p(delta), _stream())
    return dq, dk, dv
```

### include/eavqa.h

```cpp
#ifndef EAVQA_H
#define EAVQA_H

#include <stdint.h>

#ifdef __cplusplus
extern "C" {
#endif
#pragma GCC visibility push(default)

#define EAVQA_ABI_VERSION 1

enum { EAVQA_F32 = 0, EAVQA_BF16 = 1,
       EAVQA_F16 = 2 };

enum { EAVQA_GEMM_OUT_F32 = 1, EAVQA_GEMM_RESIDUAL_LOWP = 2, EAVQA_GEMM_STREAM_F16 = 4 };
enum { EAVQA_ACT_NONE = 0, EAVQA_ACT_TANH = 1, EAVQA_ACT_RELU = 2, EAVQA_ACT_GELU_NEW = 3, EAVQA_ACT_QUICK_GELU = 4 };

enum {
    EAVQA_OK = 0,
    EAVQA_E_ARG = -1,
    EAVQA_E_ALIGN = -2,
    EAVQA_E_SHAPE = -3,
    EAVQA_E_DTYPE = -4,
    EAVQA_E_LAUNCH = -5,
    EAVQA_E_ARCH = -6
};

int eavqa_abi_version(void);
const char* eavqa_strerror(int code);
int eavqa_check_device(void);

int eavqa_gemm(int dtype, int a_kc, int b_kc, int M, int N, int K,
               const void* A, int64_t lda, const void* B, int64_t ldb,
               void* C, int64_t ldc, int out_flags, float alpha,
               const float* bias, int act,
               const void* aux_in, void* aux_out, int64_t ld_aux,
               const void* residual, int64_t ldr, void* stream);

typedef struct {
    void* copy_out; int64_t ld_copy;
    float* stats_out; int32_t stats_ld;
    const float* ln_stats; int32_t ln_parts; int32_t ln_ld; int32_t ln_cols;
    const float* ln_c; float ln_eps;
    float* mean_out; float* rstd_out;
} eavqa_gemm_ln_t;
int eavqa_gemm_ln(int dtype, int a_kc, int b_kc, int M, int N, int K,
                  const void* A, int64_t lda, const void* B, int64_t ldb,
                  void* C, int64_t ldc, int out_flags, float alpha,
                  const float* bias, int act,
                  const void* aux_in, void* aux_out, int64_t ld_aux,
                  const void* residual, int64_t ldr, const eavqa_gemm_ln_t* ln, void* stream);

int eavqa_layernorm_fwd(int dtype, int x_kind, int rows, int cols, const void* x, int64_t ldx,
                        const float* gamma, const float* beta, float eps,
                        void* y, int64_t ldy, float* mean, float* rstd, void* stream);
int eavqa_layernorm_bwd(int dtype, int x_f32, int rows, int cols, const void* x, int64_t ldx,
                        const void* dy, int64_t lddy, const float* gamma,
                        const float* mean, const float* rstd,
                        const float* dres, float* dx, int64_t lddx,
                        float* dgamma, float* dbeta, void* dx_lowp, int64_t ld_lowp, void* stream);
int eavqa_layernorm_fwd_fp8(int x_kind, int rows, int cols, const void* x, int64_t ldx, const float* gamma, const float* beta,
                            float eps, void* yq, int64_t ldq, float* row_scale, float* mean, float* rstd, void* stream);
int eavqa_layernorm_bwd_fp8(int x_f32, int rows, int cols, const void* x, int64_t ldx, const void* dy, int64_t lddy,
                            const float* gamma, const float* mean, const float* rstd, const float* dres, float* dx, int64_t lddx,
                            void* dxq, int64_t ldq, float* row_scale, void* stream);


int eavqa_attention_fwd(int dtype, int B, int H, int Sq, int Sk, int hd,
                        const void* q, int64_t ldq, const void* k, int64_t ldk,
                        const void* v, int64_t ldv, void* o, int64_t ldo,
                        int64_t q_batch_rows, int64_t kv_batch_rows,
                        const int32_t* key_mask, int64_t ld_mask, const int32_t* cu_seqlens, int causal, float scale,
                        float* lse, void* stream);
int eavqa_attention_decode(int dtype, int B, int H, int Sk, int hd, const void* q, int64_t ldq, void* k_cache, int64_t ldk,
                           void* v_cache, int64_t ldv, int64_t kv_batch_rows, const void* k_new, const void* v_new, int64_t ld_new,
                           void* o, int64_t ldo, const int32_t* key_mask, int64_t ld_mask, float scale, void* stream);
int eavqa_attention_decode_splitk(int dtype, int B, int H, int Sk, int hd, const float* qkv_partials, int ks, const float* qkv_bias,
                                  void* k_cache, int64_t ldk, void* v_cache, int64_t ldv, int64_t kv_batch_rows, void* o, int64_t ldo,
                                  const int32_t* key_mask, int64_t ld_mask, float scale, void* stream);
int eavqa_attention_bwd(int dtype, int B, int H, int Sq, int Sk, int hd,
                        const void* q, int64_t ldq, const void* k, int64_t ldk,
                        const void* v, int64_t ldv, const void* o, int64_t ldo,
                        const void* d_o, int64_t lddo,
                        void* dq, int64_t lddq, void* dk, int64_t lddk, void* dv, int64_t lddv,
                        const int32_t* key_mask, const int32_t* cu_seqlens, int causal, float scale,
                        const float* lse, float* delta, void* stream);

int eavqa_build_prefix_rows(int B, int L, int T, const int64_t* tokens, const int64_t* question_mask,
                            int pos_mode, int prefix_row_stride, int prefix_row_offset,
                            int32_t* src, int32_t* mask_out, int32_t* pos, void* stream);
int eavqa_build_fewshot_rows(int B, int T, int L, int n_img, int64_t special_token_id,
                             const int64_t* tokens, const int64_t* question_mask, int pos_mode,
                             int32_t* src, int32_t* mask_out, int32_t* pos, int32_t* status, void* stream);
int eavqa_build_row_plan(int B, int S, int pack, const int32_t* mask, const int64_t* labels, const int32_t* src,
                         const int32_t* pos, int32_t* cu_seqlens, int32_t* src_rows, int32_t* pos_rows,
                         int64_t* row_labels, int32_t* flat_index, void* stream);
int eavqa_copy_rows(int dtype, int B, int S, int cols, const void* src, int64_t lds, int64_t src_batch_rows,
                    void* dst, int64_t ldd, int64_t dst_batch_rows, int64_t dst_row0, void* stream);
int eavqa_select_rows(int M, const int64_t* row_labels, int capacity, int32_t* sel_idx, int64_t* sel_labels, int32_t* count,
                      void* stream);
int eavqa_move_rows(int dtype, int scatter, int n, int cols, const void* src, int64_t ld_src, const int32_t* idx, void* dst,
                    int64_t ld_dst, void* stream);
int eavqa_transpose(int dtype, int rows, int cols, const void* src, int64_t ld_src, void* dst, int64_t ld_dst, void* stream);
int eavqa_colsum(int dtype, int rows, int cols, const void* x, int64_t ldx, float* out, int accumulate, void* stream);
int eavqa_embed_assemble(int dtype, int rows, int E, const int32_t* src, const int32_t* pos,
                         const void* wte, int64_t ld_wte, const void* prefix_rows, int64_t ld_prefix,
                         const void* wpe, int64_t ld_wpe, float* x, int64_t ldx, void* stream);
int eavqa_embed_assemble_bwd(int dtype, int rows, int E, const int32_t* src, const float* dx, int64_t lddx,
                             void* dprefix, int64_t ld_dprefix, void* stream);

int eavqa_build_labels(int mode, int B, int T, int L, const int64_t* input_ids, int64_t pad_token_id,
                       int64_t bos_token_id, int64_t* labels_out, void* stream);

int eavqa_ce_fwd(int B, int S, int V, const float* logits, int64_t ld, const int64_t* labels,
                 float* row_loss, float* row_lse, float* loss, float* count, void* stream);
int eavqa_guard_count(const int32_t* count, int capacity, float* loss, void* stream);
int eavqa_ce_bwd(int dtype, int B, int S, int V, const float* logits, int64_t ld, const int64_t* labels,
                 const float* row_lse, const float* count, const float* gscale,
                 void* dlogits, int64_t ldd, void* stream);
int eavqa_greedy_pick(int B, int V, const float* logits, int64_t ld, int64_t pad_token_id, int64_t eos_token_id,
                      int32_t* raw, int64_t* emitted, int64_t ld_emitted, int32_t* unfinished, float* logprob,
                      int32_t* any_unfinished, void* stream);

int eavqa_adamw(int64_t n, float* param, const float* grad, float* m, float* v, int step,
                float lr, float beta1, float beta2, float eps, float weight_decay, float grad_scale,
                int shadow_dtype, void* shadow, void* stream);

int eavqa_patchify(int dtype, int B, int img, int ps, const float* pixels, void* patches, int64_t ldp, void* stream);
int eavqa_vit_assemble(int dtype, int B, int n_patch, int W, const void* patch_embed, int64_t ldpe,
                       const float* cls, const float* pos, float* x, int64_t ldx, void* stream);

typedef struct {
    const float* ln1_g; const float* ln1_b;
    const void* w_qkv; const float* b_qkv;
    const void* w_o; const float* b_o;
    const float* ln2_g; const float* ln2_b;
    const void* w_fc1; const float* b_fc1;
    const void* w_fc2; const float* b_fc2;
    void* k_cache; void* v_cache;
} eavqa_lm_layer_t;
int64_t eavqa_lm_block_workspace_bytes(int dtype, int rows, int E, int F);
int eavqa_lm_block_forward(int dtype, int n_layer, const eavqa_lm_layer_t* layers, int E, int H, int F, int act, float eps,
                           int B, int Sq, int row0, int S_max, float* x, const int32_t* key_mask, int64_t ld_mask,
                           void* workspace, int64_t workspace_bytes, void* stream);

typedef struct { float s_qkv, s_o, s_fc1, s_fc2; } eavqa_lm_layer_scales_t;
int64_t eavqa_lm_block_fp8_workspace_bytes(int rows, int E, int F);
int eavqa_lm_block_forward_fp8(int n_layer, const eavqa_lm_layer_t* layers, const eavqa_lm_layer_scales_t* scales, int E, int H, int F, int act,
                               float eps, int B, int Sq, int row0, int S_max, float* x, const int32_t* key_mask, int64_t ld_mask,
                               void* workspace, int64_t workspace_bytes, void* stream);

typedef struct {
    const float* ln_sa; const void* w_qkv; const void* w_o;
    const float* ln_ca; const void* w_q_ca; const void* w_o_ca;
    const float* ln_ff; const void* w_i; const void* w_o_ff;
    void* k_cache; void* v_cache;
    const void* cross_kv;
} eavqa_t5_dec_layer_t;
int64_t eavqa_t5_decoder_step_workspace_bytes(int dtype, int B, int E, int inner, int F, int gated);
int eavqa_t5_decoder_step(int dtype, int n_layer, const eavqa_t5_dec_layer_t* layers, const float* ln_final, int E, int inner, int H,
                          int F, int gated, int act, float eps, int B, int t, int t_max, int S, float* x, void* out,
                          const int32_t* enc_mask, int64_t ld_mask, const float* rel_bias, int64_t rel_ld, int rel_zero,
                          void* workspace, int64_t workspace_bytes, void* stream);

int eavqa_gemm_splitk_plan(int M, int N, int K);
int eavqa_gemm_splitk(int dtype, int M, int N, int K, const void* A, int64_t lda, const void* B, int64_t ldb,
                      float* partials, int ks, void* stream);
int eavqa_splitk_finish(int dtype, int M, int N, const float* partials, int ks, const float* bias, int act,
                        const float* residual, int64_t ld_residual, int out_f32, int n_seg,
                        void* out0, int64_t ld0, void* out1, int64_t ld1, void* out2, int64_t ld2, void* stream);
int eavqa_layernorm_splitk(int dtype, int rows, int cols, const float* x_in, int64_t ldx, const float* partials, int ks,
                           const float* bias, float* x_out, int64_t ld_out, const float* gamma, const float* beta,
                           float eps, void* y, int64_t ldy, void* stream);

int eavqa_gemm_fp8_splitk_plan(int M, int N, int K);
int eavqa_gemm_fp8_splitk(int M, int N, int K, const void* A, int64_t lda, const float* a_row_scale, const void* B, int64_t ldb,
                          float b_scale, float* partials, int ks, void* stream);
int eavqa_layernorm_splitk_fp8(int rows, int cols, const float* x_in, int64_t ldx, const float* partials, int ks, const float* bias,
                               float* x_out, int64_t ld_out, const float* gamma, const float* beta, float eps, void* yq, int64_t ldq,
                               float* row_scale, void* stream);

int eavqa_rmsnorm_splitk(int dtype, int rows, int cols, const float* x_in, int64_t ldx, const float* partials, int ks,
                         float* x_out, int64_t ld_out, const float* gamma, float eps, void* y, int64_t ldy, void* stream);
int eavqa_splitk_finish_gated(int dtype, int M, int F, const float* partials, int ks, int act, void* out, int64_t ld, void* stream);
int eavqa_attention_decode_splitk_rel(int dtype, int B, int H, int Sk, int hd, const float* partials, int ks, int part_cols,
                                      void* k, int64_t ldk, void* v, int64_t ldv, int64_t kv_batch_rows, void* o, int64_t ldo,
                                      const int32_t* key_mask, int64_t ld_mask, float scale, const float* rel_bias, int64_t rel_ld,
                                      int rel_zero, void* stream);

typedef struct {
    int M, N, K;
    const void* A; int64_t lda; int a_kind;
    const float* gamma; const float* beta; float eps;
    const float* stats_in; int n_stats_in; int stats_in_cols;
    const void* B; int64_t ldb; int gated_rows;
    const float* bias; int act;
    const float* residual; int64_t ld_residual;
    int out_f32; int n_seg; void* out[3]; int64_t ld_out[3];
    float* stats_out;
} eavqa_decode_gemm_t;
int eavqa_gemm_decode_cols(int M, int N, int K, int a_kind, int gated);
int eavqa_gemm_decode(const eavqa_decode_gemm_t* args, void* stream);

int eavqa_l2_normalize_rows(int rows, int cols, float* x, int64_t ld, void* stream);
int eavqa_topk_rows(int rows, int cols, const float* scores, int64_t ld, int k, float* out_val, int64_t* out_idx, void* stream);

int eavqa_quantize_rows_fp8(int dtype, int rows, int cols, const void* x, int64_t ldx, void* out, int64_t ld_out,
                            float* row_scale, void* stream);
int eavqa_gemm_fp8(int M, int N, int K, const void* A, int64_t lda, const float* a_row_scale, const void* B, int64_t ldb,
                   float b_scale, void* C, int64_t ldc, int out_f32, float alpha, const float* bias, int act,
                   const void* aux_in, void* aux_out, int64_t ld_aux, const float* residual, int64_t ldr, void* stream, int tile);

int eavqa_rmsnorm_fwd(int dtype, int x_kind, int rows, int cols, const void* x, int64_t ldx, const float* gamma, float eps,
                      void* y, int64_t ldy, float* rstd, void* stream);
int eavqa_rmsnorm_bwd(int dtype, int x_kind, int rows, int cols, const void* x, int64_t ldx, const void* dy, int64_t lddy,
                      const float* gamma, const float* rstd, const float* dres, float* dx, int64_t lddx, void* dx_lowp,
                      int64_t ld_lowp, void* stream);
int eavqa_gated_act_fwd(int dtype, int rows, int F, int act, const void* u, int64_t ldu, void* h, int64_t ldh, void* stream);
int eavqa_gated_act_bwd(int dtype, int rows, int F, int act, const void* u, int64_t ldu, const void* dh, int64_t lddh,
                        void* du, int64_t lddu, void* stream);
int eavqa_attention_fwd_rel(int dtype, int B, int H, int Sq, int Sk, int hd, const void* q, int64_t ldq, const void* k, int64_t ldk,
                            const void* v, int64_t ldv, void* o, int64_t ldo, int64_t q_batch_rows, int64_t kv_batch_rows,
                            const int32_t* key_mask, int64_t ld_mask, int causal, float scale, const float* rel_bias,
                            int64_t rel_ld, int rel_zero, float* lse, void* stream);
int eavqa_attention_bwd_rel(int dtype, int B, int H, int Sq, int Sk, int hd, const void* q, int64_t ldq, const void* k, int64_t ldk,
                            const void* v, int64_t ldv, const void* o, int64_t ldo, const void* d_o, int64_t lddo,
                            void* dq, int64_t lddq, void* dk, int64_t lddk, void* dv, int64_t lddv,
                            const int32_t* key_mask, int causal, float scale, const float* rel_bias, int64_t rel_ld,
                            int rel_zero, const float* lse, float* delta, void* stream);

int eavqa_cast_rows(int dtype, int rows, int64_t cols, const float* x, int64_t ldx, void* y, int64_t ldy, void* stream);

#pragma GCC visibility pop
#ifdef __cplusplus
}
#endif
#endif
```

Baseline: 4695 samples/s.

## Prefetch next layer's weights into cache during GEMM loader tail

Adds a prefetching variant of the k64 bf16 GEMM kernel. Near the end of the K loop and after the tile store, its loader waves touch the next GEMM's weight tensor one 128-byte line at a time, so those weights are warm in L2/MALL when the next kernel launches. The LM forward and backward passes now pass the next weight as a hint for each linear, enabled by default for native bf16 weights. The extra loads compete with the current GEMM for memory bandwidth and change vmcnt accounting, and they only help if the cache holds the next weight.

```diff
diff --git a/explicit-alignment-for-vqa-tasks_amd/_lib.py b/explicit-alignment-for-vqa-tasks_amd/_lib.py
--- a/explicit-alignment-for-vqa-tasks_amd/_lib.py
+++ b/explicit-alignment-for-vqa-tasks_amd/_lib.py
@@ -93,6 +93,7 @@
 
 
 SIGNATURES["eavqa_gemm_ln"] = SIGNATURES["eavqa_gemm"][:-1] + [C.POINTER(GemmLn), ptr]
+SIGNATURES["eavqa_gemm_pf"] = SIGNATURES["eavqa_gemm"] + [ptr, i64]
 SIGNATURES["eavqa_gemm_decode_cols"] = [i32, i32, i32, i32, i32]
 SIGNATURES["eavqa_gemm_decode"] = [C.POINTER(DecodeGemm), ptr]
 SIGNATURES["eavqa_t5_decoder_step_workspace_bytes"] = [i32, i32, i32, i32, i32, i32]
diff --git a/explicit-alignment-for-vqa-tasks_amd/csrc/gemm.hip b/explicit-alignment-for-vqa-tasks_amd/csrc/gemm.hip
--- a/explicit-alignment-for-vqa-tasks_amd/csrc/gemm.hip
+++ b/explicit-alignment-for-vqa-tasks_amd/csrc/gemm.hip
@@ -37,11 +37,14 @@
     const float* ln_stats = nullptr; int ln_parts = 0, ln_ld = 0;
     const float* ln_c = nullptr; float ln_inv_n = 0.f, ln_eps = 0.f;
     float* mean_out = nullptr; float* rstd_out = nullptr;
+    const void* pf_ptr = nullptr; int64_t pf_bytes = 0;
 };
+struct GemmParamsPf : GemmParamsBase { const void* pf_ptr; int64_t pf_bytes; };
 constexpr int LN_ROWSTAT_BYTES = 2048;
 inline int ln_lds(const GemmParams& p) { return p.ln_stats ? LN_ROWSTAT_BYTES : 0; }
 __device__ __forceinline__ GemmParams widen(const GemmParams& k) { return k; }
 __device__ __forceinline__ GemmParams widen(const GemmParamsBase& k) { GemmParams p; static_cast<GemmParamsBase&>(p) = k; return p; }
+__device__ __forceinline__ GemmParams widen(const GemmParamsPf& k) { GemmParams p = widen(static_cast<const GemmParamsBase&>(k)); p.pf_ptr = k.pf_ptr; p.pf_bytes = k.pf_bytes; return p; }
 template <bool LNX> struct KernArg { using type = GemmParamsBase; };
 template <> struct KernArg<true> { using type = GemmParams; };
 
@@ -1240,7 +1243,8 @@
               void* C, int64_t ldc, int out_flags, float alpha,
               const float* bias, int act,
               const void* aux_in, void* aux_out, int64_t ld_aux,
-              const void* residual, int64_t ldr, const eavqa_gemm_ln_t* ln, void* stream, int knobs) {
+              const void* residual, int64_t ldr, const eavqa_gemm_ln_t* ln, void* stream, int knobs,
+              const void* pf_ptr = nullptr, int64_t pf_bytes = 0) {
     const Knobs kn(knobs);
     const bool ln_consumer = ln && ln->ln_stats;
     if (ln) {
@@ -1291,6 +1295,7 @@
             p.ln_inv_n = 1.0f / float(ln->ln_cols); p.ln_eps = ln->ln_eps; p.mean_out = ln->mean_out; p.rstd_out = ln->rstd_out;
         }
     }
+    if (pf_ptr && pf_bytes > 0 && !ln) { p.pf_ptr = pf_ptr; p.pf_bytes = pf_bytes; }
     hipStream_t s = reinterpret_cast<hipStream_t>(stream);
     if (dtype == EAVQA_BF16) {
         if (a_kc && b_kc && (K % 64) == 0 && kn.k64_mode >= 2 && kn.k64_mode < 2 + N_K64) return K64_SHAPES[kn.k64_mode - 2].launch(p, s);
@@ -1407,6 +1412,17 @@
                          residual, ldr, stream, 0);
 }
 
+extern "C" int eavqa_gemm_pf(int dtype, int a_kc, int b_kc, int M, int N, int K,
+                             const void* A, int64_t lda, const void* B, int64_t ldb,
+                             void* C, int64_t ldc, int out_flags, float alpha,
+                             const float* bias, int act,
+                             const void* aux_in, void* aux_out, int64_t ld_aux,
+                             const void* residual, int64_t ldr, void* stream, const void* next_weight, int64_t next_weight_bytes) {
+    if (next_weight_bytes < 0) return EAVQA_E_ARG;
+    return gemm_impl(dtype, a_kc, b_kc, M, N, K, A, lda, B, ldb, C, ldc, out_flags, alpha, bias, act, aux_in, aux_out, ld_aux, residual, ldr,
+                     nullptr, stream, 0, next_weight, next_weight_bytes);
+}
+
 extern "C" int eavqa_quantize_rows_fp8(int dtype, int rows, int cols, const void* x, int64_t ldx, void* out, int64_t ld_out,
                                        float* row_scale, void* stream) {
     if (!x || !out || !row_scale || rows <= 0 || cols <= 0) return EAVQA_E_ARG;
diff --git a/explicit-alignment-for-vqa-tasks_amd/csrc/gemm_k64.hip b/explicit-alignment-for-vqa-tasks_amd/csrc/gemm_k64.hip
--- a/explicit-alignment-for-vqa-tasks_amd/csrc/gemm_k64.hip
+++ b/explicit-alignment-for-vqa-tasks_amd/csrc/gemm_k64.hip
@@ -21,10 +21,37 @@
     static_assert(P_HI * (NST - 1) <= 63 && NST >= 2 && NST <= 6, "vmcnt field");
 };
 
+struct LookAhead { const unsigned char* ptr; int64_t lines; };
+template <class G> struct PfGeo {
+    static constexpr int PER_LOADER = 8 / G::LW;
+    static constexpr int LINES = PER_LOADER * G::LW * 64;
+    static_assert(G::LW <= 8 && G::P_HI * (G::NST - 1) + PER_LOADER <= 63, "vmcnt field");
+};
+__device__ __forceinline__ unsigned pf_touch(const unsigned char* q) { return *(const __attribute__((address_space(1))) unsigned char*)q; }
+__device__ __forceinline__ void pf_piece(const LookAhead& la, int wg, int nwg, int64_t& first, int& count) {
+    const int64_t per = (la.lines + nwg - 1) / nwg;
+    first = per * wg;
+    count = (int)max((int64_t)0, min(per, la.lines - first));
+}
 template <class G>
+__device__ __forceinline__ void k64s_lookahead_tail(const LookAhead& la, int wg, int nwg, int lw, int lane) {
+    int64_t first;
+    int count;
+    pf_piece(la, wg, nwg, first, count);
+    for (int i0 = PfGeo<G>::LINES + lw * 64; i0 < count; i0 += 4 * G::LW * 64) {
+        unsigned v[4];
+#pragma unroll
+        for (int j = 0; j < 4; ++j) v[j] = pf_touch(la.ptr + (first + min(i0 + j * G::LW * 64 + lane, count - 1)) * 128);
+        asm volatile("" ::"v"(v[0]), "v"(v[1]), "v"(v[2]), "v"(v[3]));
+    }
+}
+
+template <class G, bool PF = false>
 __device__ __forceinline__ void k64s_loader_role(const char* A, const char* B, int64_t lda_bytes, int64_t ldb_bytes, int M, int N, int m0,
-                                                 int n0, int nk, char* smem, int lw, int lane) {
+                                                 int n0, int nk, char* smem, int lw, int lane, const LookAhead la = LookAhead{nullptr, 0},
+                                                 int wg = 0, int nwg = 1) {
     constexpr int NST = G::NST;
+    constexpr int PFN = PF ? PfGeo<G>::PER_LOADER : 0;
     const bool hi = lw < G::N_HI;
     const char* src[G::P_HI];
     int dst[G::P_HI];
@@ -45,26 +72,48 @@
                 __builtin_amdgcn_global_load_lds((const __attribute__((address_space(1))) void*)(src[i] + (int64_t)kt * 128),
                                                  (__attribute__((address_space(3))) void*)(st + dst[i]), 16, 0, 0);
     };
+    auto wait_tiles_x = [&](int tiles, auto xc) {
+        constexpr int X = decltype(xc)::value;
+        if (hi) {
+            if (NST >= 6 && tiles >= 5) wait_vm<(NST >= 6 ? 5 : 0) * G::P_HI + X>();
+            else if (NST >= 5 && tiles >= 4) wait_vm<(NST >= 5 ? 4 : 0) * G::P_HI + X>();
+            else if (NST >= 4 && tiles >= 3) wait_vm<(NST >= 4 ? 3 : 0) * G::P_HI + X>();
+            else if (NST >= 3 && tiles >= 2) wait_vm<(NST >= 3 ? 2 : 0) * G::P_HI + X>();
+            else if (tiles >= 1) wait_vm<G::P_HI + X>();
+            else wait_vm<X>();
+        } else {
+            if (NST >= 6 && tiles >= 5) wait_vm<(NST >= 6 ? 5 : 0) * G::P_LO + X>();
+            else if (NST >= 5 && tiles >= 4) wait_vm<(NST >= 5 ? 4 : 0) * G::P_LO + X>();
+            else if (NST >= 4 && tiles >= 3) wait_vm<(NST >= 4 ? 3 : 0) * G::P_LO + X>();
+            else if (NST >= 3 && tiles >= 2) wait_vm<(NST >= 3 ? 2 : 0) * G::P_LO + X>();
+            else if (tiles >= 1) wait_vm<G::P_LO + X>();
+            else wait_vm<X>();
+        }
+    };
+    bool pf_out = false;
     auto wait_tiles = [&](int tiles) {
-        if (hi) {
-            if (NST >= 6 && tiles >= 5) wait_vm<(NST >= 6 ? 5 : 0) * G::P_HI>();
-            else if (NST >= 5 && tiles >= 4) wait_vm<(NST >= 5 ? 4 : 0) * G::P_HI>();
-            else if (NST >= 4 && tiles >= 3) wait_vm<(NST >= 4 ? 3 : 0) * G::P_HI>();
-            else if (NST >= 3 && tiles >= 2) wait_vm<(NST >= 3 ? 2 : 0) * G::P_HI>();
-            else if (tiles >= 1) wait_vm<G::P_HI>();
-            else wait_vm<0>();
-        } else {
-            if (NST >= 6 && tiles >= 5) wait_vm<(NST >= 6 ? 5 : 0) * G::P_LO>();
-            else if (NST >= 5 && tiles >= 4) wait_vm<(NST >= 5 ? 4 : 0) * G::P_LO>();
-            else if (NST >= 4 && tiles >= 3) wait_vm<(NST >= 4 ? 3 : 0) * G::P_LO>();
-            else if (NST >= 3 && tiles >= 2) wait_vm<(NST >= 3 ? 2 : 0) * G::P_LO>();
-            else if (tiles >= 1) wait_vm<G::P_LO>();
-            else wait_vm<0>();
+        if (PF && pf_out) wait_tiles_x(tiles, std::integral_constant<int, PFN>{});
+        else wait_tiles_x(tiles, std::integral_constant<int, 0>{});
+    };
+    unsigned pfv[PFN > 0 ? PFN : 1];
+    auto look_ahead = [&]() {
+        if constexpr (PF) {
+            int64_t first;
+            int count;
+            pf_piece(la, wg, nwg, first, count);
+            if (count > 0) {
+                __builtin_amdgcn_sched_barrier(0);
+#pragma unroll
+                for (int j = 0; j < PFN; ++j) pfv[j] = pf_touch(la.ptr + (first + min((j * G::LW + lw) * 64 + lane, count - 1)) * 128);
+                __builtin_amdgcn_sched_barrier(0);
+                pf_out = true;
+            }
         }
     };
 #pragma unroll
     for (int i = 0; i < NST; ++i)
         if (i < nk) issue(i, i);
+    if (PF && nk <= NST) look_ahead();
     wait_tiles(min(nk, NST) - 1);
     __builtin_amdgcn_s_barrier();
     int stage = 0;
@@ -72,7 +121,14 @@
         wait_tiles(min(nk - 1, t + NST - 1) - (t + 1));
         __builtin_amdgcn_s_barrier();
         if (t + NST < nk) issue(t + NST, stage);
+        if (PF && t + NST == nk - 1) look_ahead();
         stage = (stage + 1 == NST) ? 0 : stage + 1;
+    }
+    if constexpr (PF) {
+        if (pf_out) {
+#pragma unroll
+            for (int j = 0; j < PFN; ++j) asm volatile("" ::"v"(pfv[j]));
+        }
     }
 }
 
@@ -107,9 +163,8 @@
     }
 }
 
-template <int WM, int WN, int MF, int NF, int NST, int LW, bool LNX>
-__global__ __launch_bounds__(64 * (WM * WN + LW)) void gemm_bf16_k64s_kernel(typename KernArg<LNX>::type pk, int gx, int gy, int tiles_m, int tiles_n) {
-    const GemmParams p = widen(pk);
+template <int WM, int WN, int MF, int NF, int NST, int LW, bool LNX, bool PF>
+__device__ __forceinline__ void k64s_body(const GemmParams& p, int gx, int gy, int tiles_m, int tiles_n) {
     using G = K64SGeo<WM, WN, MF, NF, NST, LW>;
     extern __shared__ __attribute__((aligned(16))) char smem[];
     int tm, tn;
@@ -127,9 +182,11 @@
     const int wm = wave / WN, wn = wave % WN;
     float2* rowstat = reinterpret_cast<float2*>(smem + G::RING);
 
+    const LookAhead la{reinterpret_cast<const unsigned char*>(p.pf_ptr), p.pf_bytes >> 7};
+    const int wg = tn * tiles_m + tm, nwg = tiles_m * tiles_n;
     if (wave >= G::NC) {
-        k64s_loader_role<G>(reinterpret_cast<const char*>(p.A), reinterpret_cast<const char*>(p.B), p.lda * 2, p.ldb * 2, p.M, p.N, m0, n0, nk,
-                            smem, wave - G::NC, lane);
+        k64s_loader_role<G, PF>(reinterpret_cast<const char*>(p.A), reinterpret_cast<const char*>(p.B), p.lda * 2, p.ldb * 2, p.M, p.N, m0, n0, nk,
+                                smem, wave - G::NC, lane, la, wg, nwg);
     } else {
         const int frow = lane & 15, fk = lane >> 4;
         const int sw0 = ((fk ^ (frow & 7)) << 4);
@@ -176,6 +233,16 @@
         return;
     }
     k64s_store_tile<G, WM, WN, MF, NF, LNX>(p, acc, smem, wave, lane, m0, n0, rowstat);
+    if (PF && wave >= G::NC) k64s_lookahead_tail<G>(la, wg, nwg, wave - G::NC, lane);
+}
+
+template <int WM, int WN, int MF, int NF, int NST, int LW, bool LNX>
+__global__ __launch_bounds__(64 * (WM * WN + LW)) void gemm_bf16_k64s_kernel(typename KernArg<LNX>::type pk, int gx, int gy, int tiles_m, int tiles_n) {
+    k64s_body<WM, WN, MF, NF, NST, LW, LNX, false>(widen(pk), gx, gy, tiles_m, tiles_n);
+}
+template <int WM, int WN, int MF, int NF, int NST, int LW>
+__global__ __launch_bounds__(64 * (WM * WN + LW)) void gemm_bf16_k64s_pf_kernel(GemmParamsPf pk, int gx, int gy, int tiles_m, int tiles_n) {
+    k64s_body<WM, WN, MF, NF, NST, LW, false, true>(widen(pk), gx, gy, tiles_m, tiles_n);
 }
 
 template <int WM, int WN, int MF, int NF, int NST, int LW, bool WITH_LN = false>
@@ -192,6 +259,9 @@
             if (hipFuncSetAttribute(reinterpret_cast<const void*>(gemm_bf16_k64s_kernel<WM, WN, MF, NF, NST, LW, true>),
                                     hipFuncAttributeMaxDynamicSharedMemorySize, G::RING + LN_ROWSTAT_BYTES) != hipSuccess)
                 return EAVQA_E_LAUNCH;
+            if (hipFuncSetAttribute(reinterpret_cast<const void*>(gemm_bf16_k64s_pf_kernel<WM, WN, MF, NF, NST, LW>),
+                                    hipFuncAttributeMaxDynamicSharedMemorySize, G::RING) != hipSuccess)
+                return EAVQA_E_LAUNCH;
         }
         configured.store(true, std::memory_order_release);
     }
@@ -202,6 +272,16 @@
         if (ln) {
             hipLaunchKernelGGL((gemm_bf16_k64s_kernel<WM, WN, MF, NF, NST, LW, true>), dim3(g.per_xcd * 8), dim3(G::NT), G::RING + ln_lds(p), stream, p,
                                g.gx, g.gy, tiles_m, tiles_n);
+            EAVQA_LAUNCH_CHECK();
+            return EAVQA_OK;
+        }
+        if (p.pf_ptr && p.pf_bytes >= 128) {
+            GemmParamsPf pk;
+            static_cast<GemmParamsBase&>(pk) = p;
+            pk.pf_ptr = p.pf_ptr;
+            pk.pf_bytes = p.pf_bytes;
+            hipLaunchKernelGGL((gemm_bf16_k64s_pf_kernel<WM, WN, MF, NF, NST, LW>), dim3(g.per_xcd * 8), dim3(G::NT), G::RING, stream, pk, g.gx, g.gy,
+                               tiles_m, tiles_n);
             EAVQA_LAUNCH_CHECK();
             return EAVQA_OK;
         }
diff --git a/explicit-alignment-for-vqa-tasks_amd/models/lm.py b/explicit-alignment-for-vqa-tasks_amd/models/lm.py
--- a/explicit-alignment-for-vqa-tasks_amd/models/lm.py
+++ b/explicit-alignment-for-vqa-tasks_amd/models/lm.py
@@ -150,6 +150,7 @@
 
 def linear(a: Tensor, w, **kw) -> Tensor:
     if isinstance(w, Fp8Weight):
+        kw.pop("prefetch", None)
         aq, a_scale = a if isinstance(a, tuple) else ops.quantize_rows_fp8(a)
         return ops.gemm_fp8(aq, a_scale, w.q, w.scale, **kw)
     return ops.gemm(a, w, **kw)
@@ -177,6 +178,7 @@
         self._bwd_ready = False
         self.fold_layernorm = (dtype == torch.bfloat16 and weight_format == "native" and os.environ.get("EAVQA_LN_FOLD", "0") == "1")
         self._fold_ready = False
+        self.weight_prefetch = (dtype == torch.bfloat16 and weight_format == "native" and os.environ.get("EAVQA_WEIGHT_PREFETCH", "1") != "0")
         self.fuse_quantizer = os.environ.get("EAVQA_FUSE_QUANT", "1") != "0"
 
     def _T(self, t: Tensor) -> Tensor:
@@ -231,6 +233,13 @@
                     setattr(L, name, Fp8Weight.quantize(getattr(L, name), self.device))
             self.head_q = Fp8Weight.quantize(self.head, self.device)
 
+    PREFETCH_MAX_BYTES = 64 << 20
+
+    def _hint(self, w):
+        if not self.weight_prefetch or not isinstance(w, torch.Tensor) or w.numel() * w.element_size() > self.PREFETCH_MAX_BYTES:
+            return None
+        return w
+
     @property
     def vocab(self) -> int:
         return self.wte.shape[0]
@@ -338,6 +347,7 @@
                 return ((r[0], r[1]), r[2], r[3]) if stats else r
             return ops.layernorm_fwd(xx, g, b, c.eps, T, save_stats=stats)
 
+        hint = (lambda w: None) if fold else self._hint
         xT = st = None
         for li, L in enumerate(self.layers):
             if st is not None:
@@ -348,7 +358,7 @@
                     a, mean1, rstd1 = ln(x, L.ln1_g, L.ln1_b, True)
                 else:
                     a = ln(x, L.ln1_g, L.ln1_b, False)
-                qkv = linear(a, L.w_qkv, bias=L.b_qkv)
+                qkv = linear(a, L.w_qkv, bias=L.b_qkv, prefetch=hint(L.w_o))
             q, k, v = qkv[:, :E], qkv[:, E:2 * E], qkv[:, 2 * E:]
             if save:
                 ctx, lse = ops.attention_fwd(q, k, v, B, H, S, S, hd, key_mask=attn_mask, causal=True, scale=scale,
@@ -370,15 +380,16 @@
                 else:
                     x2 = ops.gemm(f, L.w_fc2, bias=L.b_fc2, residual=x1, out_f32=True)
             else:
-                x1 = linear(ctx, L.w_o, bias=L.b_o, residual=x, out_f32=True)
+                x1 = linear(ctx, L.w_o, bias=L.b_o, residual=x, out_f32=True, prefetch=hint(L.w_fc1))
                 if save:
                     a2, mean2, rstd2 = ln(x1, L.ln2_g, L.ln2_b, True)
                     u = torch.empty((M, c.ffn), device=self.device, dtype=T)
-                    f = linear(a2, L.w_fc1, bias=L.b_fc1, act=c.act, aux_out=u)
+                    f = linear(a2, L.w_fc1, bias=L.b_fc1, act=c.act, aux_out=u, prefetch=hint(L.w_fc2))
                 else:
                     a2 = ln(x1, L.ln2_g, L.ln2_b, False)
-                    f = linear(a2, L.w_fc1, bias=L.b_fc1, act=c.act)
-                x2 = linear(f, L.w_fc2, bias=L.b_fc2, residual=x1, out_f32=True)
+                    f = linear(a2, L.w_fc1, bias=L.b_fc1, act=c.act, prefetch=hint(L.w_fc2))
+                nxt = self.layers[li + 1].w_qkv if li + 1 < len(self.layers) else self.head
+                x2 = linear(f, L.w_fc2, bias=L.b_fc2, residual=x1, out_f32=True, prefetch=hint(nxt))
             if save:
                 tape.append((x, mean1, rstd1, qkv, ctx, lse, x1, mean2, rstd2, u))
             x = x2
@@ -433,7 +444,8 @@
         lowp = T != torch.float32
 
         dlog = ops.ce_bwd(tape["logits"], tape["labels"], self.vocab, tape["row_lse"], tape["count"], gloss, T, self.vpad)
-        dhf = linear(dlog, self.head_t)
+        hint = self._hint
+        dhf = linear(dlog, self.head_t, prefetch=hint(self.layers[-1].w_fc2_t))
         if tape.get("sel") is not None:
             dhf = ops.scatter_rows(dhf, tape["sel"], M)
         fuse_q = self.weight_format == "fp8" and self.fuse_quantizer
@@ -449,16 +461,17 @@
             def ln_bwd(xx, dy, g, mean, rstd, **kw):
                 return ops.layernorm_bwd(xx, dy, g, mean, rstd, lowp_out=dxT, **kw)
         dx = ln_bwd(tape["x_last"], dhf, self.lnf_g, tape["meanf"], tape["rstdf"])
-        for L, (x, mean1, rstd1, qkv, ctx, lse, x1, mean2, rstd2, u) in zip(reversed(self.layers), reversed(tape["layers"])):
-            du = linear(dxT if lowp else dx, L.w_fc2_t, act=c.act, aux_in=u)
-            da2 = linear(du, L.w_fc1_t)
+        for li, (L, (x, mean1, rstd1, qkv, ctx, lse, x1, mean2, rstd2, u)) in enumerate(zip(reversed(self.layers), reversed(tape["layers"]))):
+            du = linear(dxT if lowp else dx, L.w_fc2_t, act=c.act, aux_in=u, prefetch=hint(L.w_fc1_t))
+            da2 = linear(du, L.w_fc1_t, prefetch=hint(L.w_o_t))
             dx1 = ln_bwd(x1, da2, L.ln2_g, mean2, rstd2, dres=dx, out=dx)
-            dctx = linear(dxT if lowp else dx1, L.w_o_t)
+            dctx = linear(dxT if lowp else dx1, L.w_o_t, prefetch=hint(L.w_qkv_t))
             dqkv = torch.empty_like(qkv)
             q, k, v = qkv[:, :E], qkv[:, E:2 * E], qkv[:, 2 * E:]
             ops.attention_bwd(q, k, v, ctx, dctx, lse, B, H, S, S, hd, key_mask=mask, causal=True, scale=scale,
                               dq=dqkv[:, :E], dk=dqkv[:, E:2 * E], dv=dqkv[:, 2 * E:], cu_seqlens=cu)
-            da = linear(dqkv, L.w_qkv_t)
+            below = self.layers[len(self.layers) - 2 - li].w_fc2_t if li + 1 < len(self.layers) else None
+            da = linear(dqkv, L.w_qkv_t, prefetch=hint(below))
             dx = ln_bwd(x, da, L.ln1_g, mean1, rstd1, dres=dx1, out=dx1)
         return ops.embed_assemble_bwd(tape["src"], dx, n_prefix_rows, T)
 
diff --git a/explicit-alignment-for-vqa-tasks_amd/ops.py b/explicit-alignment-for-vqa-tasks_amd/ops.py
--- a/explicit-alignment-for-vqa-tasks_amd/ops.py
+++ b/explicit-alignment-for-vqa-tasks_amd/ops.py
@@ -53,7 +53,8 @@
          act: str = "none", aux_in: Optional[Tensor] = None, aux_out: Optional[Tensor] = None,
          residual: Optional[Tensor] = None, out: Optional[Tensor] = None, out_f32: bool = False,
          alpha: float = 1.0, copy_out: Optional[Tensor] = None, stats_out: Optional[Tensor] = None, ln_stats: Optional[Tensor] = None,
-         ln_c: Optional[Tensor] = None, ln_eps: float = 1e-5, ln_save: Optional[Tuple[Tensor, Tensor]] = None) -> Tensor:
+         ln_c: Optional[Tensor] = None, ln_eps: float = 1e-5, ln_save: Optional[Tuple[Tensor, Tensor]] = None,
+         prefetch: Optional[Tensor] = None) -> Tensor:
     _dev(a)
     M, K = (a.shape if a_kc else (a.shape[1], a.shape[0]))
     N, Kb = (b.shape if b_kc else (b.shape[1], b.shape[0]))
@@ -82,7 +83,14 @@
     args = (dt, int(a_kc), int(b_kc), M, N, K, _p(a), _ld(a), _p(b), _ld(b), _p(out), _ld(out),
             flags, float(alpha), _p(bias), ACT[act], _p(aux_in), _p(aux_out), _ld(aux) if aux is not None else 0,
             _p(residual), _ld(residual) if residual is not None else 0, _stream())
-    if copy_out is not None or stats_out is not None or ln_stats is not None:
+    ln_form = copy_out is not None or stats_out is not None or ln_stats is not None
+    if prefetch is not None:
+        if not prefetch.is_contiguous() or prefetch.device != a.device:
+            raise _lib.EavqaError("gemm prefetch must be a contiguous tensor on the operands' device")
+        if ln_form or KernelSelect.gemm:
+            raise _lib.EavqaError("gemm prefetch cannot be combined with the eavqa_gemm_ln arguments or a kernel selector")
+        call("eavqa_gemm_pf", *args, prefetch.data_ptr(), prefetch.numel() * prefetch.element_size())
+    elif ln_form:
         g = _lib.GemmLn()
         if copy_out is not None:
             if copy_out.dtype != a.dtype or tuple(copy_out.shape) != (M, N):
diff --git a/include/eavqa.h b/include/eavqa.h
--- a/include/eavqa.h
+++ b/include/eavqa.h
@@ -50,6 +50,13 @@
                   const float* bias, int act,
                   const void* aux_in, void* aux_out, int64_t ld_aux,
                   const void* residual, int64_t ldr, const eavqa_gemm_ln_t* ln, void* stream);
+
+int eavqa_gemm_pf(int dtype, int a_kc, int b_kc, int M, int N, int K,
+                  const void* A, int64_t lda, const void* B, int64_t ldb,
+                  void* C, int64_t ldc, int out_flags, float alpha,
+                  const float* bias, int act,
+                  const void* aux_in, void* aux_out, int64_t ld_aux,
+                  const void* residual, int64_t ldr, void* stream, const void* next_weight, int64_t next_weight_bytes);
 
 int eavqa_layernorm_fwd(int dtype, int x_kind, int rows, int cols, const void* x, int64_t ldx,
                         const float* gamma, const float* beta, float eps,
```

After: 4917 samples/s, median of 6. 1.05x the previous value.
